# ska-telescope/ska-sdp-distributed-fourier-transform

Measured on AMD Instinct MI355X. Metric: facet_to_subgrid_contributions_per_s, higher is better.
Workload: dtype complex64 (f32 arithmetic)

## Files before the change

include/swiftly_hip.h:

```cpp
#ifndef SWIFTLY_HIP_H
#define SWIFTLY_HIP_H

#include <stddef.h>
#include <stdint.h>

#ifdef __cplusplus
extern "C" {
#endif

typedef struct swiftly_hip swiftly_hip_t;

enum { SWIFTLY_C64 = 0, SWIFTLY_C128 = 1 };
enum {
    SWIFTLY_OK = 0,
    SWIFTLY_ERR_PARAM = 1,
    SWIFTLY_ERR_UNSUPPORTED = 2,
    SWIFTLY_ERR_HIP = 3
};

const char* swiftly_hip_last_error(void);
int swiftly_hip_version(void);
int swiftly_hip_device_count(void);
const char* swiftly_hip_build_id(void);

int swiftly_hip_create(swiftly_hip_t** out, int64_t N, int64_t yN_size, int64_t xM_size, double W,
                       const double* pswf, int device);
void swiftly_hip_destroy(swiftly_hip_t* h);
int64_t swiftly_hip_contribution_size(const swiftly_hip_t* h);
int swiftly_hip_supports_dtype(const swiftly_hip_t* h, int dtype);
enum {
    SWIFTLY_FEATURE_FUSED_SUBGRID = 0,
    SWIFTLY_FEATURE_BAND_PIPELINE = 1,
    SWIFTLY_FEATURE_BAND_PIPELINE_EXPLICIT = 2,
    SWIFTLY_FEATURE_BACKWARD_BAND = 3,
    SWIFTLY_FEATURE_SPLIT_BAND = 4,
    SWIFTLY_FEATURE_WINDOW_ROWS = 5,
    SWIFTLY_FEATURE_BACKWARD_BAND_EXPLICIT = 6,
    SWIFTLY_FEATURE_SPLIT_PREPARE = 7
};
int swiftly_hip_supports(int feature, int dtype, int64_t N, int64_t yN_size, int64_t xM_size, int64_t n_facets);
enum {
    SWIFTLY_LIMIT_FUSED_FACETS = 0,
    SWIFTLY_LIMIT_WINDOW_ROWS_STAGE_COLUMNS = 1,
    SWIFTLY_LIMIT_WINDOW_ROWS_WINDOWS = 2
};
int64_t swiftly_hip_limit(int which);
int swiftly_hip_mixed_factor(int64_t n, int* Q, int* log2_rest);
int swiftly_hip_set_column_precision(swiftly_hip_t* h, int bits);
int swiftly_hip_get_column_precision(const swiftly_hip_t* h);
void swiftly_hip_chain_chunk_streams(int chain);


int swiftly_hip_prepare_facet(swiftly_hip_t* h, int dtype, const void* in, int64_t rows, int64_t facet_size,
                              int64_t in_row_stride, int64_t in_col_stride, void* out, int64_t out_row_stride,
                              int64_t out_col_stride, int64_t facet_off, void* stream);

int swiftly_hip_extract_from_facet(swiftly_hip_t* h, int dtype, const void* in, int64_t rows, int64_t in_row_stride,
                                   int64_t in_col_stride, void* out, int64_t out_row_stride, int64_t out_col_stride,
                                   int64_t subgrid_off, void* stream);

int swiftly_hip_add_to_subgrid(swiftly_hip_t* h, int dtype, const void* in, int64_t rows, int64_t in_row_stride,
                               int64_t in_col_stride, void* out, int64_t out_row_stride, int64_t out_col_stride,
                               int64_t facet_off, void* stream);

int swiftly_hip_add_to_subgrid_2d(swiftly_hip_t* h, int dtype, const void* in, int64_t in_row_stride,
                                  int64_t in_col_stride, void* out, int64_t out_row_stride, int64_t out_col_stride,
                                  int64_t facet_off0, int64_t facet_off1, void* stream);

int swiftly_hip_finish_subgrid(swiftly_hip_t* h, int dtype, const void* in, int64_t rows, int64_t in_row_stride,
                               int64_t in_col_stride, void* out, int64_t out_row_stride, int64_t out_col_stride,
                               int64_t subgrid_off, int64_t subgrid_size, const void* mask, void* stream);


int swiftly_hip_prepare_subgrid(swiftly_hip_t* h, int dtype, const void* in, int64_t rows, int64_t subgrid_size,
                                int64_t in_row_stride, int64_t in_col_stride, void* out, int64_t out_row_stride,
                                int64_t out_col_stride, int64_t subgrid_off, void* stream);

int swiftly_hip_prepare_subgrid_inplace(swiftly_hip_t* h, int dtype, void* data, int64_t rows, int64_t row_stride,
                                        int64_t col_stride, int64_t subgrid_off, void* stream);
int swiftly_hip_prepare_subgrid_inplace_2d(swiftly_hip_t* h, int dtype, void* data, int64_t row_stride, int64_t col_stride,
                                           int64_t subgrid_off0, int64_t subgrid_off1, void* stream);

int swiftly_hip_extract_from_subgrid(swiftly_hip_t* h, int dtype, const void* in, int64_t rows, int64_t in_row_stride,
                                     int64_t in_col_stride, void* out, int64_t out_row_stride,
                                     int64_t out_col_stride, int64_t facet_off, void* stream);

int swiftly_hip_add_to_facet(swiftly_hip_t* h, int dtype, const void* in, int64_t rows, int64_t in_row_stride,
                             int64_t in_col_stride, void* out, int64_t out_row_stride, int64_t out_col_stride,
                             int64_t subgrid_off, void* stream);

int swiftly_hip_finish_facet(swiftly_hip_t* h, int dtype, const void* in, int64_t rows, int64_t in_row_stride,
                             int64_t in_col_stride, void* out, int64_t out_row_stride, int64_t out_col_stride,
                             int64_t facet_off, int64_t facet_size, const void* mask, void* stream);



int swiftly_hip_extract_column(swiftly_hip_t* h, int dtype, const void* in, int64_t facet_size,
                               int64_t in_row_stride, int64_t in_col_stride, void* out, int64_t out_row_stride,
                               int64_t out_col_stride, int64_t subgrid_off0, int64_t facet_off1, void* stream);

int swiftly_hip_prepare_facet_rows(swiftly_hip_t* h, int dtype, const void* in, int64_t rows, int64_t facet_size,
                                   int64_t in_row_stride, int64_t in_col_stride, void* out, int64_t out_row_stride,
                                   int64_t out_col_stride, int64_t facet_off, const int32_t* rowmap,
                                   int fold_other_axis_window, void* stream);
int swiftly_hip_extract_column_rows(swiftly_hip_t* h, int dtype, const void* in, int64_t facet_size,
                                    int64_t in_row_stride, int64_t in_col_stride, void* out, int64_t out_row_stride,
                                    int64_t out_col_stride, int64_t subgrid_off0, int64_t facet_off1,
                                    const int32_t* rowmap, int prewindowed, void* stream);

int swiftly_hip_extract_from_facet_batch(swiftly_hip_t* h, int dtype, const void* in, int64_t rows,
                                         int64_t in_row_stride, int64_t in_col_stride, void* out,
                                         int64_t out_row_stride, int64_t out_col_stride, int64_t subgrid_off,
                                         int64_t nbatch, int64_t in_batch_stride, int64_t out_batch_stride,
                                         const int64_t* subgrid_offs, void* stream);
int swiftly_hip_add_to_subgrid_batch(swiftly_hip_t* h, int dtype, const void* in, int64_t rows,
                                     int64_t in_row_stride, int64_t in_col_stride, void* out, int64_t out_row_stride,
                                     int64_t out_col_stride, int64_t facet_off, int64_t nbatch,
                                     int64_t in_batch_stride, int64_t out_batch_stride, const int64_t* facet_offs,
                                     void* stream);
int swiftly_hip_finish_subgrid_batch(swiftly_hip_t* h, int dtype, const void* in, int64_t rows,
                                     int64_t in_row_stride, int64_t in_col_stride, void* out, int64_t out_row_stride,
                                     int64_t out_col_stride, int64_t subgrid_off, int64_t subgrid_size,
                                     const void* mask, int64_t nbatch, int64_t in_batch_stride,
                                     int64_t out_batch_stride, const int64_t* subgrid_offs,
                                     int64_t mask_batch_stride, void* stream);
int swiftly_hip_prepare_subgrid_batch(swiftly_hip_t* h, int dtype, const void* in, int64_t rows,
                                      int64_t subgrid_size, int64_t in_row_stride, int64_t in_col_stride, void* out,
                                      int64_t out_row_stride, int64_t out_col_stride, int64_t subgrid_off,
                                      int64_t nbatch, int64_t in_batch_stride, int64_t out_batch_stride,
                                      const int64_t* subgrid_offs, void* stream);
int swiftly_hip_extract_from_subgrid_batch(swiftly_hip_t* h, int dtype, const void* in, int64_t rows,
                                           int64_t in_row_stride, int64_t in_col_stride, void* out,
                                           int64_t out_row_stride, int64_t out_col_stride, int64_t facet_off,
                                           int64_t nbatch, int64_t in_batch_stride, int64_t out_batch_stride,
                                           const int64_t* facet_offs, void* stream);
int swiftly_hip_add_to_facet_batch(swiftly_hip_t* h, int dtype, const void* in, int64_t rows, int64_t in_row_stride,
                                   int64_t in_col_stride, void* out, int64_t out_row_stride, int64_t out_col_stride,
                                   int64_t subgrid_off, int64_t nbatch, int64_t in_batch_stride,
                                   int64_t out_batch_stride, const int64_t* subgrid_offs, void* stream);
int swiftly_hip_finish_facet_batch(swiftly_hip_t* h, int dtype, const void* in, int64_t rows, int64_t in_row_stride,
                                   int64_t in_col_stride, void* out, int64_t out_row_stride, int64_t out_col_stride,
                                   int64_t facet_off, int64_t facet_size, const void* mask, int64_t nbatch,
                                   int64_t in_batch_stride, int64_t out_batch_stride, const int64_t* facet_offs,
                                   int64_t mask_batch_stride, void* stream);

int swiftly_hip_sum_finish_rows(swiftly_hip_t* h, int dtype, const void* in, int64_t ngroups, int64_t in_group_stride,
                                int64_t in_batch_stride, int64_t in_row_stride, const int64_t* group_facet_offs,
                                void* out, int64_t out_batch_stride, int64_t out_row_stride,
                                const int64_t* subgrid_offs, int64_t subgrid_size, const void* mask,
                                int64_t mask_batch_stride, int64_t nbatch, void* stream);

int swiftly_hip_add_to_subgrid_from_columns(swiftly_hip_t* h, int dtype, const void* in, int64_t in_row_stride,
                                            int64_t in_facet_stride, int64_t nfacets, void* out,
                                            int64_t out_col_stride, int64_t out_batch_stride, int64_t facet_off0,
                                            int64_t nsub, const int64_t* subgrid_off1s, void* stream);


int64_t swiftly_hip_band_columns(int64_t band_len);
int64_t swiftly_hip_band_columns_for(const swiftly_hip_t* h, int64_t band_len);

int swiftly_hip_prepare_facet_band(swiftly_hip_t* h, int dtype, const void* in, int64_t rows, int64_t facet_size,
                                   int64_t in_row_stride, void* out, int64_t out_row_stride, int64_t facet_off,
                                   int64_t band_start, int64_t band_len, int fold_other_axis_window, void* stream);
int swiftly_hip_prepare_facet_band_rows(swiftly_hip_t* h, int dtype, const void* in, int64_t rows, int64_t facet_size,
                                        int64_t in_row_stride, void* out, int64_t out_row_stride, int64_t facet_off,
                                        int64_t band_start, int64_t band_len, int64_t other_axis_size,
                                        int64_t other_axis_row0, void* stream);

int swiftly_hip_prepare_facet_columns(swiftly_hip_t* h, int dtype, const void* in, int64_t rows, int64_t in_row_stride,
                                      int64_t in_facet_stride, int64_t nfacets, const int64_t* facet_off0s,
                                      int64_t band_start, int64_t band_len, int64_t subgrid_off1, void* out,
                                      int64_t out_row_stride, int64_t out_facet_stride, const int32_t* out_rowmap,
                                      void* stream);

int swiftly_hip_prepare_facet_columns_waves(swiftly_hip_t* h, int dtype, const void* in, int64_t rows,
                                            int64_t in_row_stride, int64_t in_facet_stride, int64_t nfacets,
                                            const int64_t* facet_off0s, int64_t band_start, int64_t band_len,
                                            int64_t nwaves, const int64_t* wave_off1s, void* out, int64_t out_row_stride,
                                            int64_t out_facet_stride, int64_t out_wave_stride, const int32_t* rowmaps,
                                            int64_t rowmap_stride, void* workspace, int64_t workspace_bytes,
                                            void* stream);

int swiftly_hip_prepare_facet_columns_range(swiftly_hip_t* h, int dtype, const void* in, int64_t rows, int64_t in_row_stride,
                                            int64_t in_facet_stride, int64_t nfacets, const int64_t* facet_off0s,
                                            int64_t band_start, int64_t band_len, int64_t subgrid_off1, int64_t col_first,
                                            int64_t ncols, void* out, int64_t out_row_stride, int64_t out_facet_stride,
                                            const int32_t* out_rowmap, void* workspace, int64_t workspace_bytes,
                                            void* stream);

int swiftly_hip_transform_contributions(swiftly_hip_t* h, int dtype, const void* in, int layout, int64_t in_row_stride,
                                        int64_t in_facet_stride, int64_t in_sub_stride, const int32_t* in_rowmap,
                                        int64_t band_start, int64_t band_len, int64_t nfacets,
                                        const int64_t* facet_off0s, int64_t nsub, const int64_t* subgrid_offs,
                                        void* out, int64_t out_facet_stride, int64_t out_sub_stride, void* stream);

int swiftly_hip_transform_contributions_pieces(swiftly_hip_t* h, int dtype, int64_t npieces, const void* const* q,
                                               const int64_t* q_facet_strides, const int32_t* const* rowmaps,
                                               const int64_t* n_rows, const int64_t* first, const int64_t* count,
                                               int64_t nfacets, const int64_t* facet_off0s, int64_t nsub,
                                               const int64_t* sub_off0s, void* g_out, int64_t g_facet_stride,
                                               int64_t g_sub_stride, const int64_t* g_offsets,
                                               const int64_t* g_facet_strides, void* stream);
int swiftly_hip_k3_one_launch(int on);

int swiftly_hip_sum_finish_facets(swiftly_hip_t* h, int dtype, const void* in, int64_t nfacets, int64_t in_facet_stride,
                                  int64_t in_sub_stride, int64_t in_row_stride, const int64_t* facet_off0s,
                                  const int64_t* facet_off1s, void* out, int64_t out_sub_stride, int64_t out_row_stride,
                                  const int64_t* subgrid_off1s, int64_t subgrid_size, const void* mask,
                                  int64_t mask_batch_stride, int64_t nsub, void* stream);

int swiftly_hip_wave_facet_side(swiftly_hip_t* h, int dtype, const void* bands, int64_t rows, int64_t band_row_stride,
                                int64_t band_facet_stride, int64_t nfacets, const int64_t* facet_off0s,
                                int64_t band_start, int64_t band_len, int64_t wave_off1, const int32_t* rowmap,
                                int64_t n_rows, void* q_work, int64_t q_facet_stride, int compute_q, int64_t nsub,
                                const int64_t* sub_off0s, void* g_out, int64_t g_facet_stride, int64_t g_sub_stride,
                                const int64_t* g_offsets, const int64_t* g_facet_strides, void* scratch,
                                int64_t scratch_bytes, void* stream);
int swiftly_hip_wave_subgrid_side(swiftly_hip_t* h, int dtype, const void* g, int64_t nfacets, int64_t g_facet_stride,
                                  int64_t g_sub_stride, const int64_t* facet_off0s, const int64_t* facet_off1s,
                                  int64_t nsub, const int64_t* sub_off0s, const int64_t* sub_off1s, int64_t subgrid_size,
                                  const void* mask0, int64_t mask0_bs, const void* mask1, int64_t mask1_bs,
                                  void* tmp_work, void* out, void* scratch, int64_t scratch_bytes, void* stream);

int swiftly_hip_finish_axis1_rows(swiftly_hip_t* h, int dtype, const void* bands, int64_t rows, int64_t band_row_stride,
                                  int64_t band_facet_stride, int64_t nfacets, const int64_t* facet_off1s,
                                  int64_t band_start, int64_t band_len, int64_t wave_off1, void* out,
                                  int64_t out_row_stride, int64_t out_facet_stride, void* stream);
int swiftly_hip_wave_subgrid_side_placed(swiftly_hip_t* h, int dtype, const void* g, int64_t nfacets, int64_t g_facet_stride,
                                         int64_t g_sub_stride, const int64_t* facet_off0s, const int64_t* facet_off1s,
                                         int64_t nsub, const int64_t* sub_off0s, const int64_t* sub_off1s,
                                         int64_t subgrid_size, const void* mask0, int64_t mask0_bs, const void* mask1,
                                         int64_t mask1_bs, void* tmp_work, void* out, void* scratch, int64_t scratch_bytes,
                                         void* stream);

int swiftly_hip_prepare_facet_window_rows(swiftly_hip_t* h, int dtype, const void* in, int64_t rows, int64_t facet_size,
                                          int64_t in_row_stride, void* out, int64_t out_row_stride, int64_t facet_off,
                                          int64_t band_start, int64_t band_len, int64_t other_axis_size,
                                          int64_t other_axis_row0, const int32_t* window_starts, int64_t nwindows,
                                          int64_t out_window_stride, void* stream);
int swiftly_hip_split_prepare_facets(swiftly_hip_t* h, int dtype, const void* in, int64_t in_sub_stride,
                                     int64_t in_row_stride, int64_t subgrid_size, int64_t nsub,
                                     const int64_t* subgrid_off1s, int64_t nfacets, const int64_t* facet_off0s,
                                     const int64_t* facet_off1s, void* out, int64_t out_facet_stride,
                                     int64_t out_sub_stride, void* stream);

int swiftly_hip_wave_split_subgrids(swiftly_hip_t* h, int dtype, const void* subgrids, int64_t subgrid_size, int64_t nsub,
                                    const int64_t* subgrid_off0s, const int64_t* subgrid_off1s, int64_t nfacets,
                                    const int64_t* facet_off0s, const int64_t* facet_off1s, void* work,
                                    int64_t work_elems, void* out, int64_t out_facet_stride, int64_t out_sub_stride,
                                    void* stream);

int swiftly_hip_accumulate_facet_columns(swiftly_hip_t* h, int dtype, const void* parts, int64_t part_row_stride,
                                         int64_t nchunks, const int64_t* chunk_offsets,
                                         const int64_t* chunk_facet_strides, const int32_t* row_sources,
                                         int64_t nfacets, const int64_t* facet_off0s, int64_t facet_size,
                                         const void* masks, int64_t subgrid_off1, void* bands, int64_t band_row_stride,
                                         int64_t band_facet_stride, int64_t band_start, int64_t band_len,
                                         unsigned char* touched, void* workspace, int64_t workspace_bytes,
                                         void* stream);
int swiftly_hip_band_zero_untouched(swiftly_hip_t* h, int dtype, void* bands, int64_t rows, int64_t band_row_stride,
                                    int64_t band_len, const unsigned char* touched, void* stream);
int swiftly_hip_finish_facet_band(swiftly_hip_t* h, int dtype, const void* in, int64_t rows, int64_t in_row_stride,
                                  int64_t band_start, int64_t band_len, void* out, int64_t out_row_stride,
                                  int64_t facet_off, int64_t facet_size, const void* mask, void* stream);

int swiftly_hip_subgrids_from_sources(int dtype, const void* sources, int64_t n_sources, int64_t image_size,
                                      int64_t size, const int64_t* off0s, const int64_t* off1s, int64_t n_subgrids,
                                      const double* mask0s, const double* mask1s, void* out, int64_t out_sub_stride,
                                      int64_t out_row_stride, void* stream);
int swiftly_hip_check_subgrids_from_sources(int dtype, const void* sources, int64_t n_sources, int64_t image_size,
                                            int64_t size, const int64_t* off0s, const int64_t* off1s,
                                            int64_t n_subgrids, const double* mask0s, const double* mask1s,
                                            const void* approx, int64_t approx_sub_stride, int64_t approx_row_stride,
                                            double* result, void* stream);
int swiftly_hip_facet_from_sources(int dtype, const void* sources, int64_t n_sources, int64_t image_size, int64_t size,
                                   int64_t off0, int64_t off1, const double* mask0, const double* mask1, void* out,
                                   int64_t out_row_stride, void* stream);
int swiftly_hip_check_facet_from_sources(int dtype, const void* sources, int64_t n_sources, int64_t image_size,
                                         int64_t size, int64_t off0, int64_t off1, const double* mask0,
                                         const double* mask1, const void* approx, int64_t approx_row_stride,
                                         const int32_t* row_start, const int32_t* row_sources, double* result,
                                         void* stream);

int swiftly_hip_malloc(void** ptr, size_t bytes);
int swiftly_hip_free(void* ptr);
int swiftly_hip_memset_async(void* ptr, int value, size_t bytes, void* stream);
int swiftly_hip_memcpy_h2d(void* dst, const void* src, size_t bytes, void* stream);
int swiftly_hip_memcpy_d2h(void* dst, const void* src, size_t bytes, void* stream);
int swiftly_hip_stream_synchronize(void* stream);

int swiftly_hip_stream_create_cu_mask(void** stream, const uint32_t* cu_mask, int nwords);
int swiftly_hip_stream_destroy(void* stream);
int swiftly_hip_cu_census(int32_t* out, int nblocks, void* stream);

int swiftly_hip_kernel_table(int64_t* count, int64_t* max_lds_bytes);

#ifdef __cplusplus
}
#endif
#endif
```

ska-sdp-distributed-fourier-transform_amd/csrc/col_pass.hip:

```cpp
#include <cstdlib>

#include "swiftly_colpass.h"
#include "swiftly_launch.h"

namespace swf {

using CGeo512Half = CGeo<9, 5, true, 32>;
static int col512_tile32() {
    static const int v = getenv("SWIFTLY_COL512_TILE32") ? atoi(getenv("SWIFTLY_COL512_TILE32")) : 1;
    return v;
}

bool col_pass_pieces_supported(int logn, const ColPassArgs& a) {
    if (a.c128 || a.gs || a.in_bdiv <= 0 || a.in_bs) return false;
    if (a.f64) return logn == 9 && a.twd;
    return logn == 7 || logn == 8 || (logn == 9 && a.tile32 && col512_tile32());
}
template <class G, typename RC>
static int launch_pieces(const ColPassArgs& a, const ColPassSrc2& s2, const ColZ& cz, int outer, int nbatch, hipStream_t s,
                         const cx<RC>* tw, const cx<RC>* tw_full) {
    dim3 grid((unsigned)((a.ncols + G::COLS - 1) / G::COLS), (unsigned)outer, (unsigned)nbatch);
    return launch_lds<col_pass2_kernel<G, RC>, G::LDS_BYTES>(grid, dim3(G::NT), s, a, s2, a.in, a.out, a.ld_win, a.ld_win2,
                                                             a.st_win, a.st_win2, a.st_rowmap, tw, tw_full, cz);
}
template <int LOGN>
static int launch_mode_pieces(const ColPassArgs& a, const ColPassSrc2& s2, const ColZ& cz, int outer, int nbatch,
                              hipStream_t s) {
    if (!col_pass_pieces_supported(LOGN, a)) return (int)hipErrorInvalidConfiguration;
    if constexpr (LOGN == 9) {
        if (a.f64) return launch_pieces<typename CGeoFor<9, double>::type, double>(a, s2, cz, outer, nbatch, s, a.twd, a.twd_full);
        return launch_pieces<CGeo512Half, float>(a, s2, cz, outer, nbatch, s, a.tw, a.tw_full);
    }
    if constexpr (LOGN == 7 || LOGN == 8)
        return launch_pieces<typename CGeoFor<LOGN>::type, float>(a, s2, cz, outer, nbatch, s, a.tw, a.tw_full);
    return (int)hipErrorInvalidConfiguration;
}

template <int LOGN, int MODE>
static int launch_mode(const ColPassArgs& a, const ColZ& cz, int outer, int nbatch, hipStream_t s) {
    using G = typename CGeoFor<LOGN>::type;
    if constexpr (LOGN == 9 && MODE == 2) {
        if (a.tile32 && !a.gs && col512_tile32()) {
            using GH = CGeo512Half;
            dim3 hgrid((unsigned)((a.ncols + GH::COLS - 1) / GH::COLS), (unsigned)outer, (unsigned)nbatch);
            return launch_lds<col_pass_kernel<GH, 2, true>, GH::LDS_BYTES>(hgrid, dim3(GH::NT), s, a, a.in, a.out, a.ld_win,
                                                                           a.ld_win2, a.st_win, a.st_win2, a.st_rowmap, a.tw,
                                                                           a.tw_full, cz);
        }
    }
    dim3 grid((unsigned)((a.ncols + G::COLS - 1) / G::COLS), (unsigned)outer, (unsigned)nbatch);
    if constexpr (MODE == 1 || G::HALF) {
        if (a.gs) return (int)hipErrorInvalidConfiguration;
    }
    if constexpr (MODE != 1 && !G::HALF) {
        if (a.gs) {
            return launch_lds<col_pass_kernel<G, MODE, true, true>, G::LDS_BYTES>(grid, dim3(G::NT), s, a, a.in, a.out, a.ld_win,
                                                                                  a.ld_win2, a.st_win, a.st_win2, a.st_rowmap,
                                                                                  a.tw, a.tw_full, cz);
        }
    }
    if (MODE == 2 || a.scratch_nt)
        return launch_lds<col_pass_kernel<G, MODE, true>, G::LDS_BYTES>(grid, dim3(G::NT), s, a, a.in, a.out, a.ld_win, a.ld_win2,
                                                                        a.st_win, a.st_win2, a.st_rowmap, a.tw, a.tw_full, cz);
    return launch_lds<col_pass_kernel<G, (MODE == 2 ? 0 : MODE), false>, G::LDS_BYTES>(
        grid, dim3(G::NT), s, a, a.in, a.out, a.ld_win, a.ld_win2, a.st_win, a.st_win2, a.st_rowmap, a.tw, a.tw_full, cz);
}
constexpr int kColF64MinLog = 5;
template <int LOGN, int MODE>
static int launch_mode_f64(const ColPassArgs& a, const ColZ& cz, int outer, int nbatch, hipStream_t s) {
    if constexpr (LOGN < kColF64MinLog || LOGN > kColPassMaxLogF64) {
        return (int)hipErrorInvalidConfiguration;
    } else {
        using G = typename CGeoFor<LOGN, double>::type;
        if (!a.twd || (MODE == 0 && !a.twd_full)) return (int)hipErrorInvalidValue;
        if (a.gs) {
            using GG = typename CGeoFor<LOGN, double>::type_gs;
            if constexpr (MODE != 1 && !GG::HALF) {
                dim3 ggrid((unsigned)((a.ncols + GG::COLS - 1) / GG::COLS), (unsigned)outer, (unsigned)nbatch);
                return launch_lds<col_pass_kernel<GG, MODE, true, true, double>, GG::LDS_BYTES>(
                    ggrid, dim3(GG::NT), s, a, a.in, a.out, a.ld_win, a.ld_win2, a.st_win, a.st_win2, a.st_rowmap, a.twd,
                    a.twd_full, cz);
            } else {
                return (int)hipErrorInvalidConfiguration;
            }
        }
        dim3 grid((unsigned)((a.ncols + G::COLS - 1) / G::COLS), (unsigned)outer, (unsigned)nbatch);
        if (MODE == 2 || a.scratch_nt)
            return launch_lds<col_pass_kernel<G, MODE, true, false, double>, G::LDS_BYTES>(
                grid, dim3(G::NT), s, a, a.in, a.out, a.ld_win, a.ld_win2, a.st_win, a.st_win2, a.st_rowmap, a.twd, a.twd_full, cz);
        return launch_lds<col_pass_kernel<G, (MODE == 2 ? 0 : MODE), false, false, double>, G::LDS_BYTES>(
            grid, dim3(G::NT), s, a, a.in, a.out, a.ld_win, a.ld_win2, a.st_win, a.st_win2, a.st_rowmap, a.twd, a.twd_full, cz);
    }
}

template <int LOGN>
struct CGeoC128 : CGeoFor<LOGN, double>::type {};
template <>
struct CGeoC128<8> : CGeo<8, 4, true, 32, 8> {
    static constexpr int MINW = 2;
};
template <int LOGN, int MODE>
constexpr bool kColC128HasGs = (MODE == 0 && LOGN >= 5 && LOGN <= 7) || (MODE == 2 && LOGN >= 6 && LOGN <= kColPassMaxLogF64);
template <int LOGN, int MODE>
static int launch_mode_c128(const ColPassArgs& a, const ColZ& cz, int outer, int nbatch, hipStream_t s) {
    if constexpr (LOGN < kColF64MinLog || LOGN > kColPassMaxLogF64) {
        return (int)hipErrorInvalidConfiguration;
    } else {
        using G = CGeoC128<LOGN>;
        if (!a.twd || (MODE == 0 && !a.twd_full)) return (int)hipErrorInvalidValue;
        const cx<double>* in = reinterpret_cast<const cx<double>*>(a.in);
        cx<double>* out = reinterpret_cast<cx<double>*>(a.out);
        dim3 grid((unsigned)((a.ncols + G::COLS - 1) / G::COLS), (unsigned)outer, (unsigned)nbatch);
        if (a.gs) {
            if constexpr (kColC128HasGs<LOGN, MODE>) {
                return launch_lds<col_pass_kernel<G, MODE, true, true, double, double>, G::LDS_BYTES>(
                    grid, dim3(G::NT), s, a, in, out, a.ld_win, a.ld_win2, a.st_win, a.st_win2, a.st_rowmap, a.twd, a.twd_full, cz);
            } else {
                return (int)hipErrorInvalidConfiguration;
            }
        }
        if (MODE == 2 || a.scratch_nt)
            return launch_lds<col_pass_kernel<G, MODE, true, false, double, double>, G::LDS_BYTES>(
                grid, dim3(G::NT), s, a, in, out, a.ld_win, a.ld_win2, a.st_win, a.st_win2, a.st_rowmap, a.twd, a.twd_full, cz);
        return launch_lds<col_pass_kernel<G, (MODE == 2 ? 0 : MODE), false, false, double, double>, G::LDS_BYTES>(
            grid, dim3(G::NT), s, a, in, out, a.ld_win, a.ld_win2, a.st_win, a.st_win2, a.st_rowmap, a.twd, a.twd_full, cz);
    }
}

template <int LOGN>
static int launch_one(int mode, const ColPassArgs& a, const ColZ& cz, int outer, int nbatch, hipStream_t s,
                      const ColPassSrc2* src2) {
    if (src2) return mode == 2 ? launch_mode_pieces<LOGN>(a, *src2, cz, outer, nbatch, s) : (int)hipErrorInvalidConfiguration;
    if (a.c128) {
        if (mode == 0) return launch_mode_c128<LOGN, 0>(a, cz, outer, nbatch, s);
        if (mode == 1) return launch_mode_c128<LOGN, 1>(a, cz, outer, nbatch, s);
        return launch_mode_c128<LOGN, 2>(a, cz, outer, nbatch, s);
    }
    if (a.f64) {
        if (mode == 0) return launch_mode_f64<LOGN, 0>(a, cz, outer, nbatch, s);
        if (mode == 1) return launch_mode_f64<LOGN, 1>(a, cz, outer, nbatch, s);
        return launch_mode_f64<LOGN, 2>(a, cz, outer, nbatch, s);
    }
    if (mode == 0) return launch_mode<LOGN, 0>(a, cz, outer, nbatch, s);
    if (mode == 1) return launch_mode<LOGN, 1>(a, cz, outer, nbatch, s);
    return launch_mode<LOGN, 2>(a, cz, outer, nbatch, s);
}

template <int LO, int HI>
struct CDispatch {
    static int launch(int logn, int mode, const ColPassArgs& a, const ColZ& cz, int outer, int nbatch, hipStream_t s,
                      const ColPassSrc2* src2) {
        if (logn == LO) return launch_one<LO>(mode, a, cz, outer, nbatch, s, src2);
        if constexpr (LO < HI) return CDispatch<LO + 1, HI>::launch(logn, mode, a, cz, outer, nbatch, s, src2);
        return -1;
    }
};

int launch_col_pass(int logn, int mode, const ColPassArgs& a, const ColZ& cz, int outer, int nbatch, hipStream_t s,
                    const ColPassSrc2* src2) {
    return CDispatch<kColPassMinLog, kColPassMaxLog>::launch(logn, mode, a, cz, outer, nbatch, s, src2);
}
bool col_pass_f64_supported(int logn) { return logn >= kColF64MinLog && logn <= kColPassMaxLogF64; }

}
```

ska-sdp-distributed-fourier-transform_amd/csrc/sum_finish.hip:

```cpp
#include "swiftly_launch.h"
#include "swiftly_sumfinish.h"

namespace swf {

template <int LOGM, int LOGX>
static int launch_one(const SumFinishArgs& a, int nbatch, hipStream_t s) {
    using S = SFGeo<LOGM, LOGX>;
    dim3 grid((unsigned)((a.nrows + S::RB - 1) / S::RB), (unsigned)nbatch);
    return launch_lds<sum_finish_rows_kernel<LOGM, LOGX>, S::LDS_BYTES>(grid, dim3(S::NT), s, a);
}

template <int LOGM, int LOGX, typename R = float>
static int launch_one_f(const SumFinishFacetArgs& a, int nbatch, hipStream_t s) {
    using S = SFGeo<LOGM, LOGX, R>;
    dim3 grid((unsigned)((a.nrows + S::RB - 1) / S::RB), (unsigned)nbatch);
    constexpr size_t lds = sum_finish_facets_kernel_lds<LOGM, LOGX, R>();
    return launch_lds<sum_finish_facets_kernel<LOGM, LOGX, R>, lds>(grid, dim3(S::NT), s, a);
}
template <int LOGM, int LOGX, typename R>
constexpr size_t split_prepare_lds() {
    if constexpr (std::is_same_v<R, float>) return sum_finish_facets_lds<LOGM, LOGX>();
    else return SFGeo<LOGM, LOGX, R>::LDS_BYTES;
}
template <int LOGM, int LOGX, typename R = float>
static int launch_one_s(const SplitFacetArgs& a, int nbatch, hipStream_t s) {
    using S = SFGeo<LOGM, LOGX, R>;
    dim3 grid((unsigned)((a.nrows + S::RB - 1) / S::RB), (unsigned)nbatch);
    constexpr size_t lds = split_prepare_lds<LOGM, LOGX, R>();
    return launch_lds<split_prepare_facets_kernel<LOGM, LOGX, R>, lds>(grid, dim3(S::NT), s, a);
}

template <int LOGM>
static int launch_axis1(const Axis1RowsArgs& a, int nfacets, hipStream_t s) {
    using GM = typename Axis1Geo<LOGM>::GM;
    dim3 grid((unsigned)((a.nrows + GM::RB - 1) / GM::RB), (unsigned)nfacets);
    return launch_lds<axis1_rows_kernel<LOGM>, Axis1Geo<LOGM>::LDS_BYTES>(grid, dim3(kAxis1Threads), s, a);
}
int launch_axis1_rows(int logm, const Axis1RowsArgs& a, int nfacets, hipStream_t s) {
    switch (logm) {
        case 7: return launch_axis1<7>(a, nfacets, s);
        case 8: return launch_axis1<8>(a, nfacets, s);
        case 9: return launch_axis1<9>(a, nfacets, s);
        case 10: return launch_axis1<10>(a, nfacets, s);
        default: return -1;
    }
}


int launch_sum_finish_rows(int logm, int logx, const SumFinishArgs& a, int nbatch, hipStream_t s) {
#define SF_CASE(M, XX) \
    if (logm == M && logx == XX) return launch_one<M, XX>(a, nbatch, s);
    SF_PAIRS(SF_CASE)
#undef SF_CASE
    return -1;
}
int launch_sum_finish_facets(int logm, int logx, const SumFinishFacetArgs& a, int nbatch, hipStream_t s) {
#define SF_CASE_F(M, XX) \
    if (logm == M && logx == XX) return launch_one_f<M, XX>(a, nbatch, s);
    SF_PAIRS(SF_CASE_F)
#undef SF_CASE_F
    return -1;
}
int launch_sum_finish_facets_c128(int logm, int logx, const SumFinishFacetArgs& a, int nbatch, hipStream_t s) {
#define SF_CASE_D(M, XX) \
    if (logm == M && logx == XX) return launch_one_f<M, XX, double>(a, nbatch, s);
    SF_PAIRS_C128(SF_CASE_D)
#undef SF_CASE_D
    return -1;
}
int launch_split_prepare_facets(int logm, int logx, const SplitFacetArgs& a, int nbatch, hipStream_t s) {
#define SF_CASE_S(M, XX) \
    if (logm == M && logx == XX) return launch_one_s<M, XX>(a, nbatch, s);
    SF_PAIRS(SF_CASE_S)
#undef SF_CASE_S
    return -1;
}
int launch_split_prepare_facets_c128(int logm, int logx, const SplitFacetArgs& a, int nbatch, hipStream_t s) {
#define SF_CASE_SD(M, XX) \
    if (logm == M && logx == XX) return launch_one_s<M, XX, double>(a, nbatch, s);
    SPLIT_PAIRS_C128(SF_CASE_SD)
#undef SF_CASE_SD
    return -1;
}

}
```

ska-sdp-distributed-fourier-transform_amd/csrc/swiftly_abi_pipeline.hip:

```cpp
#include "swiftly_abi_internal.h"

__global__ void mark_columns_kernel(unsigned char* __restrict__ touched, int m, int rot, int base, int yN, int band_start,
                                    int band_len) {
    const int col = blockIdx.x * blockDim.x + threadIdx.x;
    if (col >= m) return;
    int scol = base + ((col + rot) & (m - 1));
    if (scol >= yN) scol -= yN;
    int d = scol - band_start;
    if (d < 0) d += yN;
    if (d < band_len) touched[d] = 1;
}
template <typename R>
__global__ void zero_untouched_kernel(cx<R>* __restrict__ band, const unsigned char* __restrict__ touched, long long rows,
                                      long long pitch, int band_len) {
    const int d = blockIdx.x * blockDim.x + threadIdx.x;
    if (d >= band_len || touched[d]) return;
    for (long long r = blockIdx.y; r < rows; r += gridDim.y) band[r * pitch + d] = cx<R>{(R)0, (R)0};
}


extern "C" {

int swiftly_hip_sum_finish_rows(swiftly_hip_t* h, int dtype, const void* in, int64_t ngroups, int64_t in_group_stride,
                                int64_t in_batch_stride, int64_t in_row_stride, const int64_t* group_facet_offs,
// ... 298 lines not shown
static int transform_contributions_impl(swiftly_hip_t* h, int dtype, const void* in, int layout, int64_t in_row_stride,
                                        int64_t in_facet_stride, int64_t in_sub_stride, const int32_t* in_rowmap,
                                        int64_t band_start, int64_t band_len, int64_t nfacets,
                                        const int64_t* facet_off0s, int64_t nsub, const int64_t* subgrid_offs,
                                        void* out, int64_t out_facet_stride, int64_t out_sub_stride,
                                        const int64_t* out_offs, const int64_t* out_fstrides, void* stream,
                                        int64_t col_first = 0, int64_t ncols = -1, const SecondSource* in_b = nullptr) {
    if (!h || !in || !out || !facet_off0s) return fail(SWIFTLY_ERR_PARAM, "null argument");
    if (ncols < 0) ncols = h->m;
    if (col_first < 0 || ncols <= 0 || col_first + ncols > h->m || ((col_first || ncols != h->m) && layout != 1))
        return fail(SWIFTLY_ERR_PARAM, "transform_contributions: bad column range [%lld, +%lld)", (long long)col_first, (long long)ncols);
    if (in_b && (layout != 1 || col_first || ncols != h->m || !in_b->in || in_b->split <= 0 || in_b->split >= h->m || in_b->split % 16))
        return fail(SWIFTLY_ERR_PARAM, "transform_contributions: bad second source (split %lld)", (long long)(in_b ? in_b->split : 0));
    const bool c128 = dtype == SWIFTLY_C128;
    CHECK_DTYPE();
    if (layout < 0 || layout > 2) return fail(SWIFTLY_ERR_PARAM, "bad layout %d", layout);
    if (c128 && (layout == 0 || !band_pipeline_c128_supported(h)))
        return fail(SWIFTLY_ERR_UNSUPPORTED, "transform_contributions: complex128 takes layouts 1 and 2 and m = 32 .. 512 with a "
                    "complex128 sum_finish_facets instance, got layout %d, m %lld, xM %lld", layout, (long long)h->m,
                    (long long)h->xM);
    if (layout != 2 && !subgrid_offs) return fail(SWIFTLY_ERR_PARAM, "null argument");
    const int m = (int)h->m, yN = (int)h->yN;
    if (h->log_m < kColPassMinLog || h->log_m > kColPassMaxLog || (layout == 0 && h->log_yN < 0))
        return fail(SWIFTLY_ERR_UNSUPPORTED, "transform_contributions: contribution size %d not supported", m);
    if (nfacets <= 0 || nsub <= 0) return 0;
    CHECK_OFFSETS_32(offsets_fit_32(yN, in_row_stride, yN));
    ColPassArgs c = col_pass_args(whole(m), whole(m));
    c.ncols = (int)ncols;
    c.full_logn = h->log_m;
    c.in_pitch = (unsigned)in_row_stride;
    c.out_pitch = (unsigned)m;
    c.st_win = c128 ? (const float*)h->fn_d : h->fn_f;
    c.scale = 1.f;
    c.tw = twiddles<float>(h, h->log_m);
    if (!c.tw) return fail(SWIFTLY_ERR_HIP, "internal: missing twiddle table");
    if (layout == 0) {
        c.cg_mod = m; c.cg_full = yN;
        c.cg_band_start = (int)band_start; c.cg_band_len = (int)band_len; c.cg_band_half = band_half_of(h, band_len);
    } else if (layout == 1) {
        c.ld_mod = yN;
        c.ld_rowmap = in_rowmap;
        c.tile32 = 1;
    }
    for (int64_t f0 = 0; f0 < nfacets; f0 += kColZF) {
        const int nf = (int)std::min<int64_t>(kColZF, nfacets - f0);
        for (int64_t b0 = 0; b0 < nsub; b0 += kColZB) {
            const int nb = (int)std::min<int64_t>(kColZB, nsub - b0);
            ColZ cz = plain_colz();
            cz.nb = nb;
            cz.flags = kZStoreAF;
            for (int f = 0; f < nf; f++) cz.f_sta[f] = contribution_in_padded_subgrid(*h, facet_off0s[f0 + f]).a;
            for (int b = 0; b < nb && layout != 2; b++) {
                const Window w = window_of(*h, subgrid_offs[b0 + b]);
                if (layout == 0) {
                    cz.b_rot[b] = w.rot;
                    cz.b_base[b] = w.base;
                } else {
                    cz.b_lda[b] = w.rot;
                    cz.b_ldc[b] = w.base;
                }
            }
            if (layout == 0) cz.flags |= kZColGather;
            if (layout == 1) cz.flags |= kZLoadB;
            c.in = cx_at(in, f0 * in_facet_stride + (layout == 2 ? b0 * in_sub_stride : 0) + col_first, c128);
            c.in_bdiv = nb; c.in_bs_hi = in_facet_stride; c.in_bs = layout == 2 ? in_sub_stride : 0;
            c.out = cx_at(out, f0 * out_facet_stride + b0 * out_sub_stride + col_first, c128);
            c.out_bdiv = nb; c.out_bs_hi = out_facet_stride; c.out_bs = out_sub_stride;
            if (out_offs) {
                cz.flags |= kZOutB;
                c.out = cx_at(out, col_first, c128);
                for (int b = 0; b < nb; b++) {
                    cz.b_out_fs[b] = out_fstrides[b0 + b];
                    cz.b_out_off[b] = out_offs[b0 + b] + f0 * out_fstrides[b0 + b];
                }
            }
            if (int rc = set_col_precision(h, c, h->log_m, c128)) return rc;
            ColPassSrc2 src2 = {};
            if (in_b) {
                if (!col_pass_pieces_supported(h->log_m, c))
                    return fail(SWIFTLY_ERR_UNSUPPORTED, "transform_contributions: no two-source instance for m = %d", m);
                src2.in = cx_at(in_b->in, f0 * in_b->facet_stride, c128);
                src2.in_bs_hi = in_b->facet_stride;
                src2.ld_rowmap = in_b->rowmap;
                src2.split = (int)in_b->split;
            }
            if (int rc = launch_col_checked(h->log_m, 2, c, cz, 1, nf * nb, (hipStream_t)stream, in_b ? &src2 : nullptr)) return rc;
        }
    }
    return 0;
}

static std::atomic<int> g_k3_one_launch{getenv("SWIFTLY_K3_ONE_LAUNCH") ? atoi(getenv("SWIFTLY_K3_ONE_LAUNCH")) != 0 : 1};

extern "C" {
int swiftly_hip_k3_one_launch(int on) {
    return on < 0 ? g_k3_one_launch.load() : g_k3_one_launch.exchange(on ? 1 : 0);
}

int swiftly_hip_transform_contributions(swiftly_hip_t* h, int dtype, const void* in, int layout, int64_t in_row_stride,
                                        int64_t in_facet_stride, int64_t in_sub_stride, const int32_t* in_rowmap,
                                        int64_t band_start, int64_t band_len, int64_t nfacets,
                                        const int64_t* facet_off0s, int64_t nsub, const int64_t* subgrid_offs,
                                        void* out, int64_t out_facet_stride, int64_t out_sub_stride, void* stream) {
    if (!h) return fail(SWIFTLY_ERR_PARAM, "null argument");
    DeviceGuard device_guard_(h->device);
    return transform_contributions_impl(h, dtype, in, layout, in_row_stride, in_facet_stride, in_sub_stride, in_rowmap,
                                        band_start, band_len, nfacets, facet_off0s, nsub, subgrid_offs, out,
                                        out_facet_stride, out_sub_stride, nullptr, nullptr, stream);
}

int swiftly_hip_transform_contributions_pieces(swiftly_hip_t* h, int dtype, int64_t npieces, const void* const* q,
                                               const int64_t* q_facet_strides, const int32_t* const* rowmaps,
                                               const int64_t* n_rows, const int64_t* first, const int64_t* count,
                                               int64_t nfacets, const int64_t* facet_off0s, int64_t nsub,
                                               const int64_t* sub_off0s, void* g_out, int64_t g_facet_stride,
                                               int64_t g_sub_stride, const int64_t* g_offsets,
                                               const int64_t* g_facet_strides, void* stream) {
    if (!h || !q || !q_facet_strides || !rowmaps || !n_rows || !first || !count || !g_out || !facet_off0s || !sub_off0s)
        return fail(SWIFTLY_ERR_PARAM, "null argument");
    if (npieces < 0 || npieces > 2) return fail(SWIFTLY_ERR_PARAM, "transform_contributions_pieces: 0..2 pieces, got %lld", (long long)npieces);
    if (!g_offsets != !g_facet_strides) return fail(SWIFTLY_ERR_PARAM, "g_offsets and g_facet_strides go together");
    DeviceGuard device_guard_(h->device);
    const int64_t m = h->m;
    int64_t covered = 0;
    for (int64_t i = 0; i < npieces; i++) {
        if (count[i] < 0 || first[i] < 0 || first[i] + count[i] > m || first[i] % 16 || count[i] % 16)
            return fail(SWIFTLY_ERR_PARAM, "transform_contributions_pieces: piece %lld = [%lld, +%lld) must be multiples of 16 "
                        "inside [0, %lld)", (long long)i, (long long)first[i], (long long)count[i], (long long)m);
        if (count[i] && (!q[i] || n_rows[i] <= 0 || n_rows[i] > h->yN || q_facet_strides[i] < n_rows[i] * m))
            return fail(SWIFTLY_ERR_PARAM, "bad row count %lld / facet stride %lld", (long long)n_rows[i], (long long)q_facet_strides[i]);
        covered += count[i];
    }
    if (npieces == 2 && count[0] && count[1] && first[0] < first[1] + count[1] && first[1] < first[0] + count[0])
        return fail(SWIFTLY_ERR_PARAM, "transform_contributions_pieces: the pieces overlap");
    if (covered != m) return fail(SWIFTLY_ERR_PARAM, "transform_contributions_pieces: the pieces hold %lld of %lld positions", (long long)covered, (long long)m);
    if (npieces == 2 && count[0] && count[1] && g_k3_one_launch.load()) {
        const int b = first[0] == 0 ? 0 : 1, a = 1 - b;
        const SecondSource second = {q[b], q_facet_strides[b], rowmaps[b], count[b]};
        const int rc = transform_contributions_impl(h, dtype, q[a], 1, m, q_facet_strides[a], 0, rowmaps[a], 0, 0, nfacets,
                                                    facet_off0s, nsub, sub_off0s, g_out, g_facet_stride, g_sub_stride,
                                                    g_offsets, g_facet_strides, stream, 0, -1, &second);
        if (rc != SWIFTLY_ERR_UNSUPPORTED) return rc;
    }
    for (int64_t i = 0; i < npieces; i++) {
        if (!count[i]) continue;
        if (int rc = transform_contributions_impl(h, dtype, q[i], 1, m, q_facet_strides[i], 0, rowmaps[i], 0, 0, nfacets,
                                                  facet_off0s, nsub, sub_off0s, g_out, g_facet_stride, g_sub_stride, g_offsets,
                                                  g_facet_strides, stream, first[i], count[i]))
            return rc;
    }
    return 0;
}

static int sum_finish_facets_impl(swiftly_hip_t* h, int dtype, const void* in, int64_t nfacets, int64_t in_facet_stride,
                                  int64_t in_sub_stride, int64_t in_row_stride, const int64_t* facet_off0s,
                                  const int64_t* facet_off1s, void* out, int64_t out_sub_stride, int64_t out_row_stride,
                                  const int64_t* subgrid_off1s, int64_t subgrid_size, const void* mask,
                                  int64_t mask_batch_stride, int64_t nsub, int placed, void* stream) {
    if (!h || !in || !out || !facet_off0s || !facet_off1s || !subgrid_off1s) return fail(SWIFTLY_ERR_PARAM, "null argument");
    DeviceGuard device_guard_(h->device);
    CHECK_SUBGRID_SIZE();
    const bool c128 = dtype == SWIFTLY_C128;
    CHECK_DTYPE();
    if (nfacets <= 0 || nfacets > kSumFinishMaxFacets)
        return fail(SWIFTLY_ERR_UNSUPPORTED, "sum_finish_facets: 1..%d facets supported", kSumFinishMaxFacets);
    if (c128 && (placed || !sum_finish_c128_supported(h->log_m, h->log_xM)))
        return fail(SWIFTLY_ERR_UNSUPPORTED, "sum_finish_facets: complex128 %s", placed ? "has no placed mode (axis-1-first pipeline)"
                    : ("instances exist for (m, xM) = " + sum_finish_c128_sizes()).c_str());
    if (!sum_finish_supported(h->log_m, h->log_xM))
        return fail(SWIFTLY_ERR_UNSUPPORTED, "sum_finish_facets: (m, xM) = (%lld, %lld) not instantiated", (long long)h->m,
                    (long long)h->xM);
    if (nsub <= 0) return 0;
    const int xM = (int)h->xM, xA = (int)subgrid_size;
    SumFinishFacetArgs a;
    std::memset(&a, 0, sizeof a);
    a.in_fs = in_facet_stride; a.in_bs = in_sub_stride; a.in_rs = in_row_stride;
    a.out_bs = out_sub_stride; a.out_rs = out_row_stride;
    a.nrows = xM;
    a.nfacets = (int)nfacets;
    a.xA = xA;
    fill_facet_groups(a, h, nfacets, facet_off0s, facet_off1s);
    fill_group_rounds(a, h);
    a.placed = placed ? 1 : 0;
    if (placed && h->log_xM > kPlacedMaxLogXM)
        return fail(SWIFTLY_ERR_UNSUPPORTED, "axis-1-first pipeline: rows of %lld points run the wave-parallel sum_finish form, "
                    "which has no placed mode", (long long)h->xM);
    a.mask_bs = mask ? mask_batch_stride : 0;
    if (int rc = fill_sum_finish_tables(h, c128, &a.fn, &a.tw_m, &a.tw_x, &a.twc_m, &a.twc_x)) return rc;
    for (int64_t b0 = 0; b0 < nsub; b0 += kSumFinishMaxBatch) {
        const int nb = (int)std::min<int64_t>(kSumFinishMaxBatch, nsub - b0);
        a.in = cx_at(in, b0 * in_sub_stride, c128);
        a.out = cx_at(out, b0 * out_sub_stride, c128);
        a.mask = mask ? (const float*)((const char*)mask + b0 * mask_batch_stride * (c128 ? 8 : 4)) : nullptr;
        for (int b = 0; b < nb; b++) a.st_a[b] = subgrid_in_padded_subgrid(*h, xA, subgrid_off1s[b0 + b]).a;
        int e = c128 ? launch_sum_finish_facets_c128(h->log_m, h->log_xM, a, nb, (hipStream_t)stream)
                     : launch_sum_finish_facets(h->log_m, h->log_xM, a, nb, (hipStream_t)stream);
        if (int rc = launch_status(e)) return rc;
    }
    return 0;
}

int swiftly_hip_sum_finish_facets(swiftly_hip_t* h, int dtype, const void* in, int64_t nfacets, int64_t in_facet_stride,
                                  int64_t in_sub_stride, int64_t in_row_stride, const int64_t* facet_off0s,
                                  const int64_t* facet_off1s, void* out, int64_t out_sub_stride, int64_t out_row_stride,
                                  const int64_t* subgrid_off1s, int64_t subgrid_size, const void* mask,
                                  int64_t mask_batch_stride, int64_t nsub, void* stream) {
    return sum_finish_facets_impl(h, dtype, in, nfacets, in_facet_stride, in_sub_stride, in_row_stride, facet_off0s, facet_off1s,
                                  out, out_sub_stride, out_row_stride, subgrid_off1s, subgrid_size, mask, mask_batch_stride, nsub,
                                  0, stream);
}

int swiftly_hip_finish_axis1_rows(swiftly_hip_t* h, int dtype, const void* bands, int64_t rows, int64_t band_row_stride,
                                  int64_t band_facet_stride, int64_t nfacets, const int64_t* facet_off1s,
                                  int64_t band_start, int64_t band_len, int64_t wave_off1, void* out,
                                  int64_t out_row_stride, int64_t out_facet_stride, void* stream) {
    if (!h || !bands || !out || !facet_off1s) return fail(SWIFTLY_ERR_PARAM, "null argument");
    DeviceGuard device_guard_(h->device);
    if (dtype != SWIFTLY_C64) return fail(SWIFTLY_ERR_UNSUPPORTED, "finish_axis1_rows: complex64 only");
    if (!band_is_split(h) || h->log_m < 7 || h->log_m > 10)
        return fail(SWIFTLY_ERR_UNSUPPORTED, "finish_axis1_rows: needs the parity-split band layout (yN_size 16384 .. 65536) and "
                    "m = 128 .. 1024");
    if (nfacets <= 0 || nfacets > kSumFinishMaxFacets)
        return fail(SWIFTLY_ERR_UNSUPPORTED, "finish_axis1_rows: 1..%d facets supported", kSumFinishMaxFacets);
    const int yN = (int)h->yN, m = (int)h->m;
    CHECK_BAND();
    if (rows <= 0) return 0;
    Axis1RowsArgs a;
    std::memset(&a, 0, sizeof a);
    a.in = (const cx<float>*)bands; a.out = (cx<float>*)out;
    a.in_fs = band_facet_stride; a.in_rs = band_row_stride; a.out_fs = out_facet_stride; a.out_rs = out_row_stride;
    a.nrows = (int)rows; a.yN = yN;
    a.band_start = (int)band_start; a.band_len = (int)band_len; a.band_half = (int)band_half_columns(band_len);
    const Window w = window_of(*h, wave_off1);
    a.c0 = w.base;
    a.s = pmod(w.s, m);
    if (window_in_band(*h, w, 0, m, band_start, band_len) >= 0)
        return fail(SWIFTLY_ERR_PARAM, "finish_axis1_rows: the window of off1 = %lld is not inside the band", (long long)wave_off1);
    for (int64_t f = 0; f < nfacets; f++) a.sp[f] = pmod(facet_shift(*h, facet_off1s[f]), m);
    if (int rc = fill_sum_finish_tables(h, false, &a.fn, &a.tw_m, nullptr, &a.twc_m, nullptr)) return rc;
    return launch_status(launch_axis1_rows(h->log_m, a, (int)nfacets, (hipStream_t)stream), nullptr, "no instance");
}

int swiftly_hip_split_prepare_facets(swiftly_hip_t* h, int dtype, const void* in, int64_t in_sub_stride,
                                     int64_t in_row_stride, int64_t subgrid_size, int64_t nsub,
                                     const int64_t* subgrid_off1s, int64_t nfacets, const int64_t* facet_off0s,
                                     const int64_t* facet_off1s, void* out, int64_t out_facet_stride,
                                     int64_t out_sub_stride, void* stream) {
    if (!h || !in || !out || !facet_off0s || !facet_off1s || !subgrid_off1s) return fail(SWIFTLY_ERR_PARAM, "null argument");
    DeviceGuard device_guard_(h->device);
    CHECK_SUBGRID_SIZE();
    const bool c128 = dtype == SWIFTLY_C128;
    CHECK_DTYPE();
    if (nfacets <= 0) return fail(SWIFTLY_ERR_UNSUPPORTED, "split_prepare_facets: 1..%d facets supported", kSumFinishMaxFacets);
    if (const std::string why = why_not_split_prepare(*h, dtype, nfacets); !why.empty())
        return fail(SWIFTLY_ERR_UNSUPPORTED, "split_prepare_facets: %s", why.c_str());
    if (nsub <= 0) return 0;
    const int xM = (int)h->xM, xA = (int)subgrid_size, m = (int)h->m;
    SplitFacetArgs a;
    std::memset(&a, 0, sizeof a);
    a.in_bs = in_sub_stride; a.in_rs = in_row_stride;
    a.out_fs = out_facet_stride; a.out_bs = out_sub_stride; a.out_rs = m;
    a.nrows = xM;
    a.nfacets = (int)nfacets;
    a.xA = xA;
    fill_facet_groups(a, h, nfacets, facet_off0s, facet_off1s);
    if (int rc = fill_sum_finish_tables(h, c128, &a.fn, &a.tw_m, &a.tw_x, c128 ? nullptr : &a.twc_m, c128 ? nullptr : &a.twc_x))
        return rc;
    for (int64_t b0 = 0; b0 < nsub; b0 += kSumFinishMaxBatch) {
        const int nb = (int)std::min<int64_t>(kSumFinishMaxBatch, nsub - b0);
        a.in = cx_at(in, b0 * in_sub_stride, c128);
        a.out = cx_at(out, b0 * out_sub_stride, c128);
        for (int b = 0; b < nb; b++) a.ld_a[b] = subgrid_in_padded_subgrid(*h, xA, subgrid_off1s[b0 + b]).a;
        int e = c128 ? launch_split_prepare_facets_c128(h->log_m, h->log_xM, a, nb, (hipStream_t)stream)
                     : launch_split_prepare_facets(h->log_m, h->log_xM, a, nb, (hipStream_t)stream);
        if (int rc = launch_status(e, nullptr, "no instance")) return rc;
    }
    ColPassArgs c = col_pass_args(whole(m), whole(m));
    c.ncols = m;
    c.full_logn = h->log_m;
    c.in_pitch = c.out_pitch = (unsigned)m;
    c.ld_win = c128 ? (const float*)h->fn_d : h->fn_f;
    c.conj_ld = c.conj_st = 1;
    c.scale = 1.f / (float)m;
    c.tw = twiddles<float>(h, h->log_m);
    for (int64_t f0 = 0; f0 < nfacets; f0 += kColZF) {
        const int nf = (int)std::min<int64_t>(kColZF, nfacets - f0);
        for (int64_t b0 = 0; b0 < nsub; b0 += kColZB) {
            const int nb = (int)std::min<int64_t>(kColZB, nsub - b0);
            ColZ cz = plain_colz();
            cz.nb = nb;
            cz.flags = kZLoadAF;
            for (int f = 0; f < nf; f++) cz.f_lda[f] = contribution_in_padded_subgrid(*h, facet_off0s[f0 + f]).a;
            c.in = cx_at((const void*)out, f0 * out_facet_stride + b0 * out_sub_stride, c128);
            c.in_bdiv = nb; c.in_bs_hi = out_facet_stride; c.in_bs = out_sub_stride;
            c.out = cx_at(out, f0 * out_facet_stride + b0 * out_sub_stride, c128);
            c.out_bdiv = nb; c.out_bs_hi = out_facet_stride; c.out_bs = out_sub_stride;
            if (int rc = set_col_precision(h, c, h->log_m, c128)) return rc;
            if (int rc = launch_col_checked(h->log_m, 2, c, cz, 1, nf * nb, (hipStream_t)stream)) return rc;
        }
    }
    return 0;
}

int swiftly_hip_wave_split_subgrids(swiftly_hip_t* h, int dtype, const void* subgrids, int64_t subgrid_size, int64_t nsub,
                                    const int64_t* subgrid_off0s, const int64_t* subgrid_off1s, int64_t nfacets,
                                    const int64_t* facet_off0s, const int64_t* facet_off1s, void* work,
                                    int64_t work_elems, void* out, int64_t out_facet_stride, int64_t out_sub_stride,
                                    void* stream) {
    if (!h || !subgrids || !work || !out || !subgrid_off0s || !subgrid_off1s) return fail(SWIFTLY_ERR_PARAM, "null argument");
    DeviceGuard device_guard_(h->device);
    CHECK_SUBGRID_SIZE();
    const bool c128 = dtype == SWIFTLY_C128;
    CHECK_DTYPE();
    if (const std::string why = why_not_split_prepare(*h, dtype, nfacets); !why.empty())
        return fail(SWIFTLY_ERR_UNSUPPORTED, "wave_split_subgrids: %s", why.c_str());
    if (nsub <= 0 || nfacets <= 0) return 0;
    const int xM = (int)h->xM, xA = (int)subgrid_size;
    const int64_t half = nsub * (int64_t)xM * xA;
    if (work_elems < 2 * half) return fail(SWIFTLY_ERR_PARAM, "work holds %lld elements, %lld needed", (long long)work_elems, (long long)(2 * half));
    void* tmp = work;
    const size_t esz = c128 ? sizeof(cx<double>) : sizeof(cx<float>);
    ColPassArgs c = col_pass_args(whole(xA), whole(xM));
    c.c128 = c128 ? 1 : 0;
    c.ncols = xA;
    c.full_logn = h->log_xM;
    c.in_pitch = c.out_pitch = (unsigned)xA;
    c.scale = 1.f;
    for (int64_t b0 = 0; b0 < nsub; b0 += kColZB) {
        const int nb = (int)std::min<int64_t>(kColZB, nsub - b0);
        ColZ cz = plain_colz();
        cz.nb = nb;
        cz.flags = kZLoadB;
        for (int b = 0; b < nb; b++) {
            cz.b_lda[b] = subgrid_in_padded_subgrid(*h, xA, subgrid_off0s[b0 + b]).a;
            cz.b_ldc[b] = 0;
        }
        c.in = cx_at(subgrids, b0 * (int64_t)xA * xA, c128);
        c.in_bs = (long long)xA * xA;
        c.out = cx_at(tmp, b0 * (int64_t)xM * xA, c128);
        c.out_bs = (long long)xM * xA;
        const int rc = col_transform(h, h->log_xM, c, cz, xA, nb, (hipStream_t)stream, cx_at(tmp, half, c128), (size_t)half * esz);
        if (rc == -1) return fail(SWIFTLY_ERR_UNSUPPORTED, "wave_split_subgrids: padded subgrid size %d not supported", xM);
        if (rc) return rc;
    }
    return swiftly_hip_split_prepare_facets(h, dtype, tmp, (int64_t)xM * xA, xA, subgrid_size, nsub, subgrid_off1s, nfacets,
                                            facet_off0s, facet_off1s, out, out_facet_stride, out_sub_stride, stream);
}


int swiftly_hip_wave_facet_side(swiftly_hip_t* h, int dtype, const void* bands, int64_t rows, int64_t band_row_stride,
                                int64_t band_facet_stride, int64_t nfacets, const int64_t* facet_off0s,
                                int64_t band_start, int64_t band_len, int64_t wave_off1, const int32_t* rowmap,
                                int64_t n_rows, void* q_work, int64_t q_facet_stride, int compute_q, int64_t nsub,
                                const int64_t* sub_off0s, void* g_out,
                                int64_t g_facet_stride, int64_t g_sub_stride, const int64_t* g_offsets,
                                const int64_t* g_facet_strides, void* scratch, int64_t scratch_bytes, void* stream) {
    if (!h || (!bands && compute_q) || !q_work || !g_out || !facet_off0s || !sub_off0s) return fail(SWIFTLY_ERR_PARAM, "null argument");
    if (nfacets <= 0 || nsub <= 0) return 0;
    const int64_t m = h->m;
    if (n_rows <= 0 || n_rows > h->yN || q_facet_stride < n_rows * m)
        return fail(SWIFTLY_ERR_PARAM, "bad row count %lld / facet stride %lld", (long long)n_rows, (long long)q_facet_stride);
    DeviceGuard device_guard_(h->device);
    if (compute_q) {
        int rc = prepare_facet_columns_impl(h, dtype, bands, rows, band_row_stride, band_facet_stride, nfacets, facet_off0s,
                                            band_start, band_len, 1, &wave_off1, q_work, m, q_facet_stride, 0, rowmap, 0,
                                            stream, scratch, scratch ? (size_t)scratch_bytes : 0);
        if (rc) return rc;
    }
    return transform_contributions_impl(h, dtype, q_work, 1, m, q_facet_stride, 0, rowmap, 0, 0, nfacets, facet_off0s, nsub,
                                        sub_off0s, g_out, g_facet_stride, g_sub_stride, g_offsets, g_facet_strides, stream);
}

static int wave_subgrid_side_impl(swiftly_hip_t* h, int dtype, const void* g, int64_t nfacets, int64_t g_facet_stride,
                                  int64_t g_sub_stride, const int64_t* facet_off0s, const int64_t* facet_off1s,
                                  int64_t nsub, const int64_t* sub_off0s, const int64_t* sub_off1s, int64_t subgrid_size,
                                  const void* mask0, int64_t mask0_bs, const void* mask1, int64_t mask1_bs,
                                  void* tmp_work, void* out, void* scratch, int64_t scratch_bytes, int placed, void* stream) {
    if (!h || !g || !tmp_work || !out || !sub_off0s || !sub_off1s) return fail(SWIFTLY_ERR_PARAM, "null argument");
    if (nsub <= 0) return 0;
    const int64_t m = h->m, xM = h->xM, xA = subgrid_size;
    int rc = sum_finish_facets_impl(h, dtype, g, nfacets, g_facet_stride, g_sub_stride, m, facet_off0s, facet_off1s,
                                    tmp_work, xM * xA, xA, sub_off1s, subgrid_size, mask1, mask1_bs, nsub, placed, stream);
    if (rc) return rc;
    CallWorkspace call_ws(scratch, scratch ? (size_t)scratch_bytes : 0);
    return swiftly_hip_finish_subgrid_batch(h, dtype, tmp_work, xA, 1, xA, out, 1, xA, 0, subgrid_size, mask0, nsub,
                                            xM * xA, xA * xA, sub_off0s, mask0 ? mask0_bs : 0, stream);
}

int swiftly_hip_wave_subgrid_side(swiftly_hip_t* h, int dtype, const void* g, int64_t nfacets, int64_t g_facet_stride,
                                  int64_t g_sub_stride, const int64_t* facet_off0s, const int64_t* facet_off1s,
                                  int64_t nsub, const int64_t* sub_off0s, const int64_t* sub_off1s, int64_t subgrid_size,
                                  const void* mask0, int64_t mask0_bs, const void* mask1, int64_t mask1_bs,
                                  void* tmp_work, void* out, void* scratch, int64_t scratch_bytes, void* stream) {
    return wave_subgrid_side_impl(h, dtype, g, nfacets, g_facet_stride, g_sub_stride, facet_off0s, facet_off1s, nsub, sub_off0s,
                                  sub_off1s, subgrid_size, mask0, mask0_bs, mask1, mask1_bs, tmp_work, out, scratch, scratch_bytes,
                                  0, stream);
}

int swiftly_hip_wave_subgrid_side_placed(swiftly_hip_t* h, int dtype, const void* g, int64_t nfacets, int64_t g_facet_stride,
                                         int64_t g_sub_stride, const int64_t* facet_off0s, const int64_t* facet_off1s,
                                         int64_t nsub, const int64_t* sub_off0s, const int64_t* sub_off1s,
                                         int64_t subgrid_size, const void* mask0, int64_t mask0_bs, const void* mask1,
                                         int64_t mask1_bs, void* tmp_work, void* out, void* scratch, int64_t scratch_bytes,
                                         void* stream) {
    return wave_subgrid_side_impl(h, dtype, g, nfacets, g_facet_stride, g_sub_stride, facet_off0s, facet_off1s, nsub, sub_off0s,
                                  sub_off1s, subgrid_size, mask0, mask0_bs, mask1, mask1_bs, tmp_work, out, scratch, scratch_bytes,
                                  1, stream);
}


int swiftly_hip_accumulate_facet_columns(swiftly_hip_t* h, int dtype, const void* parts, int64_t part_row_stride,
                                         int64_t nchunks, const int64_t* chunk_offsets,
                                         const int64_t* chunk_facet_strides, const int32_t* row_sources,
                                         int64_t nfacets, const int64_t* facet_off0s, int64_t facet_size,
                                         const void* masks, int64_t subgrid_off1, void* bands, int64_t band_row_stride,
                                         int64_t band_facet_stride, int64_t band_start, int64_t band_len,
                                         unsigned char* touched, void* workspace, int64_t workspace_bytes,
                                         void* stream) {
    if (!h || !parts || !bands || !chunk_offsets || !chunk_facet_strides || !row_sources || !facet_off0s)
        return fail(SWIFTLY_ERR_PARAM, "null argument");
    DeviceGuard device_guard_(h->device);
    const bool c128 = dtype == SWIFTLY_C128;
    CHECK_DTYPE();
    CHECK_FACET_SIZE();
    const int yN = (int)h->yN, m = (int)h->m;
    const swiftly_hip::Mixed* mx = nullptr;
    if (h->log_yN < 0) {
        auto it = h->mixed.find(h->yN);
        if (it != h->mixed.end() && it->second.tw_f && !band_is_split(h)) mx = &it->second;
    }
    if (const std::string why = why_not_backward_band(*h, dtype, true); !why.empty())
        return fail(SWIFTLY_ERR_UNSUPPORTED, "accumulate_facet_columns: %s", why.c_str());
    if (h->log_yN < 0 && !mx)
        return fail(SWIFTLY_ERR_UNSUPPORTED, "accumulate_facet_columns: yN %lld = Q * 2^k has no complex64 radix-Q table "
                    "(2^k above %d), or would need the split band layout", (long long)h->yN, 1 << kBandMixedMaxLog);
    if (nchunks <= 0 || nchunks > kColZC) return fail(SWIFTLY_ERR_PARAM, "1..%d source chunks", kColZC);
    CHECK_BAND();
    if (nfacets <= 0) return 0;
    CHECK_OFFSETS_32(offsets_fit_32(facet_size, band_row_stride) && offsets_fit_32(uint64_t(1) << kGsRowBits, part_row_stride));
    const int lo = facet_lo(*h, facet_size);
    ColPassArgs c = col_pass_args(whole(yN), whole(facet_size));
    c.ncols = m;
    c.full_logn = h->log_yN;
    c.in = (const cx<float>*)parts;
    c.in_pitch = (unsigned)part_row_stride;
    c.out_pitch = (unsigned)band_row_stride;
    c.ld_rowmap = row_sources; c.gs = 1;
    c.f64 = h->col_f64;
    c.c128 = c128 ? 1 : 0;
    const size_t rsz = c128 ? sizeof(double) : sizeof(float);
    c.st_win = (const float*)masks; c.st_win_bs = masks ? facet_size : 0;
    c.st_win2 = c128 ? (const float*)(h->invp_d + lo) : h->invp_f + lo;
    c.scale = 1.f;
    c.accumulate = 1;
    c.touched = touched;
    c.cg_mod = m; c.cg_full = yN;
    c.cg_band_start = (int)band_start; c.cg_band_len = (int)band_len; c.cg_band_half = 0;
    const int64_t cap = workspace ? workspace_bytes : (int64_t(4) << 30);
    const int64_t per_item = mx ? (int64_t)MixedWorkspace(1, yN, 1ll << mx->logM, m).bytes() : (int64_t)yN * m * (c128 ? 16 : 8);
    const int per_f = (int)std::max<int64_t>(1, std::min<int64_t>(kColZF, cap / per_item));
    const Window win = window_of(*h, subgrid_off1);
    for (int64_t f0 = 0; f0 < nfacets; f0 += per_f) {
        const int nf = (int)std::min<int64_t>(per_f, nfacets - f0);
        ColZ cz = plain_colz();
        cz.flags = kZColScatter | kZStoreAF;
        cz.nb = 1;
        cz.b_rot[0] = win.rot;
        cz.b_base[0] = win.base;
        for (int f = 0; f < nf; f++) cz.f_sta[f] = facet_in_padded_facet(*h, facet_size, facet_off0s[f0 + f]).a;
        for (int k = 0; k < nchunks; k++) {
            cz.c_base[k] = chunk_offsets[k] + f0 * chunk_facet_strides[k];
            cz.c_fs[k] = chunk_facet_strides[k];
        }
        c.out = cx_at(bands, f0 * band_facet_stride, c128);
        c.out_bs = band_facet_stride;
        if (masks) c.st_win = (const float*)((const char*)masks + (size_t)(f0 * facet_size) * rsz);
        int rc = 0;
        if (!mx) {
            rc = col_transform(h, h->log_yN, c, cz, m, nf, (hipStream_t)stream, workspace,
                               workspace ? (size_t)workspace_bytes : 0);
        } else {
            const int Q = mx->Q, logM = mx->logM;
            const long long M = 1ll << logM;
            const MixedWorkspace part(nf, yN, M, m);
            hipStream_t st = (hipStream_t)stream;
            ScratchLease lease;
            if ((rc = lease.acquire(workspace, (size_t)workspace_bytes, part.bytes(), st, "hipMallocAsync(&own, radix_bytes + sub_bytes, st)")))
                return rc;
            MixedGsArgs g;
            std::memset(&g, 0, sizeof g);
            g.in = (const cx<float>*)parts;
            g.in_pitch = (unsigned)part_row_stride;
            g.rowmap = row_sources;
            g.ncols = m;
            for (int k = 0; k < nchunks; k++) {
                g.c_base[k] = cz.c_base[k];
                g.c_fs[k] = cz.c_fs[k];
            }
            MixedArgs<float> X = mixed_args<float>(*mx, yN);
            X.scratch = (cx<float>*)lease.p;
            X.s_row = 1; X.s_y = m; X.s_j = M * m; X.s_b = (long long)yN * m;
            rc = radix_launch_status(launch_mixed_gs_pass(Q, g, X, nf, st), Q, "gather-sum pass");
            for (int j = 0; j < Q && !rc; j++) {
                ColPassArgs cs = c;
                cs.in = X.scratch + (long long)j * X.s_j;
                cs.in_pitch = (unsigned)m;
                cs.in_bs = X.s_b; cs.in_bdiv = 0; cs.in_bs_hi = 0;
                cs.ld_rowmap = nullptr; cs.gs = 0;
                rc = col_transform(h, logM, cs, cz, m, nf, st, part.sub(lease.p), part.sub_bytes, Q, j, yN);
            }
            rc = lease.release(rc);
        }
        if (rc == -1) return fail(SWIFTLY_ERR_UNSUPPORTED, "accumulate_facet_columns: padded facet size %d not supported", yN);
        if (rc) return rc;
    }
    if (touched) {
        hipLaunchKernelGGL(mark_columns_kernel, dim3((unsigned)((m + 255) / 256)), dim3(256), 0, (hipStream_t)stream, touched,
                           m, win.rot, win.base, yN, (int)band_start, (int)band_len);
        HIP_TRY(hipGetLastError());
    }
    return 0;
}

int swiftly_hip_band_zero_untouched(swiftly_hip_t* h, int dtype, void* bands, int64_t rows, int64_t band_row_stride,
                                    int64_t band_len, const unsigned char* touched, void* stream) {
    if (!h || !bands || !touched) return fail(SWIFTLY_ERR_PARAM, "null argument");
    DeviceGuard device_guard_(h->device);
    CHECK_DTYPE();
    if (rows <= 0 || band_len <= 0) return 0;
    dim3 grid((unsigned)((band_len + 63) / 64), (unsigned)std::min<int64_t>(rows, 1024));
    if (dtype == SWIFTLY_C128)
        hipLaunchKernelGGL(zero_untouched_kernel<double>, grid, dim3(64), 0, (hipStream_t)stream, (cx<double>*)bands, touched,
                           (long long)rows, (long long)band_row_stride, (int)band_len);
    else
        hipLaunchKernelGGL(zero_untouched_kernel<float>, grid, dim3(64), 0, (hipStream_t)stream, (cx<float>*)bands, touched,
                           (long long)rows, (long long)band_row_stride, (int)band_len);
    HIP_TRY(hipGetLastError());
    return 0;
}


}
```

ska-sdp-distributed-fourier-transform_amd/csrc/swiftly_abi_util.hip:

```cpp
#include "swiftly_abi_internal.h"
#include "build/build_id.h"

__global__ void cu_census_kernel(int* __restrict__ out) {
    unsigned xcc, hw;
    asm volatile("s_getreg_b32 %0, hwreg(HW_REG_XCC_ID)" : "=s"(xcc));
    asm volatile("s_getreg_b32 %0, hwreg(HW_REG_HW_ID)" : "=s"(hw));
    const long long t0 = __builtin_readcyclecounter();
    while (__builtin_readcyclecounter() - t0 < 20000) {
    }
    if (threadIdx.x == 0) out[blockIdx.x] = (int)(((xcc & 0xf) << 16) | (((hw >> 13) & 0x7) << 8) | ((hw >> 8) & 0xf));
}


thread_local int g_chain_chunk_streams = 0;

namespace swf {
struct KernelLdsEntry {
    const void* host_fn;
    int lds_bytes;
};
static std::vector<KernelLdsEntry>& kernel_lds_table() {
    static std::vector<KernelLdsEntry> table;
    return table;
}
bool register_kernel_lds(const void* host_fn, int lds_bytes) {
    kernel_lds_table().push_back({host_fn, lds_bytes});
    return true;
}
int set_registered_kernel_attributes(int* failed_lds_bytes) {
    for (const KernelLdsEntry& e : kernel_lds_table())
        if (const hipError_t rc = hipFuncSetAttribute(e.host_fn, hipFuncAttributeMaxDynamicSharedMemorySize, e.lds_bytes)) {
            *failed_lds_bytes = e.lds_bytes;
            return (int)rc;
        }
    return 0;
}
}

extern "C" {

const char* swiftly_hip_build_id(void) { return SWF_SRC_HASH; }

void swiftly_hip_chain_chunk_streams(int chain) { g_chain_chunk_streams = chain ? 1 : 0; }

int swiftly_hip_set_column_precision(swiftly_hip_t* h, int bits) {
    if (!h) return fail(SWIFTLY_ERR_PARAM, "null argument");
    if (bits != 32 && bits != 64) return fail(SWIFTLY_ERR_PARAM, "column precision must be 32 or 64");
    h->col_f64 = bits == 64;
    return 0;
}
int swiftly_hip_get_column_precision(const swiftly_hip_t* h) { return h ? (h->col_f64 ? 64 : 32) : -1; }

int swiftly_hip_supports(int feature, int dtype, int64_t N, int64_t yN_size, int64_t xM_size, int64_t n_facets) {
    std::string why = check_sizes(N, yN_size, xM_size);
    if (why.empty()) {
        const Sizes s = make_sizes(N, yN_size, xM_size);
        switch (feature) {
            case SWIFTLY_FEATURE_FUSED_SUBGRID: why = why_not_fused_subgrid(s, dtype, n_facets); break;
            case SWIFTLY_FEATURE_BAND_PIPELINE: why = why_not_band_pipeline(s, dtype, n_facets, false); break;
            case SWIFTLY_FEATURE_BAND_PIPELINE_EXPLICIT: why = why_not_band_pipeline(s, dtype, n_facets, true); break;
            case SWIFTLY_FEATURE_BACKWARD_BAND: why = why_not_backward_band(s, dtype); break;
            case SWIFTLY_FEATURE_SPLIT_BAND: why = why_not_split_band(s); break;
            case SWIFTLY_FEATURE_WINDOW_ROWS: why = why_not_window_rows(s); break;
            case SWIFTLY_FEATURE_BACKWARD_BAND_EXPLICIT: why = why_not_backward_band(s, dtype, true); break;
            case SWIFTLY_FEATURE_SPLIT_PREPARE: why = why_not_split_prepare(s, dtype, n_facets); break;
            default: why = reason("unknown feature %d", feature);
        }
    }
    if (why.empty()) return 1;
    fail(SWIFTLY_ERR_UNSUPPORTED, "%s", why.c_str());
    return 0;
}
int64_t swiftly_hip_limit(int which) {
    switch (which) {
        case SWIFTLY_LIMIT_FUSED_FACETS: return kSumFinishMaxFacets;
        case SWIFTLY_LIMIT_WINDOW_ROWS_STAGE_COLUMNS: return row_pass_whole_stage_columns();
        case SWIFTLY_LIMIT_WINDOW_ROWS_WINDOWS: return kWholeMaxWindows;
        default: return -1;
    }
}
int swiftly_hip_mixed_factor(int64_t n, int* Q, int* log2_rest) {
    int q = 0, l = 0;
    if (!mixed_factor(n, &q, &l)) return 0;
    if (Q) *Q = q;
    if (log2_rest) *log2_rest = l;
    return 1;
}

int swiftly_hip_debug_row_band_occupancy(void) { return swf::row_pass_band_occupancy(); }

int swiftly_hip_debug_occupancy(int lds_bytes) { return swf::row_pass_half_occupancy(lds_bytes); }

int swiftly_hip_malloc(void** ptr, size_t bytes) {
    if (!ptr) return fail(SWIFTLY_ERR_PARAM, "null argument");
    HIP_TRY(hipMalloc(ptr, bytes));
    return 0;
}
int swiftly_hip_free(void* ptr) {
    HIP_TRY(hipFree(ptr));
    return 0;
}
int swiftly_hip_memset_async(void* ptr, int value, size_t bytes, void* stream) {
    HIP_TRY(hipMemsetAsync(ptr, value, bytes, (hipStream_t)stream));
    return 0;
}
int swiftly_hip_memcpy_h2d(void* dst, const void* src, size_t bytes, void* stream) {
    HIP_TRY(hipMemcpyAsync(dst, src, bytes, hipMemcpyHostToDevice, (hipStream_t)stream));
    return 0;
}
int swiftly_hip_memcpy_d2h(void* dst, const void* src, size_t bytes, void* stream) {
    HIP_TRY(hipMemcpyAsync(dst, src, bytes, hipMemcpyDeviceToHost, (hipStream_t)stream));
    return 0;
}
int swiftly_hip_stream_synchronize(void* stream) {
    HIP_TRY(hipStreamSynchronize((hipStream_t)stream));
    return 0;
}

int swiftly_hip_stream_create_cu_mask(void** stream, const uint32_t* cu_mask, int nwords) {
    if (!stream || !cu_mask || nwords <= 0) return fail(SWIFTLY_ERR_PARAM, "null argument");
    hipStream_t st = nullptr;
    HIP_TRY(hipExtStreamCreateWithCUMask(&st, (uint32_t)nwords, cu_mask));
    *stream = (void*)st;
    return 0;
}
int swiftly_hip_stream_destroy(void* stream) {
    HIP_TRY(hipStreamDestroy((hipStream_t)stream));
    return 0;
}
int swiftly_hip_cu_census(int32_t* out, int nblocks, void* stream) {
    if (!out || nblocks <= 0) return fail(SWIFTLY_ERR_PARAM, "null argument");
    hipLaunchKernelGGL(cu_census_kernel, dim3((unsigned)nblocks), dim3(64), 0, (hipStream_t)stream, out);
    HIP_TRY(hipGetLastError());
    return 0;
}
int swiftly_hip_kernel_table(int64_t* count, int64_t* max_lds_bytes) {
    if (!count || !max_lds_bytes) return fail(SWIFTLY_ERR_PARAM, "null argument");
    *count = 0;
    *max_lds_bytes = 0;
    for (const KernelLdsEntry& e : kernel_lds_table()) {
        ++*count;
        *max_lds_bytes = std::max<int64_t>(*max_lds_bytes, e.lds_bytes);
    }
    return 0;
}

}
```

ska-sdp-distributed-fourier-transform_amd/csrc/swiftly_caps.h:

```cpp
#pragma once

#include <cstdarg>
#include <cstdint>
#include <cstdio>
#include <string>

#include "../../include/swiftly_hip.h"

namespace swf {

static inline int ilog2_exact(int64_t n) {
    if (n <= 0 || (n & (n - 1))) return -1;
    int l = 0;
    while ((int64_t(1) << l) < n) l++;
    return l;
}

constexpr int kMinLogN = 3;
constexpr int kMaxLogNFloat = 15;

constexpr int kSumFinishMaxFacets = 64;
constexpr int kWholeMaxWindows = 256;

bool col_pass_f64_supported(int logn);
int row_pass_whole_stage_columns();

#define SF_PAIRS(X) X(7, 8) X(7, 10) X(8, 9) X(8, 10) X(9, 10) X(9, 11) X(10, 11) X(10, 12)
#define SF_PAIRS_C128(X) X(7, 8) X(7, 10) X(8, 9) X(8, 10) X(9, 10)
#define SPLIT_PAIRS_C128(X) X(7, 8) X(7, 10) X(8, 9) X(8, 10) X(9, 10)

#define SF_HAS(M, XX) \
    if (logm == M && logx == XX) return true;
inline bool sum_finish_supported(int logm, int logx) {
    SF_PAIRS(SF_HAS)
    return false;
}
inline bool sum_finish_c128_supported(int logm, int logx) {
    SF_PAIRS_C128(SF_HAS)
    return false;
}
inline bool split_prepare_c128_supported(int logm, int logx) {
    SPLIT_PAIRS_C128(SF_HAS)
    return false;
}
#undef SF_HAS
#define SF_NAME(M, XX) s += (s.empty() ? "(" : ", (") + std::to_string(1 << M) + ", " + std::to_string(1 << XX) + ")";
inline std::string sum_finish_c128_sizes() {
    std::string s;
    SF_PAIRS_C128(SF_NAME)
    return s;
}
inline std::string split_prepare_c128_sizes() {
    std::string s;
    SPLIT_PAIRS_C128(SF_NAME)
    return s;
}
#undef SF_NAME

inline bool mixed_factor(int64_t n, int* Q, int* logM) {
    if (n <= 0) return false;
    for (int q : {3, 5, 7, 9}) {
        if (n % q) continue;
        const int l = ilog2_exact(n / q);
        if (l >= kMinLogN) {
            *Q = q;
            *logM = l;
            return true;
        }
    }
    return false;
}

struct Sizes {
    int64_t N = 0, yN = 0, xM = 0, m = 0;
    int log_yN = -1, log_xM = -1, log_m = -1;
};

inline std::string reason(const char* fmt, ...) {
    char buf[512];
    va_list ap;
    va_start(ap, fmt);
    vsnprintf(buf, sizeof buf, fmt, ap);
    va_end(ap);
    return buf;
}
inline std::string check_sizes(int64_t N, int64_t yN, int64_t xM) {
    if (N <= 0 || yN <= 0 || xM <= 0) return "sizes must be positive";
    if (N % yN != 0) return reason("Image size %lld not divisible by facet size %lld!", (long long)N, (long long)yN);
    if (N % xM != 0) return reason("Image size %lld not divisible by subgrid size %lld!", (long long)N, (long long)xM);
    if ((xM * yN) % N != 0)
        return reason("Contribution size not integer with image size %lld, subgrid size %lld and facet size %lld!", (long long)N,
                      (long long)xM, (long long)yN);
    return {};
}
inline Sizes make_sizes(int64_t N, int64_t yN, int64_t xM) {
    Sizes s;
    s.N = N; s.yN = yN; s.xM = xM; s.m = xM * yN / N;
    s.log_yN = ilog2_exact(yN); s.log_xM = ilog2_exact(xM); s.log_m = ilog2_exact(s.m);
    return s;
}

constexpr int kBandMinLog = 6;
constexpr int kBandMaxLogYN = kMaxLogNFloat + 1;
constexpr int kBandMaxLogYNC128 = 15;
constexpr int kBandMixedMaxLog = kMaxLogNFloat;
constexpr int kFusedMaxLogM = 10;
constexpr int kBackwardBandMinLogYN = kBandMinLog;
constexpr int kBackwardBandMaxLogYN = kMaxLogNFloat + 1;
constexpr int kSplitBandMinLogYN = 14;
constexpr int kSplitBandMaxLogYN = 16;
constexpr int kPlacedMaxLogXM = 11;
constexpr int kWindowRowsLogYN = 15, kWindowRowsLogM = 9;

inline bool band_is_split(const Sizes* s) { return s->log_yN >= kSplitBandMinLogYN && s->log_yN <= kSplitBandMaxLogYN; }
inline bool band_pipeline_c128_supported(const Sizes* s) {
    return s->log_yN >= kBandMinLog && s->log_yN <= kBandMaxLogYNC128 && col_pass_f64_supported(s->log_m) &&
           sum_finish_c128_supported(s->log_m, s->log_xM);
}

inline bool band_yN_supported(const Sizes& s, int lo, int hi) {
    int Q = 0, k = 0;
    if (s.log_yN >= 0) return s.log_yN >= lo && s.log_yN <= hi;
    return mixed_factor(s.yN, &Q, &k) && k >= kBandMinLog && k <= kBandMixedMaxLog;
}

inline std::string too_many_facets(int64_t n_facets) {
    if (n_facets <= kSumFinishMaxFacets) return {};
    return reason("the fused subgrid side sums at most %d facets in one kernel, got %lld", kSumFinishMaxFacets, (long long)n_facets);
}
inline std::string why_not_fused_subgrid(const Sizes& s, int dtype, int64_t n_facets) {
    if (s.log_m < 0 || s.log_xM < 0)
        return reason("fused subgrid side: m %lld and xM %lld must be powers of two", (long long)s.m, (long long)s.xM);
    if (dtype != SWIFTLY_C64) return "fused subgrid side: complex64 only (complex128: the band pipeline, when asked for explicitly)";
    if (std::string why = too_many_facets(n_facets); !why.empty()) return why;
    if (s.log_m > kFusedMaxLogM || !sum_finish_supported(s.log_m, s.log_xM))
        return reason("fused subgrid side: no sum_finish instance for m %lld, xM %lld", (long long)s.m, (long long)s.xM);
    return {};
}
inline std::string why_not_split_prepare(const Sizes& s, int dtype, int64_t n_facets) {
    if (dtype != SWIFTLY_C128) return why_not_fused_subgrid(s, dtype, n_facets);
    if (s.log_m < 0 || s.log_xM < 0)
        return reason("split_prepare_facets: m %lld and xM %lld must be powers of two", (long long)s.m, (long long)s.xM);
    if (std::string why = too_many_facets(n_facets); !why.empty()) return why;
    if (!split_prepare_c128_supported(s.log_m, s.log_xM) || !col_pass_f64_supported(s.log_m))
        return reason("split_prepare_facets: complex128 instances exist for (m, xM) = %s; got (%lld, %lld)",
                      split_prepare_c128_sizes().c_str(), (long long)s.m, (long long)s.xM);
    return {};
}
inline std::string why_not_band_pipeline(const Sizes& s, int dtype, int64_t n_facets, bool explicit_) {
    if (dtype == SWIFTLY_C128) {
        if (!explicit_) return "complex128 band pipeline: runs only when asked for explicitly";
        if (s.log_yN < 0 || s.log_xM < 0 || s.log_m < 0)
            return reason("complex128 band pipeline: yN %lld, xM %lld and m %lld must be powers of two", (long long)s.yN,
                          (long long)s.xM, (long long)s.m);
        if (std::string why = too_many_facets(n_facets); !why.empty()) return why;
        if (!band_pipeline_c128_supported(&s) || s.log_m < kBandMinLog)
            return reason("complex128 band pipeline: needs yN %d .. %d and an instance for (m, xM) = %s; got yN %lld, m %lld, xM %lld",
                          1 << kBandMinLog, 1 << kBandMaxLogYNC128, sum_finish_c128_sizes().c_str(), (long long)s.yN,
                          (long long)s.m, (long long)s.xM);
        return {};
    }
    if (std::string why = why_not_fused_subgrid(s, dtype, n_facets); !why.empty()) return why;
    if (s.log_m < kBandMinLog || !band_yN_supported(s, kBandMinLog, kBandMaxLogYN))
        return reason("band pipeline: needs m >= %d and yN a power of two %d .. %d or Q * 2^k (Q = 3, 5, 7, 9; 2^k %d .. %d); "
                      "got m %lld, yN %lld", 1 << kBandMinLog, 1 << kBandMinLog, 1 << kBandMaxLogYN, 1 << kBandMinLog,
                      1 << kBandMixedMaxLog, (long long)s.m, (long long)s.yN);
    return {};
}
inline std::string why_not_backward_band(const Sizes& s, int dtype, bool explicit_ = false) {
    if (dtype == SWIFTLY_C128 && explicit_) {
        if (s.log_xM < 0 || s.log_m < 0 || s.log_yN < kBackwardBandMinLogYN || s.log_yN > kBandMaxLogYNC128)
            return reason("complex128 backward band: needs xM and m powers of two and yN a power of two %d .. %d (no Q * 2^k: "
                          "there is no float64 radix-Q gather-sum pass); got xM %lld, m %lld, yN %lld",
                          1 << kBackwardBandMinLogYN, 1 << kBandMaxLogYNC128, (long long)s.xM, (long long)s.m, (long long)s.yN);
        return {};
    }
    if (dtype != SWIFTLY_C64) return "backward band: complex64 only (complex128: when asked for explicitly)";
    if (s.log_xM < 0 || s.log_m < 0 || !band_yN_supported(s, kBackwardBandMinLogYN, kBackwardBandMaxLogYN))
        return reason("backward band: needs xM and m powers of two and yN a power of two %d .. %d or Q * 2^k (Q = 3, 5, 7, 9; "
                      "2^k %d .. %d); got xM %lld, m %lld, yN %lld", 1 << kBackwardBandMinLogYN, 1 << kBackwardBandMaxLogYN,
                      1 << kBandMinLog, 1 << kBandMixedMaxLog, (long long)s.xM, (long long)s.m, (long long)s.yN);
    return {};
}
inline std::string why_not_split_band(const Sizes& s) {
    if (band_is_split(&s)) return {};
    return reason("yN %lld keeps the whole padded axis in the plain band layout (split: %d .. %d)", (long long)s.yN,
                  1 << kSplitBandMinLogYN, 1 << kSplitBandMaxLogYN);
}
inline std::string why_not_window_rows(const Sizes& s) {
    if (s.log_yN == kWindowRowsLogYN && s.log_m == kWindowRowsLogM && s.xM <= (int64_t(1) << kPlacedMaxLogXM)) return {};
    return reason("window rows: needs yN %d, m %d and xM <= %d; got yN %lld, m %lld, xM %lld", 1 << kWindowRowsLogYN,
                  1 << kWindowRowsLogM, 1 << kPlacedMaxLogXM, (long long)s.yN, (long long)s.m, (long long)s.xM);
}

}
```

ska-sdp-distributed-fourier-transform_amd/csrc/swiftly_colpass.h:

```cpp
#pragma once
#include "swiftly_caps.h"
#include "swiftly_fft.h"

namespace swf {

template <bool NT>
__device__ __forceinline__ cx<float> cp_load(const cx<float>* p) {
    if constexpr (NT) {
        const f32x2 v = __builtin_nontemporal_load(reinterpret_cast<const f32x2*>(p));
        return {v.x, v.y};
    } else {
        return *p;
    }
}
template <bool NT>
__device__ __forceinline__ void cp_store(cx<float>* p, cx<float> v) {
    if constexpr (NT) {
        const f32x2 w = {v.x, v.y};
        __builtin_nontemporal_store(w, reinterpret_cast<f32x2*>(p));
    } else {
        *p = v;
    }
}

// ... 261 lines not shown
                    if (A.ld_rowmap) idx = A.ld_rowmap[ok ? idx : 0];
                }
                in_row = ok ? idx : -1;
            }
            const int qs = ok ? q : 0;
            if (ld_win) in_w *= win_at(ld_win, qs);
            if (ld_win2) in_w *= win_at(ld_win2, qs);
        }
    }
    int out_row;
    RC out_w = (RC)A.scale;
    cx<RC> out_tw = {(RC)1, (RC)0};
    {
        const int u = slot >> LR, r = slot & ((1 << LR) - 1);
        const int j = t + u * T;
        const int k = j & ((1 << LNS) - 1);
        const int e = ((j - k) << LR) + k + (r << LNS);
        if constexpr (RAW_ST) {
            out_row = o * A.out_o_rows + e * A.out_i_rows;
            out_tw = tw_full[((unsigned)e * (unsigned)o) & (unsigned)(FS - 1)];
        } else {
            int pk = e * A.st_mul + o;
            if (A.st_qmul > 0) pk = pk * A.st_qmul + A.st_qadd;
            const int ck = wrapn(pk + (FN >> 1));
            const int d = wrapn(ck + st_a);
            int idx = d + A.st_c;
            if (idx >= A.st_mod) idx -= A.st_mod;
            const bool ok = d < A.st_len;
            const int ds = ok ? d : 0;
            if (st_win) out_w *= win_at(st_win, (long long)z * A.st_win_bs + ds);
            if (st_win2) out_w *= win_at(st_win2, ds);
            int row = idx;
            if (st_rowmap) row = st_rowmap[(long long)zb * A.st_rowmap_bs + (ok ? idx : 0)];
            out_row = ok ? row : -1;
        }
    }

    cx<RC> x[P];
    if constexpr (PW) {
        if (straddle) {
            static_for<0, P>([&](auto vI) {
                constexpr int v = decltype(vI)::value;
                const int row_a = slot_bcast<HALF>(in_row, v, hw), row_b = slot_bcast<HALF>(in_row_b, v, hw);
                const int row = from_b ? row_b : row_a;
                cx<ST> val = {(ST)0, (ST)0};
                if (row >= 0 && live) val = cp_load<NT_LD>(in + (unsigned)row * A.in_pitch);
                x[v] = cx<RC>{(RC)val.x, (RC)val.y};
            });
        }
    }
    if (!straddle) static_for<0, P>([&](auto vI) {
        constexpr int v = decltype(vI)::value;
        const int row = slot_bcast<HALF>(in_row, v, hw);
        cx<ST> val = {(ST)0, (ST)0};
        if constexpr (GS) {
            const int lo1 = slot_bcast<HALF>((int)gs_off1, v, hw), hi1 = slot_bcast<HALF>((int)(gs_off1 >> 32), v, hw);
            if (hi1 >= 0) {
                const long long o1 = ((long long)hi1 << 32) | (unsigned)lo1;
                if (live) val = cp_load<NT_LD>(in + o1);
            }
            const int lo2 = slot_bcast<HALF>((int)gs_off2, v, hw), hi2 = slot_bcast<HALF>((int)(gs_off2 >> 32), v, hw);
            if (hi2 >= 0) {
                const long long o2 = ((long long)hi2 << 32) | (unsigned)lo2;
                if (live) {
                    const cx<ST> w2 = cp_load<NT_LD>(in + o2);
                    if constexpr (sizeof(RC) == 8) {
                        x[v] = cx<RC>{(RC)val.x + (RC)w2.x, (RC)val.y + (RC)w2.y};
                        return;
                    }
                    val.x += w2.x;
                    val.y += w2.y;
                }
            }
        } else {
            if (row >= 0) {
                if (live) val = cp_load<NT_LD>(in + (unsigned)row * A.in_pitch);
            }
        }
        x[v] = cx<RC>{(RC)val.x, (RC)val.y};
    });
    static_for<0, P>([&](auto vI) {
        constexpr int v = decltype(vI)::value;
        if constexpr (!RAW_LD) {
            const RC w = slot_bcast_f<HALF>(in_w, v, hw);
            x[v].x *= w;
            x[v].y *= w * sg_ld;
        } else {
            x[v].y *= sg_ld;
        }
    });

    fft_phases<G, RC, 0>(x, t, clane, true, smem, tw, [&](int, cx<RC> v, auto sI) {
        constexpr int s = decltype(sI)::value;
        const int row = slot_bcast<HALF>(out_row, s, hw);
        if (row < 0) return;
        if constexpr (RAW_ST) {
            cx<RC> w;
            w.x = slot_bcast_f<HALF>(out_tw.x, s, hw);
            w.y = slot_bcast_f<HALF>(out_tw.y, s, hw);
            v = cmul(v, w);
            v.y *= sg_st;
            if (live) cp_store<NT_ST>(out + (unsigned)row * A.out_pitch, cx<ST>{(ST)v.x, (ST)v.y});
        } else {
            const RC w = slot_bcast_f<HALF>(out_w, s, hw) * col_w;
            v.x *= w;
            v.y *= w * sg_st;
            cx<ST>* p = out + (unsigned)row * A.out_pitch;
            if (A.accumulate) {
                if (live && rmw) {
                    const cx<ST> old = *p;
                    v.x += (RC)old.x;
                    v.y += (RC)old.y;
                }
            }
            if (live) cp_store<NT_ST>(p, cx<ST>{(ST)v.x, (ST)v.y});
        }
    });
}

template <class G, int MODE, bool SNT, bool GS = false, typename RC = float, typename ST = float>
__global__ __launch_bounds__(G::NT, G::MINW) void col_pass_kernel(const ColPassArgs A, const cx<ST>* __restrict__ gin,
                                                         cx<ST>* __restrict__ gout,
                                                         const float* __restrict__ ld_win,
                                                         const float* __restrict__ ld_win2,
                                                         const float* __restrict__ st_win,
                                                         const float* __restrict__ st_win2,
                                                         const int* __restrict__ st_rowmap,
                                                         const cx<RC>* __restrict__ tw,
                                                         const cx<RC>* __restrict__ tw_full, const ColZ cz) {
    extern __shared__ __attribute__((aligned(16))) unsigned char smem[];
    col_pass_body<G, MODE, SNT, GS, ColZ, RC, ST>(A, gin, gout, ld_win, ld_win2, st_win, st_win2, st_rowmap, tw, tw_full, cz,
                                    __builtin_amdgcn_readfirstlane(threadIdx.x >> 6), threadIdx.x & 63, blockIdx.x,
                                    blockIdx.y, blockIdx.z + A.z0, smem);
}

template <class G, typename RC = float>
__global__ __launch_bounds__(G::NT, G::MINW) void col_pass2_kernel(const ColPassArgs A, const ColPassSrc2 S2,
                                                          const cx<float>* __restrict__ gin,
                                                          cx<float>* __restrict__ gout,
                                                          const float* __restrict__ ld_win,
                                                          const float* __restrict__ ld_win2,
                                                          const float* __restrict__ st_win,
                                                          const float* __restrict__ st_win2,
                                                          const int* __restrict__ st_rowmap,
                                                          const cx<RC>* __restrict__ tw,
                                                          const cx<RC>* __restrict__ tw_full, const ColZ cz) {
    extern __shared__ __attribute__((aligned(16))) unsigned char smem[];
    col_pass_body<G, 2, true, false, ColZ, RC, float, true>(A, gin, gout, ld_win, ld_win2, st_win, st_win2, st_rowmap, tw,
                                                            tw_full, cz, __builtin_amdgcn_readfirstlane(threadIdx.x >> 6),
                                                            threadIdx.x & 63, blockIdx.x, blockIdx.y, blockIdx.z + A.z0, smem,
                                                            &S2);
}

constexpr int kColPassMinLog = 2;
constexpr int kColPassMaxLog = 10;

int launch_col_pass(int logn, int mode, const ColPassArgs& a, const ColZ& cz, int outer, int nbatch, hipStream_t s,
                    const ColPassSrc2* src2 = nullptr);
bool col_pass_pieces_supported(int logn, const ColPassArgs& a);

}
```

ska-sdp-distributed-fourier-transform_amd/csrc/swiftly_geometry.h:

```cpp
#pragma once

#include <cstdint>

#include "swiftly_caps.h"

namespace swf {

static inline int64_t floordiv(int64_t a, int64_t b) {
    int64_t q = a / b;
    if ((a % b != 0) && ((a < 0) != (b < 0))) q--;
    return q;
}
static inline int pmod(int64_t a, int64_t n) {
    int64_t r = a % n;
    if (r < 0) r += n;
    return (int)r;
}

struct Map {
    int a, len, c, mod;
};
inline Map whole(int64_t n) { return Map{0, (int)n, 0, (int)n}; }

inline int facet_lo(const Sizes& z, int64_t yB) { return (int)z.yN / 2 - (int)(yB / 2); }
inline Map facet_in_padded_facet(const Sizes& z, int64_t yB, int64_t facet_off) {
    return Map{pmod(-(facet_off + facet_lo(z, yB)), z.yN), (int)yB, 0, (int)yB};
}

inline int64_t facet_shift(const Sizes& z, int64_t facet_off) { return floordiv(facet_off * z.xM, z.N); }
inline int placement_start(const Sizes& z, int64_t sp) { return pmod((int)z.xM / 2 - (int)z.m / 2 + sp, z.xM); }
inline Map contribution_in_padded_subgrid(const Sizes& z, int64_t facet_off) {
    const int64_t sp = facet_shift(z, facet_off);
    return Map{pmod(-sp, z.m), (int)z.m, placement_start(z, sp), (int)z.xM};
}

inline Map subgrid_in_padded_subgrid(const Sizes& z, int64_t xA, int64_t subgrid_off) {
    return Map{pmod(-((int)z.xM / 2 - (int)xA / 2 + subgrid_off), z.xM), (int)xA, 0, (int)xA};
}

inline bool band_valid(int64_t yN, int64_t band_start, int64_t band_len) {
    return band_len > 0 && band_len <= yN && band_start >= 0 && band_start < yN;
}
inline Map band_as_load_map(const Sizes& z, int64_t band_start, int64_t band_len) {
    return Map{pmod(-band_start, z.yN), (int)band_len, 0, (int)band_len};
}

struct Window {
    int64_t s;
    int rot, base;
};
inline Window window_of(const Sizes& z, int64_t subgrid_off) {
    const int64_t s = floordiv(subgrid_off * z.yN, z.N);
    return Window{s, pmod(-s, z.m), pmod((int)z.yN / 2 - (int)z.m / 2 + s, z.yN)};
}
inline int window_column(const Sizes& z, const Window& w, int64_t q) {
    const int col = w.base + (int)((q + w.rot) % z.m);
    return col >= z.yN ? col - (int)z.yN : col;
}
inline int64_t window_in_band(const Sizes& z, const Window& w, int64_t first, int64_t count, int64_t band_start,
                              int64_t band_len) {
    for (int64_t q = first; q < first + count; q++) {
        int d = window_column(z, w, q) - (int)band_start;
        if (d < 0) d += (int)z.yN;
        if (d >= band_len) return q;
    }
    return -1;
}

inline bool offsets_fit_32(uint64_t count, uint64_t stride, uint64_t extra = 0) {
    return count * stride + extra < (uint64_t(1) << 32);
}

}
```

ska-sdp-distributed-fourier-transform_amd/csrc/swiftly_sumfinish.h:

```cpp
#pragma once
#include "swiftly_caps.h"
#include "swiftly_fft.h"

namespace swf {

constexpr int kSumFinishThreads = 256;
constexpr int kSumFinishInFlight = 3;
constexpr int kSumFinishMaxGroups = 8;
constexpr int kSumFinishMaxBatch = 64;
#ifndef SWF_SUMFINISH_COMPACT
#define SWF_SUMFINISH_COMPACT 1
#endif
template <class G>
using SFCompact = std::conditional_t<SWF_SUMFINISH_COMPACT != 0, CompactTw<G>, G>;

struct SumFinishArgs {
    const cx<float>* in;
    cx<float>* out;
    long long in_gs, in_bs, in_rs;
    long long out_bs, out_rs;
    int nrows;
    int ngroups, xA;
    int sp[kSumFinishMaxGroups];
    int st_a[kSumFinishMaxBatch];
    const float* fn;
    const float* mask;
    long long mask_bs;
    const cx<float>* tw_m;
    const cx<float>* tw_x;
};

template <int LOGM, int LOGX, typename R = float>
struct SFGeo {
    static constexpr int LOGTR = LOGX >= 12 ? 8 : 6;
    static constexpr int TR = 1 << LOGTR;
    static constexpr int NT = LOGX >= 12 ? 256 : (LOGX == 11 ? 64 : kSumFinishThreads);
    using GM = Geo<R, LOGM, LOGM - LOGTR, NT, false>;
    using GX = Geo<R, LOGX, LOGX - LOGTR, NT, false>;
    static_assert(LOGM - LOGTR >= 1, "at least two points per lane");
    static_assert(GM::T == TR && GX::T == TR, "TR threads per row");
    static constexpr int RB = NT / TR;
    static constexpr size_t LDS_M = (size_t)RB * GM::PITCH * 2 * sizeof(R);
    static constexpr size_t LDS_X = (size_t)RB * GX::PITCH * 2 * sizeof(R);
    static constexpr size_t LDS_BYTES = LDS_M + LDS_X;
};

template <int LOGM, int LOGX>
struct SFWide {
    using S = SFGeo<LOGM, LOGX>;
    static constexpr bool ON = LOGX >= 12 && LOGM >= 7;
    using GM = Geo<float, LOGM, (LOGM >= 7 ? LOGM - 6 : 1), S::NT, false>;
    static constexpr size_t LDS_M = GM::LDS_BYTES;
    static constexpr size_t LDS_BYTES = LDS_M + S::LDS_X;
};
template <int LOGM, int LOGX>
constexpr size_t sum_finish_facets_lds() {
    return SFWide<LOGM, LOGX>::ON ? SFWide<LOGM, LOGX>::LDS_BYTES : SFGeo<LOGM, LOGX>::LDS_BYTES;
}
template <int LOGM, int LOGX, typename R = float>
constexpr size_t sum_finish_facets_reg_lds() {
    using S = SFGeo<LOGM, LOGX, R>;
    return (S::LDS_X > S::LDS_M ? S::LDS_X : S::LDS_M) + (sizeof(R) << LOGM);
}
template <int LOGM, int LOGX, typename R = float>
constexpr size_t sum_finish_facets_kernel_lds() {
    return SFWide<LOGM, LOGX>::ON ? SFWide<LOGM, LOGX>::LDS_BYTES : sum_finish_facets_reg_lds<LOGM, LOGX, R>();
}

template <int LOGM, int LOGX>
__global__ __launch_bounds__((SFGeo<LOGM, LOGX>::NT)) void sum_finish_rows_kernel(const SumFinishArgs A) {
    using S = SFGeo<LOGM, LOGX>;
    using GM = typename S::GM;
    using GX = typename S::GX;
    extern __shared__ __attribute__((aligned(16))) unsigned char smem[];
    cx<float>* ex_m = reinterpret_cast<cx<float>*>(smem);
    cx<float>* acc = reinterpret_cast<cx<float>*>(smem + S::LDS_M);
    constexpr int M = GM::N, X = GX::N, PM = GM::P, PX = GX::P, TR = S::TR;
    const int t = threadIdx.x % TR, rb = threadIdx.x / TR;
    const int b = blockIdx.y;
    const int row = blockIdx.x * S::RB + rb;
    const bool live = row < A.nrows;
    const int rrow = live ? row : 0;

    static_for<0, PX>([&](auto vI) {
        constexpr int v = decltype(vI)::value;
        acc[lds_pos<GX>(rb, t + v * TR, false)] = cx<float>{0.f, 0.f};
    });
    row_sync<GX>(false);

    for (int g = 0; g < A.ngroups; g++) {
        const cx<float>* __restrict__ in = A.in + (long long)g * A.in_gs + (long long)b * A.in_bs + (long long)rrow * A.in_rs;
        cx<float> x[PM];
        static_for<0, PM>([&](auto vI) {
            constexpr int v = decltype(vI)::value;
            x[v] = in[(t + v * TR) ^ (M >> 1)];
        });
        const int sp = A.sp[g];
        fft_phases<GM, float, 0>(x, t, rb, false, ex_m, A.tw_m, [&](int e, cx<float> v) {
            const int ck = e ^ (M >> 1);
            const int k = (ck - sp) & (M - 1);
            const int dest = (k + (X >> 1) - (M >> 1) + sp) & (X - 1);
            const float w = A.fn[k];
            cx<float>* p = acc + lds_pos<GX>(rb, dest ^ (X >> 1), false);
            cx<float> o = *p;
            o.x += v.x * w;
            o.y += v.y * w;
            *p = o;
        });
        row_sync<GX>(false);
    }

    cx<float> y[PX];
    static_for<0, PX>([&](auto vI) {
        constexpr int v = decltype(vI)::value;
        cx<float> val = acc[lds_pos<GX>(rb, t + v * TR, false)];
        val.y = -val.y;
        y[v] = val;
    });
    row_sync<GX>(false);
    cx<float>* __restrict__ out = A.out + (long long)b * A.out_bs + (long long)rrow * A.out_rs;
    const float* __restrict__ mask = A.mask ? A.mask + (long long)b * A.mask_bs : nullptr;
    const int st_a = A.st_a[b];
    const float scale = 1.f / (float)X;
    fft_phases<GX, float, 0>(y, t, rb, false, acc, A.tw_x, [&](int e, cx<float> v) {
        const int ck = e ^ (X >> 1);
        const int d = (ck + st_a) & (X - 1);
        if (d < A.xA && live) {
            float w = scale;
            if (mask) w *= mask[d];
            out[d] = cx<float>{v.x * w, -v.y * w};
        }
    });
}

struct SumFinishFacetArgs {
    const cx<float>* in;
    cx<float>* out;
    long long in_fs, in_bs, in_rs;
    long long out_bs, out_rs;
    int nrows;
    int nfacets, xA;
    int ngroups;
    int gstart[kSumFinishMaxFacets + 1];
    int fidx[kSumFinishMaxFacets];
    int base0[kSumFinishMaxFacets];
    int gsp1[kSumFinishMaxFacets];
    int st_a[kSumFinishMaxBatch];
    const float* fn;
    const float* mask;
    long long mask_bs;
    const cx<float>* tw_m;
    const cx<float>* tw_x;
    const cx<float>* twc_m;
    const cx<float>* twc_x;
    int nrounds;
    int rstart[kSumFinishMaxFacets + 1];
    int rgroup[kSumFinishMaxFacets];
    int placed;
};

template <int LOGM, int LOGX, typename R = float>
__global__ __launch_bounds__((SFGeo<LOGM, LOGX, R>::NT), (!std::is_same_v<R, float> ? 2 : LOGX <= 10 ? 4 : 1)) void sum_finish_facets_kernel(const SumFinishFacetArgs A) {
    using S = SFGeo<LOGM, LOGX, R>;
    using GX = typename S::GX;
    using W = SFWide<LOGM, LOGX>;
    using GM = std::conditional_t<W::ON, typename W::GM, typename S::GM>;
    static_assert(std::is_same_v<R, float> || !W::ON, "complex128: register form only");
    constexpr bool F32 = std::is_same_v<R, float>;
    using GMC = std::conditional_t<F32, SFCompact<GM>, GM>;
    using GXC = std::conditional_t<F32, SFCompact<GX>, GX>;
    const cx<R>* g_in = reinterpret_cast<const cx<R>*>(A.in);
    cx<R>* g_out = reinterpret_cast<cx<R>*>(A.out);
    const R* g_fn = reinterpret_cast<const R*>(A.fn);
    const R* g_mask = reinterpret_cast<const R*>(A.mask);
    const cx<R>* tw_m = reinterpret_cast<const cx<R>*>(A.tw_m);
    const cx<R>* tw_x = reinterpret_cast<const cx<R>*>(A.tw_x);
    const cx<R>* twc_m = F32 ? reinterpret_cast<const cx<R>*>(A.twc_m) : nullptr;
    const cx<R>* twc_x = F32 ? reinterpret_cast<const cx<R>*>(A.twc_x) : nullptr;
    extern __shared__ __attribute__((aligned(16))) unsigned char smem[];
    cx<R>* ex_m = reinterpret_cast<cx<R>*>(smem);
    cx<R>* acc = reinterpret_cast<cx<R>*>(smem + (W::ON ? W::LDS_M : 0));
    constexpr int M = GM::N, X = GX::N, PM = GM::P, PX = GX::P, TR = S::TR;
    const int t = threadIdx.x % TR, rb = threadIdx.x / TR;
    const int b = blockIdx.y;
    const int row0 = blockIdx.x * S::RB;
    const int row = row0 + rb;
    const bool live = row < A.nrows;
    cx<R> y[PX];

    if constexpr (W::ON) {
        static_for<0, PX>([&](auto vI) {
            constexpr int v = decltype(vI)::value;
            acc[lds_pos<GX>(rb, t + v * TR, false)] = cx<R>{(R)0, (R)0};
        });
        row_sync<GX>(false);
    }

    if constexpr (W::ON) {
        static_assert(S::RB == 1, "one row per workgroup");
        constexpr int NBW = 2;
        const int lane = threadIdx.x & 63;
        const int wv = __builtin_amdgcn_readfirstlane(threadIdx.x >> 6);
        constexpr int NW = S::NT / 64;
        for (int r = 0; r < A.nrounds; r++) {
            for (int i0 = A.rstart[r]; i0 < A.rstart[r + 1]; i0 += NW) {
                const int i = i0 + wv;
                if (i < A.rstart[r + 1]) {
                    const int g = A.rgroup[i];
                    cx<R> xs[PM];
                    static_for<0, PM>([&](auto vI) { xs[decltype(vI)::value] = cx<R>{(R)0, (R)0}; });
                    bool anyg = false;
                    int n = A.gstart[g];
                    const int ne = A.gstart[g + 1];
                    while (n < ne) {
                        int fs[NBW];
                        int cnt = 0;
                        for (; n < ne && cnt < NBW; n++) {
                            const bool any = live && ((row - A.base0[n]) & (X - 1)) < M;
                            if (any) fs[cnt++] = n;
                        }
                        if (cnt == 0) break;
                        anyg = true;
                        cx<R> x[NBW][PM];
                        static_for<0, NBW>([&](auto sI) {
                            constexpr int sl = decltype(sI)::value;
                            if (sl < cnt) {
                                const int nn = fs[sl];
                                const int k = (row - A.base0[nn]) & (X - 1);
                                const cx<R>* __restrict__ in = g_in + (long long)A.fidx[nn] * A.in_fs +
                                                                   (long long)b * A.in_bs + (long long)(live ? k : 0) * A.in_rs;
                                static_for<0, PM>([&](auto vI) {
                                    constexpr int v = decltype(vI)::value;
                                    x[sl][v] = in[(lane + v * 64) ^ (M >> 1)];
                                });
                            }
                        });
                        const R lw = live ? (R)1 : (R)0;
                        static_for<0, NBW>([&](auto sI) {
                            constexpr int sl = decltype(sI)::value;
                            if (sl < cnt) {
                                static_for<0, PM>([&](auto vI) {
                                    constexpr int v = decltype(vI)::value;
                                    xs[v].x += x[sl][v].x * lw;
                                    xs[v].y += x[sl][v].y * lw;
                                });
                            }
                        });
                    }
                    if (anyg) {
                        const int sp = A.gsp1[g];
                        fft_phases<GMC, R, 0>(xs, lane, wv, false, ex_m, tw_m, [&](int e, cx<R> v) {
                            const int ck = e ^ (M >> 1);
                            const int kk = (ck - sp) & (M - 1);
                            const int dest = (kk + (X >> 1) - (M >> 1) + sp) & (X - 1);
                            const R w = g_fn[kk];
                            cx<R>* p = acc + lds_pos<GX>(0, dest ^ (X >> 1), false);
                            cx<R> o = *p;
                            o.x += v.x * w;
                            o.y += v.y * w;
                            *p = o;
                        }, nullptr, twc_m);
                    }
                }
            }
            __syncthreads();
        }
    } else {

    static_assert(S::LDS_X >= S::LDS_M, "one exchange buffer per row, sized by the longer transform");
    constexpr int RATIO = X / M;
    static_assert(PX == PM * RATIO, "accumulator slots");
    cx<R>* ex_row = reinterpret_cast<cx<R>*>(smem) + (size_t)rb * GX::PITCH;
    R* fn_l = reinterpret_cast<R*>(smem + (S::LDS_X > S::LDS_M ? S::LDS_X : S::LDS_M));
    for (int i = threadIdx.x; i < M; i += S::NT) fn_l[i] = g_fn[i];
    static_for<0, PX>([&](auto vI) { y[decltype(vI)::value] = cx<R>{(R)0, (R)0}; });
    __syncthreads();
    constexpr int NB = (PM >= 8 && LOGX <= 10 && kSumFinishInFlight > 2) ? 2 : kSumFinishInFlight;
    for (int g = 0; g < A.ngroups; g++) {
        cx<R> xs[PM];
        static_for<0, PM>([&](auto vI) { xs[decltype(vI)::value] = cx<R>{(R)0, (R)0}; });
        bool anyg = false;
        int n = A.gstart[g];
        const int ne = A.gstart[g + 1];
        while (n < ne) {
            int fs[NB];
            int cnt = 0;
            for (; n < ne && cnt < NB; n++) {
                const int base = A.base0[n];
                bool any = false;
                for (int q = 0; q < S::RB; q++) any = any || (((row0 + q - base) & (X - 1)) < M && row0 + q < A.nrows);
                if (any) fs[cnt++] = n;
            }
            if (cnt == 0) break;
            anyg = true;
            cx<R> x[NB][PM];
            R wgt[NB];
            static_for<0, NB>([&](auto sI) {
                constexpr int sl = decltype(sI)::value;
                if (sl < cnt) {
                    const int nn = fs[sl];
                    const int k = (row - A.base0[nn]) & (X - 1);
                    const bool on = live && k < M;
                    const cx<R>* __restrict__ in =
                        g_in + (long long)A.fidx[nn] * A.in_fs + (long long)b * A.in_bs + (long long)(on ? k : 0) * A.in_rs;
                    wgt[sl] = on ? (R)1 : (R)0;
                    const int rot = A.placed ? A.gsp1[g] : 0;
                    static_for<0, PM>([&](auto vI) {
                        constexpr int v = decltype(vI)::value;
                        x[sl][v] = in[(((t + v * TR) ^ (M >> 1)) - rot) & (M - 1)];
                    });
                }
            });
            static_for<0, NB>([&](auto sI) {
                constexpr int sl = decltype(sI)::value;
                if (sl < cnt) {
                    static_for<0, PM>([&](auto vI) {
                        constexpr int v = decltype(vI)::value;
                        xs[v].x += x[sl][v].x * wgt[sl];
                        xs[v].y += x[sl][v].y * wgt[sl];
                    });
                }
            });
        }
        if (!anyg) continue;
        const int sp = A.gsp1[g];
        if (A.placed) {
            static_for<0, PM>([&](auto vI) {
                constexpr int v = decltype(vI)::value;
                const int ck = (t + v * TR) ^ (M >> 1);
                const int kk = (ck - sp) & (M - 1);
                const int p = (kk - (M >> 1) + sp) & (X - 1);
                const int c = p >> LOGM;
                static_for<0, RATIO>([&](auto cI) {
                    constexpr int cc = decltype(cI)::value;
                    const R wc = c == cc ? (R)1 : (R)0;
                    y[v + PM * cc].x += xs[v].x * wc;
                    y[v + PM * cc].y += xs[v].y * wc;
                });
            });
            continue;
        }
        fft_phases<GMC, R, 0>(xs, t, 0, false, ex_row, tw_m, [&](int e, cx<R> v, auto sI) {
            constexpr int LR = GM::LOGN % GM::LOGP == 0 ? GM::LOGP : GM::LOGN % GM::LOGP, RAD = 1 << LR, NBL = PM / RAD;
            constexpr int slot = (decltype(sI)::value / RAD) + NBL * (decltype(sI)::value % RAD);
            const int ck = e ^ (M >> 1);
            const int kk = (ck - sp) & (M - 1);
            const int p = (kk - (M >> 1) + sp) & (X - 1);
            const int c = p >> LOGM;
            const R w = fn_l[kk];
            static_for<0, RATIO>([&](auto cI) {
                constexpr int cc = decltype(cI)::value;
                const R wc = c == cc ? w : (R)0;
                y[slot + PM * cc].x += v.x * wc;
                y[slot + PM * cc].y += v.y * wc;
            });
        }, nullptr, twc_m);
        row_sync<GX>(false);
    }
    static_for<0, PX>([&](auto vI) { y[decltype(vI)::value].y = -y[decltype(vI)::value].y; });
    acc = ex_row - (size_t)rb * GX::PITCH;

    }

    if constexpr (W::ON) {
        static_for<0, PX>([&](auto vI) {
            constexpr int v = decltype(vI)::value;
            cx<R> val = acc[lds_pos<GX>(rb, t + v * TR, false)];
            val.y = -val.y;
            y[v] = val;
        });
        row_sync<GX>(false);
    }
    cx<R>* __restrict__ out = g_out + (long long)b * A.out_bs + (long long)(live ? row : 0) * A.out_rs;
    const R* __restrict__ mask = A.mask ? g_mask + (long long)b * A.mask_bs : nullptr;
    const int st_a = A.st_a[b];
    const R scale = (R)1 / (R)X;
    if constexpr (!W::ON) {
        constexpr int LRX = GX::LOGN % GX::LOGP == 0 ? GX::LOGP : GX::LOGN % GX::LOGP, RADX = 1 << LRX, NBX = PX / RADX;
        R mw[PX];
        static_for<0, PX>([&](auto sI) {
            constexpr int sl = decltype(sI)::value;
            constexpr int vi = (sl / RADX) + NBX * (sl % RADX);
            const int d = (((t + TR * vi) ^ (X >> 1)) + st_a) & (X - 1);
            const bool ok = d < A.xA && live;
            mw[sl] = mask ? mask[ok ? d : 0] : (R)1;
        });
        fft_phases<GXC, R, 0>(y, t, rb, false, acc, tw_x, [&](int e, cx<R> v, auto sI) {
            constexpr int sl = decltype(sI)::value;
            const int ck = e ^ (X >> 1);
            const int d = (ck + st_a) & (X - 1);
            const R w = scale * mw[sl];
            if (d < A.xA && live) out[d] = cx<R>{v.x * w, -v.y * w};
        }, nullptr, twc_x);
        return;
    }
    fft_phases<GXC, R, 0>(y, t, rb, false, acc, tw_x, [&](int e, cx<R> v) {
        const int ck = e ^ (X >> 1);
        const int d = (ck + st_a) & (X - 1);
        if (d < A.xA && live) {
            R w = scale;
            if (mask) w *= mask[d];
            out[d] = cx<R>{v.x * w, -v.y * w};
        }
    }, nullptr, twc_x);
}

struct Axis1RowsArgs {
    const cx<float>* in;
    cx<float>* out;
    long long in_fs, in_rs, out_fs, out_rs;
    int nrows, yN;
    int band_start, band_len, band_half;
    int c0;
    int s;
    int sp[kSumFinishMaxFacets];
    const float* fn;
    const cx<float>* tw_m;
    const cx<float>* twc_m;
};
constexpr int kAxis1Threads = 256;
template <int LOGM>
struct Axis1Geo {
    using GM = Geo<float, LOGM, LOGM - 6, kAxis1Threads, false>;
    static constexpr size_t LDS_BYTES = GM::LDS_BYTES;
};
template <int LOGM>
__global__ __launch_bounds__(kAxis1Threads) void axis1_rows_kernel(const Axis1RowsArgs A) {
    using GM = typename Axis1Geo<LOGM>::GM;
    extern __shared__ __attribute__((aligned(16))) unsigned char smem[];
    cx<float>* ex = reinterpret_cast<cx<float>*>(smem);
    constexpr int M = GM::N, PM = GM::P, TR = 64;
    const int t = threadIdx.x & 63, rb = threadIdx.x >> 6;
    const int f = blockIdx.y;
    const int row = blockIdx.x * GM::RB + rb;
    const bool live = row < A.nrows;
    const cx<float>* __restrict__ in = A.in + (long long)f * A.in_fs + (long long)(live ? row : 0) * A.in_rs;
// ... 31 lines not shown
    int ngroups;
    int gstart[kSumFinishMaxFacets + 1];
    int fidx[kSumFinishMaxFacets];
    int base0[kSumFinishMaxFacets];
    int gsp1[kSumFinishMaxFacets];
    int ld_a[kSumFinishMaxBatch];
    const float* fn;
    const cx<float>* tw_m;
    const cx<float>* tw_x;
    const cx<float>* twc_m;
    const cx<float>* twc_x;
};

template <int LOGM, int LOGX, typename R = float>
__global__ __launch_bounds__((SFGeo<LOGM, LOGX, R>::NT)) void split_prepare_facets_kernel(const SplitFacetArgs A) {
    using S = SFGeo<LOGM, LOGX, R>;
    using GX = typename S::GX;
    using W = SFWide<LOGM, LOGX>;
    using GM = std::conditional_t<W::ON, typename W::GM, typename S::GM>;
    constexpr bool F32 = std::is_same_v<R, float>;
    static_assert(F32 || !W::ON, "complex128: one transform per row group only");
    using GMC = std::conditional_t<F32, SFCompact<GM>, GM>;
    using GXC = std::conditional_t<F32, SFCompact<GX>, GX>;
    const cx<R>* g_in = reinterpret_cast<const cx<R>*>(A.in);
    cx<R>* g_out = reinterpret_cast<cx<R>*>(A.out);
    const R* g_fn = reinterpret_cast<const R*>(A.fn);
    const cx<R>* tw_m = reinterpret_cast<const cx<R>*>(A.tw_m);
    const cx<R>* tw_x = reinterpret_cast<const cx<R>*>(A.tw_x);
    const cx<R>* twc_m = F32 ? reinterpret_cast<const cx<R>*>(A.twc_m) : nullptr;
    const cx<R>* twc_x = F32 ? reinterpret_cast<const cx<R>*>(A.twc_x) : nullptr;
    extern __shared__ __attribute__((aligned(16))) unsigned char smem[];
    cx<R>* ex_m = reinterpret_cast<cx<R>*>(smem);
    cx<R>* acc = reinterpret_cast<cx<R>*>(smem + (W::ON ? W::LDS_M : S::LDS_M));
    constexpr int M = GM::N, X = GX::N, PM = GM::P, PX = GX::P, TR = S::TR;
    const int t = threadIdx.x % TR, rb = threadIdx.x / TR;
    const int b = blockIdx.y;
    const int row0 = blockIdx.x * S::RB;
    const int row = row0 + rb;
    const bool live = row < A.nrows;

    {
        const cx<R>* __restrict__ in = g_in + (long long)b * A.in_bs + (long long)(live ? row : 0) * A.in_rs;
        const int lda = A.ld_a[b];
        cx<R> y[PX];
        static_for<0, PX>([&](auto vI) {
            constexpr int v = decltype(vI)::value;
            const int q = (((t + v * TR) ^ (X >> 1)) + lda) & (X - 1);
            const bool ok = live && q < A.xA;
            const cx<R> val = in[ok ? q : 0];
            y[v] = ok ? val : cx<R>{(R)0, (R)0};
        });
        fft_phases<GXC, R, 0>(y, t, rb, false, acc, tw_x, [&](int e, cx<R> v) {
            acc[lds_pos<GX>(rb, e ^ (X >> 1), false)] = v;
        }, nullptr, twc_x);
        row_sync<GX>(false);
    }
    const R scale = (R)1 / (R)M;
    constexpr int NS = 4;
    if constexpr (W::ON) {
        static_assert(S::RB == 1, "one row per workgroup");
        const int lane = threadIdx.x & 63;
        const int wv = __builtin_amdgcn_readfirstlane(threadIdx.x >> 6);
        constexpr int NW = S::NT / 64;
        for (int g = wv; g < A.ngroups; g += NW) {
            int n = A.gstart[g];
            const int ne = A.gstart[g + 1];
            const int sp = A.gsp1[g];
            const int c1 = ((X >> 1) - (M >> 1) + sp) & (X - 1);
            while (n < ne) {
                cx<R>* outp[NS];
                int cnt = 0;
                static_for<0, NS>([&](auto sI) {
                    constexpr int sl = decltype(sI)::value;
                    outp[sl] = nullptr;
                    for (; n < ne && cnt == sl; n++) {
                        const int k = (row - A.base0[n]) & (X - 1);
                        if (live && k < M) {
                            outp[sl] = g_out + (long long)A.fidx[n] * A.out_fs + (long long)b * A.out_bs + (long long)k * A.out_rs;
                            cnt++;
                        }
                    }
                });
                if (cnt == 0) break;
                cx<R> x[PM];
                static_for<0, PM>([&](auto vI) {
                    constexpr int v = decltype(vI)::value;
                    const int q = (((lane + v * 64) ^ (M >> 1)) - sp) & (M - 1);
                    const cx<R> val = acc[lds_pos<GX>(0, (q + c1) & (X - 1), false)];
                    const R w = g_fn[q];
                    x[v] = cx<R>{val.x * w, -val.y * w};
                });
                fft_phases<GMC, R, 0>(x, lane, wv, false, ex_m, tw_m, [&](int e, cx<R> v) {
                    const cx<R> o = cx<R>{v.x * scale, -v.y * scale};
                    static_for<0, NS>([&](auto sI) {
                        constexpr int sl = decltype(sI)::value;
                        if (outp[sl]) outp[sl][e ^ (M >> 1)] = o;
                    });
                }, nullptr, twc_m);
                __builtin_amdgcn_wave_barrier();
            }
        }
        return;
    }
    for (int g = 0; g < A.ngroups; g++) {
        int n = A.gstart[g];
        const int ne = A.gstart[g + 1];
        const int sp = A.gsp1[g];
        const int c1 = ((X >> 1) - (M >> 1) + sp) & (X - 1);
        while (n < ne) {
            int fs[NS];
            int cnt = 0;
            for (; n < ne && cnt < NS; n++) {
                const int base = A.base0[n];
                bool any = false;
                for (int q = 0; q < S::RB; q++) any = any || (((row0 + q - base) & (X - 1)) < M && row0 + q < A.nrows);
                if (any) fs[cnt++] = n;
            }
            if (cnt == 0) break;
            cx<R>* outp[NS];
            static_for<0, NS>([&](auto sI) {
                constexpr int sl = decltype(sI)::value;
                outp[sl] = nullptr;
                if (sl < cnt) {
                    const int nn = fs[sl];
                    const int k = (row - A.base0[nn]) & (X - 1);
                    if (live && k < M)
                        outp[sl] = g_out + (long long)A.fidx[nn] * A.out_fs + (long long)b * A.out_bs + (long long)k * A.out_rs;
                }
            });
            cx<R> x[PM];
            static_for<0, PM>([&](auto vI) {
                constexpr int v = decltype(vI)::value;
                const int q = (((t + v * TR) ^ (M >> 1)) - sp) & (M - 1);
                const cx<R> val = acc[lds_pos<GX>(rb, (q + c1) & (X - 1), false)];
                const R w = g_fn[q];
                x[v] = cx<R>{val.x * w, -val.y * w};
            });
            fft_phases<GMC, R, 0>(x, t, rb, false, ex_m, tw_m, [&](int e, cx<R> v) {
                const cx<R> o = cx<R>{v.x * scale, -v.y * scale};
                static_for<0, NS>([&](auto sI) {
                    constexpr int sl = decltype(sI)::value;
                    if (outp[sl]) outp[sl][e ^ (M >> 1)] = o;
                });
            }, nullptr, twc_m);
            row_sync<GX>(false);
        }
    }
}

int launch_split_prepare_facets(int logm, int logx, const SplitFacetArgs& a, int nbatch, hipStream_t s);
int launch_split_prepare_facets_c128(int logm, int logx, const SplitFacetArgs& a, int nbatch, hipStream_t s);
int launch_sum_finish_facets(int logm, int logx, const SumFinishFacetArgs& a, int nbatch, hipStream_t s);
int launch_sum_finish_facets_c128(int logm, int logx, const SumFinishFacetArgs& a, int nbatch, hipStream_t s);
int launch_sum_finish_rows(int logm, int logx, const SumFinishArgs& a, int nbatch, hipStream_t s);
int launch_axis1_rows(int logm, const Axis1RowsArgs& a, int nfacets, hipStream_t s);

}
```

ska-sdp-distributed-fourier-transform_amd/ska_sdp_exec_swiftly_amd/_lib.py:

```python
import ctypes
import os
from ctypes import POINTER, c_char_p, c_double, c_int, c_int64, c_size_t, c_void_p

_HERE = os.path.dirname(os.path.abspath(__file__))
LIB_PATH = os.path.join(_HERE, os.environ.get("SWIFTLY_HIP_LIB", "libswiftly_hip.so"))

C64, C128 = 0, 1
ERR_PARAM, ERR_UNSUPPORTED, ERR_HIP = 1, 2, 3
(FEATURE_FUSED_SUBGRID, FEATURE_BAND_PIPELINE, FEATURE_BAND_PIPELINE_EXPLICIT, FEATURE_BACKWARD_BAND, FEATURE_SPLIT_BAND,
 FEATURE_WINDOW_ROWS, FEATURE_BACKWARD_BAND_EXPLICIT, FEATURE_SPLIT_PREPARE) = range(8)
LIMIT_FUSED_FACETS, LIMIT_WINDOW_ROWS_STAGE_COLUMNS, LIMIT_WINDOW_ROWS_WINDOWS = range(3)

_lib = None


class SwiftlyHipError(RuntimeError):
    """HIP runtime / launch failure reported by libswiftly_hip.so"""


def _declare(lib):
    i64, vp = c_int64, c_void_p
    lib.swiftly_hip_last_error.restype = c_char_p
    lib.swiftly_hip_last_error.argtypes = []
    lib.swiftly_hip_version.restype = c_int
    lib.swiftly_hip_device_count.restype = c_int
    lib.swiftly_hip_create.restype = c_int
    lib.swiftly_hip_create.argtypes = [POINTER(vp), i64, i64, i64, c_double, POINTER(c_double), c_int]
    lib.swiftly_hip_destroy.restype = None
    lib.swiftly_hip_destroy.argtypes = [vp]
    lib.swiftly_hip_contribution_size.restype = i64
    lib.swiftly_hip_contribution_size.argtypes = [vp]
    lib.swiftly_hip_supports_dtype.restype = c_int
    lib.swiftly_hip_supports_dtype.argtypes = [vp, c_int]
    lib.swiftly_hip_supports.restype = c_int
    lib.swiftly_hip_supports.argtypes = [c_int, c_int, i64, i64, i64, i64]
    lib.swiftly_hip_limit.restype = i64
    lib.swiftly_hip_limit.argtypes = [c_int]
    lib.swiftly_hip_mixed_factor.restype = c_int
    lib.swiftly_hip_mixed_factor.argtypes = [i64, POINTER(c_int), POINTER(c_int)]
    lib.swiftly_hip_build_id.restype = ctypes.c_char_p
    lib.swiftly_hip_build_id.argtypes = []
    lib.swiftly_hip_k3_one_launch.restype = c_int
    lib.swiftly_hip_k3_one_launch.argtypes = [c_int]
    lib.swiftly_hip_chain_chunk_streams.restype = None
    lib.swiftly_hip_chain_chunk_streams.argtypes = [ctypes.c_int]
    lib.swiftly_hip_set_column_precision.restype = ctypes.c_int
    lib.swiftly_hip_set_column_precision.argtypes = [vp, ctypes.c_int]
    lib.swiftly_hip_get_column_precision.restype = ctypes.c_int
    lib.swiftly_hip_get_column_precision.argtypes = [vp]
    sized_in = [vp, c_int, vp, i64, i64, i64, i64, vp, i64, i64, i64, vp]
    plain = [vp, c_int, vp, i64, i64, i64, vp, i64, i64, i64, vp]
    finish = [vp, c_int, vp, i64, i64, i64, vp, i64, i64, i64, i64, vp, vp]
    for name, args in [
        ("prepare_facet", sized_in),
        ("extract_from_facet", plain),
        ("add_to_subgrid", plain),
        ("finish_subgrid", finish),
        ("prepare_subgrid", sized_in),
        ("extract_from_subgrid", plain),
        ("add_to_facet", plain),
        ("finish_facet", finish),
    ]:
        fn = getattr(lib, "swiftly_hip_" + name)
        fn.restype = c_int
        fn.argtypes = args
    lib.swiftly_hip_add_to_subgrid_2d.restype = c_int
    lib.swiftly_hip_add_to_subgrid_2d.argtypes = [vp, c_int, vp, i64, i64, vp, i64, i64, i64, i64, vp]
    lib.swiftly_hip_prepare_subgrid_inplace.restype = c_int
    lib.swiftly_hip_prepare_subgrid_inplace.argtypes = [vp, c_int, vp, i64, i64, i64, i64, vp]
    lib.swiftly_hip_prepare_subgrid_inplace_2d.restype = c_int
    lib.swiftly_hip_prepare_subgrid_inplace_2d.argtypes = [vp, c_int, vp, i64, i64, i64, i64, vp]
    pi64 = POINTER(i64)
    batch = [i64, i64, i64, pi64]
    for name, args in [
        ("extract_column", [vp, c_int, vp, i64, i64, i64, vp, i64, i64, i64, i64, vp]),
        ("extract_column_rows", [vp, c_int, vp, i64, i64, i64, vp, i64, i64, i64, i64, vp, c_int, vp]),
        ("prepare_facet_rows", sized_in[:-1] + [vp, c_int, vp]),
        ("extract_from_facet_batch", plain[:-1] + batch + [vp]),
        ("add_to_subgrid_batch", plain[:-1] + batch + [vp]),
        ("finish_subgrid_batch", finish[:-1] + batch + [i64, vp]),
        ("prepare_subgrid_batch", sized_in[:-1] + batch + [vp]),
        ("extract_from_subgrid_batch", plain[:-1] + batch + [vp]),
        ("add_to_facet_batch", plain[:-1] + batch + [vp]),
        ("finish_facet_batch", finish[:-1] + batch + [i64, vp]),
    ]:
        fn = getattr(lib, "swiftly_hip_" + name)
        fn.restype = c_int
        fn.argtypes = args
    lib.swiftly_hip_sum_finish_rows.restype = c_int
    lib.swiftly_hip_sum_finish_rows.argtypes = [vp, c_int, vp, i64, i64, i64, i64, pi64, vp, i64, i64, pi64, i64, vp, i64, i64, vp]
    lib.swiftly_hip_add_to_subgrid_from_columns.restype = c_int
    lib.swiftly_hip_add_to_subgrid_from_columns.argtypes = [vp, c_int, vp, i64, i64, i64, vp, i64, i64, i64, i64, pi64, vp]
    lib.swiftly_hip_band_columns.restype = i64
    lib.swiftly_hip_band_columns.argtypes = [i64]
    lib.swiftly_hip_band_columns_for.restype = i64
    lib.swiftly_hip_band_columns_for.argtypes = [vp, i64]
    lib.swiftly_hip_prepare_facet_band.restype = c_int
    lib.swiftly_hip_prepare_facet_band.argtypes = [vp, c_int, vp, i64, i64, i64, vp, i64, i64, i64, i64, c_int, vp]
    lib.swiftly_hip_prepare_facet_band_rows.restype = c_int
    lib.swiftly_hip_prepare_facet_band_rows.argtypes = [vp, c_int, vp, i64, i64, i64, vp, i64, i64, i64, i64, i64, i64, vp]
    lib.swiftly_hip_prepare_facet_columns.restype = c_int
    lib.swiftly_hip_prepare_facet_columns.argtypes = [vp, c_int, vp, i64, i64, i64, i64, pi64, i64, i64, i64, vp, i64, i64, vp, vp]
    lib.swiftly_hip_transform_contributions.restype = c_int
    lib.swiftly_hip_transform_contributions.argtypes = [
        vp, c_int, vp, c_int, i64, i64, i64, vp, i64, i64, i64, pi64, i64, pi64, vp, i64, i64, vp,
    ]
    lib.swiftly_hip_sum_finish_facets.restype = c_int
    lib.swiftly_hip_sum_finish_facets.argtypes = [
        vp, c_int, vp, i64, i64, i64, i64, pi64, pi64, vp, i64, i64, pi64, i64, vp, i64, i64, vp,
    ]
    lib.swiftly_hip_wave_facet_side.restype = c_int
    lib.swiftly_hip_wave_facet_side.argtypes = [
        vp, c_int, vp, i64, i64, i64, i64, pi64, i64, i64, i64, vp, i64, vp, i64, c_int, i64, pi64, vp, i64, i64, pi64, pi64,
        vp, i64, vp,
    ]
    lib.swiftly_hip_prepare_facet_columns_waves.restype = c_int
    lib.swiftly_hip_prepare_facet_columns_waves.argtypes = [
        vp, c_int, vp, i64, i64, i64, i64, pi64, i64, i64, i64, pi64, vp, i64, i64, i64, vp, i64, vp, i64, vp,
    ]
    lib.swiftly_hip_prepare_facet_columns_range.restype = c_int
    lib.swiftly_hip_prepare_facet_columns_range.argtypes = [
        vp, c_int, vp, i64, i64, i64, i64, pi64, i64, i64, i64, i64, i64, vp, i64, i64, vp, vp, i64, vp,
    ]
    lib.swiftly_hip_transform_contributions_pieces.restype = c_int
    lib.swiftly_hip_transform_contributions_pieces.argtypes = [
        vp, c_int, i64, POINTER(vp), pi64, POINTER(vp), pi64, pi64, pi64, i64, pi64, i64, pi64, vp, i64, i64, pi64, pi64, vp,
    ]
    lib.swiftly_hip_wave_subgrid_side.restype = c_int
    lib.swiftly_hip_wave_subgrid_side.argtypes = [
        vp, c_int, vp, i64, i64, i64, pi64, pi64, i64, pi64, pi64, i64, vp, i64, vp, i64, vp, vp, vp, i64, vp,
    ]
    lib.swiftly_hip_wave_subgrid_side_placed.restype = c_int
    lib.swiftly_hip_wave_subgrid_side_placed.argtypes = list(lib.swiftly_hip_wave_subgrid_side.argtypes)
    lib.swiftly_hip_prepare_facet_window_rows.restype = c_int
    lib.swiftly_hip_prepare_facet_window_rows.argtypes = [
        vp, c_int, vp, i64, i64, i64, vp, i64, i64, i64, i64, i64, i64, vp, i64, i64, vp,
    ]
    lib.swiftly_hip_finish_axis1_rows.restype = c_int
    lib.swiftly_hip_finish_axis1_rows.argtypes = [vp, c_int, vp, i64, i64, i64, i64, pi64, i64, i64, i64, vp, i64, i64, vp]
    lib.swiftly_hip_accumulate_facet_columns.restype = c_int
    lib.swiftly_hip_accumulate_facet_columns.argtypes = [
        vp, c_int, vp, i64, i64, pi64, pi64, vp, i64, pi64, i64, vp, i64, vp, i64, i64, i64, i64, vp, vp, i64, vp,
    ]
    lib.swiftly_hip_split_prepare_facets.restype = c_int
    lib.swiftly_hip_split_prepare_facets.argtypes = [vp, c_int, vp, i64, i64, i64, i64, pi64, i64, pi64, pi64, vp, i64, i64, vp]
    lib.swiftly_hip_wave_split_subgrids.restype = c_int
    lib.swiftly_hip_wave_split_subgrids.argtypes = [vp, c_int, vp, i64, i64, pi64, pi64, i64, pi64, pi64, vp, i64, vp, i64, i64, vp]
    lib.swiftly_hip_band_zero_untouched.restype = c_int
    lib.swiftly_hip_band_zero_untouched.argtypes = [vp, c_int, vp, i64, i64, i64, vp, vp]
    lib.swiftly_hip_finish_facet_band.restype = c_int
    lib.swiftly_hip_finish_facet_band.argtypes = [vp, c_int, vp, i64, i64, i64, i64, vp, i64, i64, i64, vp, vp]
    src = [c_int, vp, i64, i64, i64]
    for name, args in [
        ("subgrids_from_sources", src + [pi64, pi64, i64, vp, vp, vp, i64, i64, vp]),
        ("check_subgrids_from_sources", src + [pi64, pi64, i64, vp, vp, vp, i64, i64, vp, vp]),
        ("facet_from_sources", src + [i64, i64, vp, vp, vp, i64, vp]),
        ("check_facet_from_sources", src + [i64, i64, vp, vp, vp, i64, vp, vp, vp, vp]),
    ]:
        fn = getattr(lib, "swiftly_hip_" + name)
        fn.restype = c_int
        fn.argtypes = args
    lib.swiftly_hip_malloc.restype = c_int
    lib.swiftly_hip_malloc.argtypes = [POINTER(vp), c_size_t]
    lib.swiftly_hip_free.restype = c_int
    lib.swiftly_hip_free.argtypes = [vp]
    lib.swiftly_hip_memset_async.restype = c_int
    lib.swiftly_hip_memset_async.argtypes = [vp, c_int, c_size_t, vp]
    for name in ("swiftly_hip_memcpy_h2d", "swiftly_hip_memcpy_d2h"):
        fn = getattr(lib, name)
        fn.restype = c_int
        fn.argtypes = [vp, vp, c_size_t, vp]
    lib.swiftly_hip_stream_synchronize.restype = c_int
    lib.swiftly_hip_stream_synchronize.argtypes = [vp]
    lib.swiftly_hip_stream_create_cu_mask.restype = c_int
    lib.swiftly_hip_stream_create_cu_mask.argtypes = [POINTER(vp), POINTER(ctypes.c_uint32), c_int]
    lib.swiftly_hip_stream_destroy.restype = c_int
    lib.swiftly_hip_stream_destroy.argtypes = [vp]
    lib.swiftly_hip_cu_census.restype = c_int
    lib.swiftly_hip_cu_census.argtypes = [vp, c_int, vp]
    lib.swiftly_hip_kernel_table.restype = c_int
    lib.swiftly_hip_kernel_table.argtypes = [POINTER(ctypes.c_int64), POINTER(ctypes.c_int64)]


def load():
    global _lib
    if _lib is not None:
        return _lib
    if not os.path.exists(LIB_PATH):
        raise ImportError(
            f"{LIB_PATH} is missing: build it with `python -c 'import __graft_entry__ as g; g.build()'` "
            "or `make -C ska-sdp-distributed-fourier-transform_amd/csrc`. "
            "The HIP backend has no CPU fallback."
        )
    import torch

    lib = ctypes.CDLL(LIB_PATH, mode=ctypes.RTLD_GLOBAL)
    _declare(lib)
    _lib = lib
    return lib


def check(rc):
    if rc == 0:
        return
    msg = last_error()
    if rc == ERR_PARAM:
        raise ValueError(msg)
    if rc == ERR_UNSUPPORTED:
        raise NotImplementedError(msg)
    raise SwiftlyHipError(msg)


def last_error():
    return load().swiftly_hip_last_error().decode("utf-8", "replace")


def build_info():
    import hashlib

    lib = load()
    with open(LIB_PATH, "rb") as fh:
        sha = hashlib.sha256(fh.read()).hexdigest()
    head = None
    try:
        with open(os.path.join(os.path.dirname(_HERE), "csrc", "build", "GIT_HEAD"), encoding="utf-8") as fh:
            head = "".join(fh.read().split())
    except OSError:
        pass
    return dict(src_hash=lib.swiftly_hip_build_id().decode(), so_sha256=sha[:16], git_head=head, library=os.path.basename(LIB_PATH))
```

ska-sdp-distributed-fourier-transform_amd/ska_sdp_exec_swiftly_amd/core_hip.py:

```python
import ctypes
import functools

import numpy
import scipy.special

from . import _lib

__all__ = ["SwiftlyCoreHip", "calculate_pswf"]


def calculate_pswf(W, yN_size):
    half = yN_size // 2
    hi = half if yN_size % 2 == 0 else half + 1
    xs = 2.0 * numpy.arange(-half, hi, dtype=float) / yN_size
    vals = numpy.empty(yN_size, dtype=float)
    for start in range(1, yN_size, 500):
        stop = start + 500
        vals[start:stop] = scipy.special.pro_ang1(0, 0, numpy.pi * W / 2, xs[start:stop])[0]
    vals[0] = 0.0
    return vals


def band_range(N, yN, m, subgrid_offs, align=32):
    return _band_range_cached(int(N), int(yN), int(m), tuple(sorted(set(int(o) for o in subgrid_offs))), int(align))
# ... 400 lines not shown
    def MAX_FUSED_FACETS(self):
        return int(_lib.load().swiftly_hip_limit(_lib.LIMIT_FUSED_FACETS))

    def supports_fused_subgrid(self, dtype=None, n_facets=None):
        return self._supports(_lib.FEATURE_FUSED_SUBGRID, dtype, n_facets)

    def supports_band_pipeline(self, dtype=None, n_facets=None, explicit=False):
        feature = _lib.FEATURE_BAND_PIPELINE_EXPLICIT if explicit else _lib.FEATURE_BAND_PIPELINE
        return self._supports(feature, dtype, n_facets)

    def supports_backward_band(self, dtype=None, explicit=False):
        feature = _lib.FEATURE_BACKWARD_BAND_EXPLICIT if explicit else _lib.FEATURE_BACKWARD_BAND
        return self._supports(feature, dtype)

    def supports_split_prepare(self, dtype=None, n_facets=None):
        return self._supports(_lib.FEATURE_SPLIT_PREPARE, dtype, n_facets)

    def band_for_offsets(self, subgrid_offs):
        if not self._supports(_lib.FEATURE_SPLIT_BAND):
            return 0, self.yN_size
        return band_range(self.N, self.yN_size, self.xM_yN_size, subgrid_offs)

    def band_columns(self, band):
        return int(self._lib.swiftly_hip_band_columns_for(self._handle, int(band[1])))

    def prepare_facet_band(self, facet, facet_off, band, out=None, fold_other_axis_window=True, rows_of=None):
        torch = _torch()
        if facet.dim() != 2 or facet.stride(1) != 1:
            raise ValueError("prepare_facet_band needs a row-major 2-D device tensor")
        ncols = self.band_columns(band)
        if out is None:
            out = torch.empty((facet.shape[0], ncols), dtype=facet.dtype, device=self._device)
        elif tuple(out.shape) != (facet.shape[0], ncols) or out.stride(1) != 1:
            raise ValueError(f"Output array has shape {tuple(out.shape)}, expected {(facet.shape[0], ncols)}!")
        if rows_of is not None:
            _lib.check(
                self._lib.swiftly_hip_prepare_facet_band_rows(
                    self._handle, self._code(facet), ctypes.c_void_p(facet.data_ptr()), int(facet.shape[0]),
                    int(facet.shape[1]), facet.stride(0), ctypes.c_void_p(out.data_ptr()), out.stride(0), int(facet_off),
                    int(band[0]), int(band[1]), int(rows_of[0]) if fold_other_axis_window else 0, int(rows_of[1]),
                    self._stream(),
                )
            )
            return out
        _lib.check(
            self._lib.swiftly_hip_prepare_facet_band(
                self._handle, self._code(facet), ctypes.c_void_p(facet.data_ptr()), int(facet.shape[0]),
                int(facet.shape[1]), facet.stride(0), ctypes.c_void_p(out.data_ptr()), out.stride(0), int(facet_off),
                int(band[0]), int(band[1]), int(bool(fold_other_axis_window)), self._stream(),
            )
        )
        return out

    @property
    def WINDOW_ROWS_STAGE_COLUMNS(self):
        return int(_lib.load().swiftly_hip_limit(_lib.LIMIT_WINDOW_ROWS_STAGE_COLUMNS))

    def window_starts(self, band, wave_off1s):
        m, yN = self.xM_yN_size, self.yN_size
        return [((yN // 2 - m // 2 + int(o) * yN // self.N) - int(band[0])) % yN for o in wave_off1s]

    def supports_window_rows(self, band, facet_size, facet_off1s, n_windows=1):
        return (
            0 < int(n_windows) <= int(_lib.load().swiftly_hip_limit(_lib.LIMIT_WINDOW_ROWS_WINDOWS)) and
            self._supports(_lib.FEATURE_WINDOW_ROWS) and
            self.band_columns(band) <= self.WINDOW_ROWS_STAGE_COLUMNS and int(band[1]) < self.yN_size and
            int(facet_size) % 2 == 0 and all(int(o) % 2 == 0 for o in facet_off1s)
        )

    def prepare_facet_window_rows(self, facet, facet_off, band, window_starts, out, fold_other_axis_window=True,
                                  rows_of=None):
        m = self.xM_yN_size
        nwin = int(window_starts.numel())
        if facet.dim() != 2 or facet.stride(1) != 1 or out.stride(-1) != 1:
            raise ValueError("prepare_facet_window_rows needs row-major device tensors")
        if out.dim() == 3 and tuple(out.shape) == (nwin, facet.shape[0], m):
            row_stride, win_stride = out.stride(1), out.stride(0)
        elif out.dim() == 2 and tuple(out.shape) == (facet.shape[0], nwin * m):
            row_stride, win_stride = out.stride(0), m
        else:
            raise ValueError(f"Output array has shape {tuple(out.shape)}, expected {(nwin, facet.shape[0], m)} or "
                             f"{(facet.shape[0], nwin * m)}!")
        size, row0 = rows_of if rows_of is not None else (facet.shape[0], 0)
        cvp = ctypes.c_void_p
        _lib.check(
            self._lib.swiftly_hip_prepare_facet_window_rows(
                self._handle, self._code(facet), cvp(facet.data_ptr()), int(facet.shape[0]), int(facet.shape[1]),
                facet.stride(0), cvp(out.data_ptr()), row_stride, int(facet_off), int(band[0]), int(band[1]),
                int(size) if fold_other_axis_window else 0, int(row0), cvp(window_starts.data_ptr()), nwin, win_stride,
                self._stream(),
            )
        )
        return out

    def prepare_facet_columns(self, bands, facet_off0s, band, subgrid_off1, rowmap=None, n_rows=None, out=None):
        torch = _torch()
        F, yB = bands.shape[0], bands.shape[1]
        m = self.xM_yN_size
        n_rows = self.yN_size if rowmap is None else int(n_rows)
        if out is None:
            out = torch.empty((F, n_rows, m), dtype=bands.dtype, device=self._device)
        scr = self.scratch("k2", self._k2_scratch_bytes(F, bands.element_size()))
        cvp = ctypes.c_void_p
        _lib.check(
            self._lib.swiftly_hip_prepare_facet_columns_waves(
                self._handle, self._code(bands), cvp(bands.data_ptr()), int(yB), bands.stride(1), bands.stride(0), F,
                self._i64(facet_off0s), int(band[0]), int(band[1]), 1, self._i64([subgrid_off1]), cvp(out.data_ptr()),
                out.stride(1), out.stride(0), 0, cvp(rowmap.data_ptr()) if rowmap is not None else None, 0,
                cvp(scr.data_ptr()), scr.numel(), self._stream(),
            )
        )
        self.k2_columns_issued += m
        return out

    k2_columns_issued = 0

    def prepare_facet_columns_range(self, bands, facet_off0s, band, subgrid_off1, col_first, ncols, out, rowmap=None):
        F, yB = bands.shape[0], bands.shape[1]
        if out.dim() != 3 or out.shape[0] != F or out.shape[2] != self.xM_yN_size or out.stride(2) != 1:
            raise ValueError(f"Output array has shape {tuple(out.shape)}, expected ({F}, rows, {self.xM_yN_size})!")
        scr = self.scratch("k2", self._k2_scratch_bytes(F, bands.element_size()))
        cvp = ctypes.c_void_p
        _lib.check(
            self._lib.swiftly_hip_prepare_facet_columns_range(
                self._handle, self._code(bands), cvp(bands.data_ptr()), int(yB), bands.stride(1), bands.stride(0), F,
                self._i64(facet_off0s), int(band[0]), int(band[1]), int(subgrid_off1), int(col_first), int(ncols),
                cvp(out.data_ptr()), out.stride(1), out.stride(0), cvp(rowmap.data_ptr()) if rowmap is not None else None,
                cvp(scr.data_ptr()), scr.numel(), self._stream(),
            )
        )
        self.k2_columns_issued += int(ncols)
        return out

    def transform_contributions_pieces(self, pieces, facet_off0s, sub_off0s, g_out, g_layout=None):
        n = len(pieces)
        F, S = pieces[0][0].shape[0], len(sub_off0s)
        cvp = ctypes.c_void_p
        qs = (cvp * n)(*[pc[0].data_ptr() for pc in pieces])
        maps = (cvp * n)(*[pc[1].data_ptr() if pc[1] is not None else None for pc in pieces])
        if g_layout is None:
            fs, ss, offs, fstr = g_out.stride(0), g_out.stride(1), None, None
        else:
            fs, ss, offs, fstr = 0, 0, self._i64(g_layout[0]), self._i64(g_layout[1])
        _lib.check(
            self._lib.swiftly_hip_transform_contributions_pieces(
                self._handle, self._code(pieces[0][0]), n, qs, self._i64([pc[0].stride(0) for pc in pieces]), maps,
                self._i64([pc[2] for pc in pieces]), self._i64([pc[3] for pc in pieces]),
                self._i64([pc[4] for pc in pieces]), F, self._i64(facet_off0s), S, self._i64(sub_off0s),
                cvp(g_out.data_ptr()), fs, ss, offs, fstr, self._stream(),
            )
        )
        return g_out

    def transform_contributions(self, src, layout, facet_off0s, subgrid_offs, out=None, rowmap=None, band=None, nsub=None):
        torch = _torch()
        F = src.shape[0]
        m = self.xM_yN_size
        S = int(nsub) if layout == 2 else len(subgrid_offs)
        if out is None:
            out = torch.empty((F, S, m, m), dtype=src.dtype, device=self._device)
        foffs = (ctypes.c_int64 * F)(*[int(o) for o in facet_off0s])
        soffs = (ctypes.c_int64 * S)(*[int(o) for o in subgrid_offs]) if layout != 2 else None
        if layout == 2:
            row_stride, facet_stride, sub_stride = src.stride(2), src.stride(0), src.stride(1)
        else:
            row_stride, facet_stride, sub_stride = src.stride(1), src.stride(0), 0
        band = band or (0, 0)
        _lib.check(
            self._lib.swiftly_hip_transform_contributions(
                self._handle, self._code(src), ctypes.c_void_p(src.data_ptr()), int(layout), row_stride, facet_stride,
                sub_stride, ctypes.c_void_p(rowmap.data_ptr()) if rowmap is not None else None, int(band[0]),
                int(band[1]), F, foffs, S, soffs, ctypes.c_void_p(out.data_ptr()), out.stride(0), out.stride(1),
                self._stream(),
            )
        )
        return out

    _I64_CACHE = {}

    @classmethod
    def _i64(cls, values):
        key = tuple(values)
        arr = cls._I64_CACHE.get(key)
        if arr is None:
            if len(cls._I64_CACHE) >= 8192:
                cls._I64_CACHE.clear()
            arr = cls._I64_CACHE[key] = (ctypes.c_int64 * len(key))(*[int(v) for v in key])
        return arr

    def _k2_scratch_bytes(self, F, element_size=8):
        n = F * self.yN_size * self.xM_yN_size * int(element_size)
        return n if mixed_factor(self.yN_size) is None else 2 * n + 4096

    SCRATCH_TAIL_BYTES = 1 << 16

    def scratch(self, name, nbytes):
        torch = _torch()
        pool = self.__dict__.setdefault("_scratch_pool", {})
        key = (name, self._raw_stream())
        nbytes = int(nbytes) + self.SCRATCH_TAIL_BYTES
        buf = pool.get(key)
        if buf is None or buf.numel() < nbytes:
            buf = pool[key] = torch.empty((nbytes,), dtype=torch.uint8, device=self._device)
        return buf

    def wave_facet_side(self, bands, facet_off0s, band, wave_off1, rowmap, n_rows, Q, compute_q, sub_off0s, g_out,
                        g_layout=None):
        F, S = Q.shape[0], len(sub_off0s)
        cvp = ctypes.c_void_p
        scr = self.scratch("k2", self._k2_scratch_bytes(F, Q.element_size())) if compute_q else None
        if g_layout is None:
            fs, ss, offs, fstr = g_out.stride(0), g_out.stride(1), None, None
        else:
            fs, ss, offs, fstr = 0, 0, self._i64(g_layout[0]), self._i64(g_layout[1])
        _lib.check(
            self._lib.swiftly_hip_wave_facet_side(
                self._handle, self._code(Q), cvp(bands.data_ptr()) if bands is not None else None,
                int(bands.shape[1]) if bands is not None else 0, bands.stride(1) if bands is not None else 0,
                bands.stride(0) if bands is not None else 0, F, self._i64(facet_off0s), int(band[0]), int(band[1]),
                int(wave_off1), cvp(rowmap.data_ptr()) if rowmap is not None else None, int(n_rows),
                cvp(Q.data_ptr()), Q.stride(0), int(bool(compute_q)), S, self._i64(sub_off0s), cvp(g_out.data_ptr()), fs,
                ss, offs, fstr, cvp(scr.data_ptr()) if scr is not None else None, scr.numel() if scr is not None else 0,
                self._stream(),
            )
        )
        if compute_q:
            self.k2_columns_issued += self.xM_yN_size

    def chain_chunk_streams(self, chain):
        self._lib.swiftly_hip_chain_chunk_streams(1 if chain else 0)

    def side_stream(self):
        st = self.__dict__.get("_side_stream")
        if st is None:
            st = self.__dict__["_side_stream"] = _torch().cuda.Stream(device=self._device)
        return st

    def stacked_rowmaps(self, key, maps):
        cache = self.__dict__.setdefault("_rowmap_stack_cache", {})
        hit = cache.get(key)
        if hit is None:
            if len(cache) >= 64:
                cache.pop(next(iter(cache)))
            hit = cache[key] = _torch().stack(list(maps)).contiguous()
        return hit

    def prepare_facet_columns_waves(self, bands, facet_off0s, band, wave_off1s, out, rowmaps=None, workspace=None):
        F, W = bands.shape[0], len(wave_off1s)
        cvp = ctypes.c_void_p
        _lib.check(
            self._lib.swiftly_hip_prepare_facet_columns_waves(
                self._handle, self._code(bands), cvp(bands.data_ptr()), int(bands.shape[1]), bands.stride(1),
                bands.stride(0), F, self._i64(facet_off0s), int(band[0]), int(band[1]), W, self._i64(wave_off1s),
                cvp(out.data_ptr()), out.stride(2), out.stride(0), out.stride(1),
                cvp(rowmaps.data_ptr()) if rowmaps is not None else None,
                rowmaps.stride(0) if rowmaps is not None else 0,
                cvp(workspace.data_ptr()) if workspace is not None else None,
                workspace.numel() * workspace.element_size() if workspace is not None else 0, self._stream(),
            )
        )
        self.k2_columns_issued += W * self.xM_yN_size
        return out

    def wave_subgrid_side(self, G, facet_off0s, facet_off1s, sub_off0s, sub_off1s, subgrid_size, mask0, mask1, tmp, out,
                          placed=False):
        F, S = G.shape[0], G.shape[1]
        cvp = ctypes.c_void_p
        scr = self.scratch("k5b", min(S, 64) * self.xM_size * int(subgrid_size) * G.element_size())
        entry = self._lib.swiftly_hip_wave_subgrid_side_placed if placed else self._lib.swiftly_hip_wave_subgrid_side
        _lib.check(
            entry(
                self._handle, self._code(G), cvp(G.data_ptr()), F, G.stride(0), G.stride(1), self._i64(facet_off0s),
                self._i64(facet_off1s), S, self._i64(sub_off0s), self._i64(sub_off1s), int(subgrid_size),
                cvp(mask0.data_ptr()) if mask0 is not None else None, mask0.stride(0) if mask0 is not None else 0,
                cvp(mask1.data_ptr()) if mask1 is not None else None, mask1.stride(0) if mask1 is not None else 0,
                cvp(tmp.data_ptr()), cvp(out.data_ptr()), cvp(scr.data_ptr()), scr.numel(), self._stream(),
            )
        )
        return out

    def finish_axis1_rows(self, bands, facet_off1s, band, wave_off1, out=None):
        torch = _torch()
        F, rows = bands.shape[0], bands.shape[1]
        m, yN = self.xM_yN_size, self.yN_size
        if out is None:
            out = torch.empty((F, rows, m), dtype=bands.dtype, device=bands.device)
        cvp = ctypes.c_void_p
        _lib.check(
            self._lib.swiftly_hip_finish_axis1_rows(
                self._handle, self._code(bands), cvp(bands.data_ptr()), rows, bands.stride(1), bands.stride(0), F,
                self._i64(facet_off1s), int(band[0]), int(band[1]), int(wave_off1), cvp(out.data_ptr()), out.stride(1),
                out.stride(0), self._stream(),
            )
        )
        s = int(wave_off1) * yN // self.N
        return out, ((yN // 2 - m // 2 + s) % yN, m)

    def sum_finish_facets(self, G, facet_off0s, facet_off1s, out, subgrid_off1s, subgrid_size, mask=None):
        F, S = G.shape[0], G.shape[1]
        f0 = (ctypes.c_int64 * F)(*[int(o) for o in facet_off0s])
        f1 = (ctypes.c_int64 * F)(*[int(o) for o in facet_off1s])
        so = (ctypes.c_int64 * S)(*[int(o) for o in subgrid_off1s])
        _lib.check(
            self._lib.swiftly_hip_sum_finish_facets(
                self._handle, self._code(G), ctypes.c_void_p(G.data_ptr()), F, G.stride(0), G.stride(1), G.stride(2),
                f0, f1, ctypes.c_void_p(out.data_ptr()), out.stride(0), out.stride(1), so, int(subgrid_size),
# ... 246 lines not shown
```

ska-sdp-distributed-fourier-transform_amd/ska_sdp_exec_swiftly_amd/forward.py:

```python
import logging
import os
from functools import cached_property

import numpy

from . import _lib, slabs
from .core_hip import band_range
from .ingest import _FacetIngest, _mask_table
from .prefetch import WavePrefetch, _knobs
from .tasks import DeviceTask, LRUCache, TaskQueue, _torch, _unwrap

log = logging.getLogger("fourier-logger")


def preferred_wave_axis(swiftly_config, dtype=None, n_facets=None):
    return 1 if swiftly_config.core.supports_band_pipeline(dtype, n_facets) else 0


K1_DESCRIPTION = {
    0: "K1 prepare_facet(axis=0) per facet = col_pass<n1=128, mapped load> + col_pass<n2=256, mapped store>",
    1: "K1 prepare_facet(axis=1) of all facet rows, band-compacted parity-split store = row_pass_band_kernel (2 workgroups per row)",
}

class SwiftlyForward(WavePrefetch):
# ... 313 lines not shown
                t0 = timer.start() if timer is not None else None
                if mode == 2:
                    core.prepare_facet_window_rows(data, cfg.off1, self._band, starts, bands[j])
                else:
                    core.prepare_facet_band(data, cfg.off1, self._band, out=bands[j])
                if timer is not None:
                    timer.stop("K1_full_facet_transform", t0)
                self._ingest.prefetch(j + 1)
            ready = None
            if self._plan is not None and _knobs()._PREFETCH and _knobs()._PREFETCH_DEPTH >= 2:
                ready = torch.cuda.Event()
                ready.record(torch.cuda.current_stream(core.device))
            self.install_bands(bands, ready)
            self._bands_own = True
        return self.BF_Fs_persist

    def set_band(self, band):
        self._band = band
        self._axis1_mode = self._choose_axis1_mode()
        self._window_of = {k: w for w, k in enumerate(sorted(self._planned_keys))} if self._axis1_mode == 2 else None
        return self._axis1_mode

    def install_bands(self, bands, ready=None):
        self.BF_Fs_persist, self._bands_ready = bands, ready
        self._k2_chain_forked = False
        self._bands_own = False

    def _wave_rows(self, off1):
        if self._plan is None:
            return None, self.core.yN_size
        key = int(off1)
        if key not in self._wave_rowmaps:
            self._wave_rowmaps[key] = self.core.subgrid_column_rows(self._plan_off0s.get(key, []))
        return self._wave_rowmaps[key]

    axis1_fused = True

    def _choose_axis1_mode(self):
        if not axis1_first_active(self.core, self.wave_axis, self.dtype):
            return 0
        if (self.core.axis1_first is True and self.axis1_fused and self._plan is not None and self._band is not None and
                self.core.supports_window_rows(self._band, self._facet_info[0][1][1], [cfg.off1 for cfg in self.facet_configs],
                                               n_windows=len(self._planned_keys))):
            return 2
        return 1

    def _axis1(self):
        mode = self._axis1_mode
        if mode is None:
            mode = self._choose_axis1_mode() if self.BF_Fs_persist is None else 0
        return mode

    def _placed(self):
        return bool(self._axis1())

    def _k2_source(self, off1):
        bands = self.BF_Fs_persist
        mode = self._axis1()
        if not mode:
            return bands, self._band
        if mode == 2:
            core = self.core
            m, w = core.xM_yN_size, self._window_of[int(off1)]
            start = (core.window_starts(self._band, [off1])[0] + self._band[0]) % core.yN_size
            return bands[:, w], (start, m)
        return self.core.finish_axis1_rows(bands, [cfg.off1 for cfg in self.facet_configs], self._band, off1)

    def _lookup_Q(self, off1):
        self._take_prefetched(off1)
        hit = self.lru.get(("b", off1))
        if hit is not None:
            return hit, hit[1], hit[0].shape[1]
        if self._plan is not None and int(off1) not in self._planned_keys:
            raise ValueError(f"subgrid wave off1={off1} was not in the subgrid_configs plan")
        self.prepare_all_facets()
        return (None, *self._wave_rows(off1))

    def _get_wave_columns(self, off1):
        hit, rowmap, n_rows = self._lookup_Q(off1)
        if hit is None:
            bands, band = self._k2_source(off1)
            Q = self.core.prepare_facet_columns(
                bands, [cfg.off0 for cfg in self.facet_configs], band, off1, rowmap, n_rows
            )
            hit = (Q, rowmap)
            self.lru.set(("b", off1), hit)
        return hit

    def _check_planned(self, sgs):
        if self._plan is not None and any((int(sg.off0), int(sg.off1)) not in self._plan_set for sg in sgs):
            raise ValueError("subgrid was not in the subgrid_configs plan")

    def _wave_b_staged(self, sgs):
        Q, rowmap = self._get_wave_columns(sgs[0].off1)
        self._check_planned(sgs)
        return _finish_from_columns(self.core, Q, 1, self.facet_configs, sgs, [sg.off0 for sg in sgs], rowmap=rowmap,
                                    placed=self._placed())

    def _wave_Q(self, off1):
        hit, rowmap, n_rows = self._lookup_Q(off1)
        if hit is not None:
            return hit[0], rowmap, n_rows, False
        core = self.core
        Q = _torch().empty((len(self.facet_configs), n_rows, core.xM_yN_size), dtype=self.dtype, device=core.device)
        self.lru.set(("b", off1), (Q, rowmap))
        return Q, rowmap, n_rows, True

    @cached_property
    def _slab_plan(self):
        core = self.core
        N, yN, m = core.N, core.yN_size, core.xM_yN_size
        if self._plan is None or yN & (yN - 1) or not slabs.supported(N, yN, m, self._planned_keys):
            return None
        return slabs.SlabPlan(N, yN, m, ((sg.off0, sg.off1) for sg in self._plan))

    def _slabs_on(self):
        return bool(
            _knobs()._K2_SLABS and self.wave_axis == 1 and self._plan is not None and self._bands_own
            and self.dtype == _torch().complex64 and self._axis1() == 0 and self._slab_plan is not None
        )

    def _slab_rows(self, j):
        if j not in self._slab_rowmaps:
            self._slab_rowmaps[j] = self.core.subgrid_column_rows(self._slab_plan.off0s[j])
        return self._slab_rowmaps[j]

    def _slab_has(self, j):
        return ("q", j) in self._slab_lru._items or j in self._slab_kept

    def _slab_cached(self, j):
        hit = self._slab_lru.get(("q", j))
        if hit is None and j in self._slab_kept:
            hit = self._slab_kept.pop(j)
            self._slab_store(j, hit, fresh=False)
        return hit

    def _slab_store(self, j, hit, fresh=True):
        if fresh:
            self._slab_served[j] = set()
        key, old = self._slab_lru.set(("q", j), hit)
        if key is not None and set(self._slab_plan.users[key[1]]) - self._slab_served.get(key[1], set()):
            kept = self._slab_kept
            kept[key[1]] = old
            while len(kept) > self._slab_lru.cache_size:
                kept.pop(next(iter(kept)))

    def _compute_slab(self, j, Q, rowmap):
        plan = self._slab_plan
        off0s = [cfg.off0 for cfg in self.facet_configs]
        for first, count in plan.ranges[j]:
            self.core.prepare_facet_columns_range(self.BF_Fs_persist, off0s, self._band, plan.off1(j), first, count, Q, rowmap)
        return len(plan.ranges[j])

    def _facet_side_slabs(self, sgs, g_out, g_layout):
        core, off1 = self.core, sgs[0].off1
        if int(off1) not in self._planned_keys:
            raise ValueError(f"subgrid wave off1={off1} was not in the subgrid_configs plan")
        torch = _torch()
        wanted = self._slab_plan.pieces(off1)
        self._check_slab_prediction([j for j, _, _ in wanted])
        nxt = self._predict_next_waves(off1, _knobs()._PREFETCH_DEPTH)
        pieces = []
        for j, first, count in wanted:
            hit = self._slab_hit(j)
            if hit is None:
                rowmap, n_rows = self._slab_rows(j)
                Q = torch.empty((len(self.facet_configs), n_rows, core.xM_yN_size), dtype=self.dtype, device=core.device)
                self._compute_slab(j, Q, rowmap)
                hit = (Q, rowmap, n_rows)
                self._slab_store(j, hit)
            self._slab_served.setdefault(j, set()).add(int(off1))
            pieces.append((*hit, first, count))
        self._prefetch_slabs_of(nxt)
        if g_out is None:
            m = core.xM_yN_size
            g_out = torch.empty((len(self.facet_configs), len(sgs), m, m), dtype=self.dtype, device=core.device)
        core.transform_contributions_pieces(pieces, [cfg.off0 for cfg in self.facet_configs], [sg.off0 for sg in sgs], g_out,
                                            g_layout=g_layout)
        return g_out

    def _facet_side(self, sgs, g_out=None, g_layout=None):
        core, off1 = self.core, sgs[0].off1
        bands = self.prepare_all_facets()
        if self._slabs_on():
            return self._facet_side_slabs(sgs, g_out, g_layout)
        Q, rowmap, n_rows, compute = self._wave_Q(off1)
        nxt = self._predict_next_waves(off1, _knobs()._PREFETCH_DEPTH)
        if not compute:
            self._prefetch_waves(nxt)
        if g_out is None:
            m = core.xM_yN_size
            g_out = _torch().empty((len(self.facet_configs), len(sgs), m, m), dtype=self.dtype, device=core.device)
        band = self._band
        if compute:
            bands, band = self._k2_source(off1)
        try:
            core.wave_facet_side(bands, [cfg.off0 for cfg in self.facet_configs], band, off1, rowmap, n_rows, Q, compute,
                                 [sg.off0 for sg in sgs], g_out, g_layout=g_layout)
        except Exception:
            if compute:
                self.lru.discard(("b", off1))
            raise
        if compute:
            self._prefetch_waves(nxt)
        return g_out

    def _wave_b(self, sgs):
        self._check_planned(sgs)
        return _finish_from_G(self.core, self._facet_side(sgs), self.facet_configs, sgs, placed=self._placed())


def axis1_first_active(core, wave_axis, dtype):
    if not (wave_axis == 1 and bool(getattr(core, "axis1_first", False))):
        return False
    return dtype == _torch().complex64


def _finish_from_columns(core, src, layout, facet_configs, sgs, window_offs, rowmap=None, band=None, placed=False):
    torch = _torch()
    xM, xA, S = core.xM_size, sgs[0].size, len(sgs)
    dt, dev = src.dtype, core.device
    if dt != torch.complex64 and not (dt == torch.complex128 and layout == 1):
        raise NotImplementedError("fused subgrid path is complex64 only")
    off0s = [cfg.off0 for cfg in facet_configs]
    off1s = [cfg.off1 for cfg in facet_configs]
    G = core.transform_contributions(src, layout, off0s, window_offs, rowmap=rowmap, band=band)
    return _finish_from_G(core, G, facet_configs, sgs, placed=placed)


def _finish_from_G(core, G, facet_configs, sgs, placed=False):
    torch = _torch()
    xM, xA, S = core.xM_size, sgs[0].size, len(sgs)
    dt, dev = G.dtype, core.device
    off0s = [cfg.off0 for cfg in facet_configs]
    off1s = [cfg.off1 for cfg in facet_configs]
    mask1 = _mask_table(core, sgs, "mask1", xA, dt)
    mask0 = _mask_table(core, sgs, "mask0", xA, dt)
    tmp = torch.empty((S, xM, xA), dtype=dt, device=dev)
    res = torch.empty((S, xA, xA), dtype=dt, device=dev)
    return core.wave_subgrid_side(G, off0s, off1s, [sg.off0 for sg in sgs], [sg.off1 for sg in sgs], xA, mask0, mask1,
                                  tmp, res, placed=placed)


def finish_from_blocks(core, blocks, facet_configs, sgs, transformed=True, placed=False):
    if transformed:
        return _finish_from_G(core, blocks, facet_configs, sgs, placed=placed)
    return sum_and_finish_wave(core, blocks, facet_configs, sgs)


def _facet_grid(facet_configs):
    off0s = sorted({cfg.off0 for cfg in facet_configs})
    off1s = sorted({cfg.off1 for cfg in facet_configs})
    if [(cfg.off0, cfg.off1) for cfg in facet_configs] == [(a, b) for a in off0s for b in off1s]:
        return off0s, off1s
    return None


def _colacc_from_columns(core, cols, facet_configs, sgs):
    torch = _torch()
    grid = _facet_grid(facet_configs)
    if grid is None:
        raise NotImplementedError("fused path needs an off0 x off1 facet grid")
    off0s, groups = grid
    m, xM, S, G = core.xM_yN_size, core.xM_size, len(sgs), len(groups)
    colacc = torch.zeros((G, S, xM, m), dtype=cols.dtype, device=core.device)
    off1s = [sg.off1 for sg in sgs]
    for i, off0_f in enumerate(off0s):
        core.add_to_subgrid_from_columns(cols[i * G : (i + 1) * G], off0_f, colacc, off1s)
    return colacc


def sum_and_finish_wave(core, contrib, facet_configs, sgs):
    torch = _torch()
    m, xM = core.xM_yN_size, core.xM_size
    S = len(sgs)
    dev, dt = core.device, contrib.dtype
    groups = sorted({cfg.off1 for cfg in facet_configs})
    colacc = torch.zeros((len(groups), S, xM, m), dtype=dt, device=dev)
    grid = _facet_grid(facet_configs)
    if grid is not None and contrib.is_contiguous():
        G = len(groups)
        for i, off0_f in enumerate(grid[0]):
            core.launch("add_to_subgrid", contrib[i * G], m, 1, m, colacc, 1, m, off0_f,
                        nbatch=G * S, in_bs=m * m, out_bs=xM * m)
    else:
        for j, cfg in enumerate(facet_configs):
            core.launch("add_to_subgrid", contrib[j], m, 1, m, colacc[groups.index(cfg.off1)], 1, m, cfg.off0,
                        nbatch=S, in_bs=m * m, out_bs=xM * m)
    return _finish_from_colacc(core, colacc, facet_configs, sgs)


def _finish_from_colacc(core, colacc, facet_configs, sgs):
    torch = _torch()
    m, xM = core.xM_yN_size, core.xM_size
    off0, xA, S = sgs[0].off0, sgs[0].size, len(sgs)
    dev, dt = core.device, colacc.dtype
    groups = sorted({cfg.off1 for cfg in facet_configs})
    off1s = [sg.off1 for sg in sgs]
    mask1 = _mask_table(core, sgs, "mask1", xA, dt)
    mask0 = _mask_table(core, sgs, "mask0", xA, dt)
    tmp = torch.empty((S, xM, xA), dtype=dt, device=dev)
    try:
        core.sum_finish_rows(colacc, groups, tmp, off1s, xA, mask=mask1)
    except NotImplementedError:
        acc = torch.zeros((S, xM, xM), dtype=dt, device=dev)
        for g, off1 in enumerate(groups):
            core.launch("add_to_subgrid", colacc[g], xM, m, 1, acc, xM, 1, off1,
                        nbatch=S, in_bs=xM * m, out_bs=xM * xM)
        core.launch("finish_subgrid", acc, xM, xM, 1, tmp, xA, 1, 0, size=xA, mask=mask1,
                    nbatch=S, in_bs=xM * xM, out_bs=xM * xA, offs=off1s, mask_bs=xA if mask1 is not None else 0)
    res = torch.empty((S, xA, xA), dtype=dt, device=dev)
    core.launch("finish_subgrid", tmp, xA, 1, xA, res, 1, xA, off0, size=xA, mask=mask0,
                nbatch=S, in_bs=xM * xA, out_bs=xA * xA, mask_bs=xA if mask0 is not None else 0)
    return res
```

Baseline: 135,700.

## Sum facet contributions per off1 group inside the K3 column kernel

Adds a group-summing K3 column kernel that accumulates the contributions of all facets sharing an off1 into one plane per group, instead of writing a separate plane per facet. A matching sum/finish kernel then reads one plane per group. This cuts the intermediate G tensor size and the memory traffic between K3 and the subgrid-side finish. It is enabled by default through an environment switch when the slab path is on and the facet geometry fits the kernel's held-row budget. The cost is extra planning logic and an LDS-heavy kernel whose occupancy may be limited.

```diff
diff --git a/include/swiftly_hip.h b/include/swiftly_hip.h
--- a/include/swiftly_hip.h
+++ b/include/swiftly_hip.h
@@ -36,7 +36,8 @@
     SWIFTLY_FEATURE_SPLIT_BAND = 4,
     SWIFTLY_FEATURE_WINDOW_ROWS = 5,
     SWIFTLY_FEATURE_BACKWARD_BAND_EXPLICIT = 6,
-    SWIFTLY_FEATURE_SPLIT_PREPARE = 7
+    SWIFTLY_FEATURE_SPLIT_PREPARE = 7,
+    SWIFTLY_FEATURE_K3_GROUP_SUM = 8
 };
 int swiftly_hip_supports(int feature, int dtype, int64_t N, int64_t yN_size, int64_t xM_size, int64_t n_facets);
 enum {
@@ -203,6 +204,16 @@
                                                const int64_t* g_facet_strides, void* stream);
 int swiftly_hip_k3_one_launch(int on);
 
+int swiftly_hip_transform_contributions_groups(swiftly_hip_t* h, int dtype, int64_t npieces, const void* const* q,
+                                               const int64_t* q_facet_strides, const int32_t* const* rowmaps,
+                                               const int64_t* n_rows, const int64_t* first, const int64_t* count,
+                                               int64_t nfacets, const int64_t* facet_off0s, const int64_t* facet_off1s,
+                                               int64_t nsub, const int64_t* sub_off0s, void* p_out, int64_t p_group_stride,
+                                               int64_t p_sub_stride, void* stream);
+int swiftly_hip_k3_group_sum_cover(const swiftly_hip_t* h, int dtype, int64_t nfacets, const int64_t* facet_off0s,
+                                   const int64_t* facet_off1s);
+int swiftly_hip_k3_group_sum(int on);
+
 int swiftly_hip_sum_finish_facets(swiftly_hip_t* h, int dtype, const void* in, int64_t nfacets, int64_t in_facet_stride,
                                   int64_t in_sub_stride, int64_t in_row_stride, const int64_t* facet_off0s,
                                   const int64_t* facet_off1s, void* out, int64_t out_sub_stride, int64_t out_row_stride,
@@ -221,6 +232,12 @@
                                   int64_t nsub, const int64_t* sub_off0s, const int64_t* sub_off1s, int64_t subgrid_size,
                                   const void* mask0, int64_t mask0_bs, const void* mask1, int64_t mask1_bs,
                                   void* tmp_work, void* out, void* scratch, int64_t scratch_bytes, void* stream);
+int swiftly_hip_wave_subgrid_side_groups(swiftly_hip_t* h, int dtype, const void* p, int64_t p_group_stride,
+                                         int64_t p_sub_stride, int64_t nfacets, const int64_t* facet_off0s,
+                                         const int64_t* facet_off1s, int64_t nsub, const int64_t* sub_off0s,
+                                         const int64_t* sub_off1s, int64_t subgrid_size, const void* mask0, int64_t mask0_bs,
+                                         const void* mask1, int64_t mask1_bs, void* tmp_work, void* out, void* scratch,
+                                         int64_t scratch_bytes, void* stream);
 
 int swiftly_hip_finish_axis1_rows(swiftly_hip_t* h, int dtype, const void* bands, int64_t rows, int64_t band_row_stride,
                                   int64_t band_facet_stride, int64_t nfacets, const int64_t* facet_off1s,
diff --git a/ska-sdp-distributed-fourier-transform_amd/csrc/col_pass.hip b/ska-sdp-distributed-fourier-transform_amd/csrc/col_pass.hip
--- a/ska-sdp-distributed-fourier-transform_amd/csrc/col_pass.hip
+++ b/ska-sdp-distributed-fourier-transform_amd/csrc/col_pass.hip
@@ -34,6 +34,28 @@
     if constexpr (LOGN == 7 || LOGN == 8)
         return launch_pieces<typename CGeoFor<LOGN>::type, float>(a, s2, cz, outer, nbatch, s, a.tw, a.tw_full);
     return (int)hipErrorInvalidConfiguration;
+}
+
+template <int LOGN>
+static int launch_group(const ColGroupArgs& a, int ngroups, int nbatch, hipStream_t s) {
+    using G = CGroupGeo<LOGN>;
+    static_assert(G::LDS_BYTES <= 80 * 1024, "two workgroups per CU next to K2");
+    dim3 grid((unsigned)((a.ncols + G::COLS - 1) / G::COLS), (unsigned)ngroups, (unsigned)nbatch);
+    return launch_lds<col_group_kernel<G>, G::LDS_BYTES>(grid, dim3(G::NT), s, a);
+}
+int launch_col_group(int logn, const ColGroupArgs& a, int ngroups, int nbatch, hipStream_t s) {
+#define CG_CASE(M, XX) \
+    if (logn == M) return launch_group<M>(a, ngroups, nbatch, s);
+    K3_GROUP_PAIRS(CG_CASE)
+#undef CG_CASE
+    return (int)hipErrorInvalidConfiguration;
+}
+int col_group_held_rows(int logn) {
+#define CG_HELD(M, XX) \
+    if (logn == M) return CGroupGeo<M>::HELD;
+    K3_GROUP_PAIRS(CG_HELD)
+#undef CG_HELD
+    return 0;
 }
 
 template <int LOGN, int MODE>
diff --git a/ska-sdp-distributed-fourier-transform_amd/csrc/sum_finish.hip b/ska-sdp-distributed-fourier-transform_amd/csrc/sum_finish.hip
--- a/ska-sdp-distributed-fourier-transform_amd/csrc/sum_finish.hip
+++ b/ska-sdp-distributed-fourier-transform_amd/csrc/sum_finish.hip
@@ -16,6 +16,13 @@
     dim3 grid((unsigned)((a.nrows + S::RB - 1) / S::RB), (unsigned)nbatch);
     constexpr size_t lds = sum_finish_facets_kernel_lds<LOGM, LOGX, R>();
     return launch_lds<sum_finish_facets_kernel<LOGM, LOGX, R>, lds>(grid, dim3(S::NT), s, a);
+}
+template <int LOGM, int LOGX>
+static int launch_one_g(const SumFinishFacetArgs& a, int nbatch, hipStream_t s) {
+    using S = SFGeo<LOGM, LOGX>;
+    dim3 grid((unsigned)((a.nrows + S::RB - 1) / S::RB), (unsigned)nbatch);
+    constexpr size_t lds = sum_finish_facets_reg_lds<LOGM, LOGX>();
+    return launch_lds<sum_finish_facets_kernel<LOGM, LOGX, float, true>, lds>(grid, dim3(S::NT), s, a);
 }
 template <int LOGM, int LOGX, typename R>
 constexpr size_t split_prepare_lds() {
@@ -61,6 +68,13 @@
 #undef SF_CASE_F
     return -1;
 }
+int launch_sum_finish_groups(int logm, int logx, const SumFinishFacetArgs& a, int nbatch, hipStream_t s) {
+#define SF_CASE_G(M, XX) \
+    if (logm == M && logx == XX) return launch_one_g<M, XX>(a, nbatch, s);
+    K3_GROUP_PAIRS(SF_CASE_G)
+#undef SF_CASE_G
+    return -1;
+}
 int launch_sum_finish_facets_c128(int logm, int logx, const SumFinishFacetArgs& a, int nbatch, hipStream_t s) {
 #define SF_CASE_D(M, XX) \
     if (logm == M && logx == XX) return launch_one_f<M, XX, double>(a, nbatch, s);
diff --git a/ska-sdp-distributed-fourier-transform_amd/csrc/swiftly_abi_pipeline.hip b/ska-sdp-distributed-fourier-transform_amd/csrc/swiftly_abi_pipeline.hip
--- a/ska-sdp-distributed-fourier-transform_amd/csrc/swiftly_abi_pipeline.hip
+++ b/ska-sdp-distributed-fourier-transform_amd/csrc/swiftly_abi_pipeline.hip
@@ -474,6 +474,127 @@
     return 0;
 }
 
+static std::atomic<int> g_k3_group_sum{getenv("SWIFTLY_K3_GROUP_SUM") ? atoi(getenv("SWIFTLY_K3_GROUP_SUM")) != 0 : 1};
+int swiftly_hip_k3_group_sum(int on) {
+    return on < 0 ? g_k3_group_sum.load() : g_k3_group_sum.exchange(on ? 1 : 0);
+}
+}
+
+static std::string plan_group_sum(const swiftly_hip* h, int dtype, int64_t nfacets, const int64_t* facet_off0s,
+                                  const int64_t* facet_off1s, ColGroupArgs* c, int* ngroups) {
+    if (std::string why = why_not_k3_group_sum(*h, dtype, nfacets); !why.empty()) return why;
+    if (h->col_f64) return "group-summing K3: float32 column arithmetic only";
+    if (nfacets <= 0 || nfacets > kColGroupMaxEntries)
+        return reason("group-summing K3: 1..%d facets, got %lld", kColGroupMaxEntries, (long long)nfacets);
+    SumFinishFacetArgs a;
+    fill_facet_groups(a, h, nfacets, facet_off0s, facet_off1s);
+    const int room = col_group_held_rows(h->log_m);
+    for (int g = 0; g < a.ngroups; g++) {
+        const int n0 = a.gstart[g], n = a.gstart[g + 1] - n0;
+        int64_t off0s[kColGroupMaxEntries];
+        GroupEntry e[kColGroupMaxEntries];
+        for (int i = 0; i < n; i++) off0s[i] = facet_off0s[a.fidx[n0 + i]];
+        int held = 0;
+        if (!group_sum_geometry(*h, n, off0s, e, &held))
+            return reason("group-summing K3: the facets of off1 = %lld overlap by more than m / 2 = %lld rows",
+                          (long long)facet_off1s[a.fidx[n0]], (long long)(h->m / 2));
+        if (held > room)
+            return reason("group-summing K3: %d rows of the group off1 = %lld wait at one time, the kernel holds %d", held,
+                          (long long)facet_off1s[a.fidx[n0]], room);
+        for (int i = 0; i < n && c; i++) {
+            c->fidx[n0 + i] = a.fidx[n0 + e[i].facet];
+            c->st_a[n0 + i] = contribution_in_padded_subgrid(*h, off0s[e[i].facet]).a;
+            c->base0[n0 + i] = e[i].base0; c->head[n0 + i] = e[i].head; c->tail[n0 + i] = e[i].tail; c->gap[n0 + i] = e[i].gap;
+        }
+        if (c) c->gstart[g] = n0;
+    }
+    if (c) c->gstart[a.ngroups] = (int)nfacets;
+    if (ngroups) *ngroups = a.ngroups;
+    return {};
+}
+static int check_pieces(const swiftly_hip* h, const char* who, int64_t npieces, const void* const* q,
+                        const int64_t* q_facet_strides, const int64_t* n_rows, const int64_t* first, const int64_t* count) {
+    if (npieces < 0 || npieces > 2) return fail(SWIFTLY_ERR_PARAM, "%s: 0..2 pieces, got %lld", who, (long long)npieces);
+    const int64_t m = h->m;
+    int64_t covered = 0;
+    for (int64_t i = 0; i < npieces; i++) {
+        if (count[i] < 0 || first[i] < 0 || first[i] + count[i] > m || first[i] % 16 || count[i] % 16)
+            return fail(SWIFTLY_ERR_PARAM, "%s: piece %lld = [%lld, +%lld) must be multiples of 16 "
+                        "inside [0, %lld)", who, (long long)i, (long long)first[i], (long long)count[i], (long long)m);
+        if (count[i] && (!q[i] || n_rows[i] <= 0 || n_rows[i] > h->yN || q_facet_strides[i] < n_rows[i] * m))
+            return fail(SWIFTLY_ERR_PARAM, "bad row count %lld / facet stride %lld", (long long)n_rows[i], (long long)q_facet_strides[i]);
+        covered += count[i];
+    }
+    if (npieces == 2 && count[0] && count[1] && first[0] < first[1] + count[1] && first[1] < first[0] + count[0])
+        return fail(SWIFTLY_ERR_PARAM, "%s: the pieces overlap", who);
+    if (covered != m) return fail(SWIFTLY_ERR_PARAM, "%s: the pieces hold %lld of %lld positions", who, (long long)covered, (long long)m);
+    return 0;
+}
+
+extern "C" {
+int swiftly_hip_k3_group_sum_cover(const swiftly_hip_t* h, int dtype, int64_t nfacets, const int64_t* facet_off0s,
+                                   const int64_t* facet_off1s) {
+    if (!h || !facet_off0s || !facet_off1s) return fail(SWIFTLY_ERR_PARAM, "null argument"), 0;
+    if (!g_k3_group_sum.load()) return fail(SWIFTLY_ERR_UNSUPPORTED, "group-summing K3: switched off"), 0;
+    const std::string why = plan_group_sum(h, dtype, nfacets, facet_off0s, facet_off1s, nullptr, nullptr);
+    if (!why.empty()) return fail(SWIFTLY_ERR_UNSUPPORTED, "%s", why.c_str()), 0;
+    return 1;
+}
+
+int swiftly_hip_transform_contributions_groups(swiftly_hip_t* h, int dtype, int64_t npieces, const void* const* q,
+                                               const int64_t* q_facet_strides, const int32_t* const* rowmaps,
+                                               const int64_t* n_rows, const int64_t* first, const int64_t* count,
+                                               int64_t nfacets, const int64_t* facet_off0s, const int64_t* facet_off1s,
+                                               int64_t nsub, const int64_t* sub_off0s, void* p_out, int64_t p_group_stride,
+                                               int64_t p_sub_stride, void* stream) {
+    if (!h || !q || !q_facet_strides || !rowmaps || !n_rows || !first || !count || !p_out || !facet_off0s || !facet_off1s || !sub_off0s)
+        return fail(SWIFTLY_ERR_PARAM, "null argument");
+    DeviceGuard device_guard_(h->device);
+    if (int rc = check_pieces(h, "transform_contributions_groups", npieces, q, q_facet_strides, n_rows, first, count)) return rc;
+    ColGroupArgs c;
+    std::memset(&c, 0, sizeof c);
+    int ngroups = 0;
+    if (std::string why = plan_group_sum(h, dtype, nfacets, facet_off0s, facet_off1s, &c, &ngroups); !why.empty())
+        return fail(SWIFTLY_ERR_UNSUPPORTED, "%s", why.c_str());
+    if (nsub <= 0) return 0;
+    const int64_t m = h->m, xM = h->xM;
+    if (p_sub_stride < xM * m || p_group_stride < xM * m)
+        return fail(SWIFTLY_ERR_PARAM, "transform_contributions_groups: plane strides %lld / %lld below xM * m", (long long)p_group_stride, (long long)p_sub_stride);
+    CHECK_OFFSETS_32(offsets_fit_32((uint64_t)h->yN, (uint64_t)m, (uint64_t)h->yN) && offsets_fit_32((uint64_t)xM, (uint64_t)m * 8, (uint64_t)m * 8));
+    for (int64_t i = 0; i < npieces; i++) CHECK_OFFSETS_32(!count[i] || offsets_fit_32((uint64_t)n_rows[i], (uint64_t)m * 8, (uint64_t)m * 8));
+    int ia = -1, ib = -1;
+    for (int64_t i = 0; i < npieces; i++) {
+        if (!count[i]) continue;
+        if (count[i] == m) ia = (int)i;
+        else if (first[i] == 0) ib = (int)i;
+        else ia = (int)i;
+    }
+    if (ia < 0) return fail(SWIFTLY_ERR_PARAM, "transform_contributions_groups: no piece");
+    c.in_a = (const cx<float>*)q[ia]; c.fs_a = q_facet_strides[ia]; c.map_a = rowmaps[ia];
+    if (ib >= 0) {
+        c.in_b = (const cx<float>*)q[ib]; c.fs_b = q_facet_strides[ib]; c.map_b = rowmaps[ib];
+        c.split = (int)count[ib];
+    }
+    c.in_pitch = (unsigned)m;
+    c.yN = (int)h->yN;
+    c.out_gs = p_group_stride; c.out_bs = p_sub_stride;
+    c.xM = (int)xM; c.ncols = (int)m;
+    c.fn = h->fn_f;
+    c.tw = twiddles<float>(h, h->log_m);
+    if (!c.tw || !c.fn) return fail(SWIFTLY_ERR_HIP, "internal: missing twiddle table");
+    for (int64_t b0 = 0; b0 < nsub; b0 += kColZB) {
+        const int nb = (int)std::min<int64_t>(kColZB, nsub - b0);
+        for (int b = 0; b < nb; b++) {
+            const Window w = window_of(*h, sub_off0s[b0 + b]);
+            c.b_lda[b] = w.rot;
+            c.b_ldc[b] = w.base;
+        }
+        c.out = (cx<float>*)p_out + b0 * p_sub_stride;
+        if (int rc = launch_status(launch_col_group(h->log_m, c, ngroups, nb, (hipStream_t)stream))) return rc;
+    }
+    return 0;
+}
+
 static int sum_finish_facets_impl(swiftly_hip_t* h, int dtype, const void* in, int64_t nfacets, int64_t in_facet_stride,
                                   int64_t in_sub_stride, int64_t in_row_stride, const int64_t* facet_off0s,
                                   const int64_t* facet_off1s, void* out, int64_t out_sub_stride, int64_t out_row_stride,
@@ -717,6 +838,47 @@
     return wave_subgrid_side_impl(h, dtype, g, nfacets, g_facet_stride, g_sub_stride, facet_off0s, facet_off1s, nsub, sub_off0s,
                                   sub_off1s, subgrid_size, mask0, mask0_bs, mask1, mask1_bs, tmp_work, out, scratch, scratch_bytes,
                                   0, stream);
+}
+
+int swiftly_hip_wave_subgrid_side_groups(swiftly_hip_t* h, int dtype, const void* p, int64_t p_group_stride,
+                                         int64_t p_sub_stride, int64_t nfacets, const int64_t* facet_off0s,
+                                         const int64_t* facet_off1s, int64_t nsub, const int64_t* sub_off0s,
+                                         const int64_t* sub_off1s, int64_t subgrid_size, const void* mask0, int64_t mask0_bs,
+                                         const void* mask1, int64_t mask1_bs, void* tmp_work, void* out, void* scratch,
+                                         int64_t scratch_bytes, void* stream) {
+    if (!h || !p || !tmp_work || !out || !sub_off0s || !sub_off1s || !facet_off0s || !facet_off1s)
+        return fail(SWIFTLY_ERR_PARAM, "null argument");
+    DeviceGuard device_guard_(h->device);
+    CHECK_SUBGRID_SIZE();
+    const bool c128 = false;
+    int ngroups = 0;
+    if (std::string why = plan_group_sum(h, dtype, nfacets, facet_off0s, facet_off1s, nullptr, &ngroups); !why.empty())
+        return fail(SWIFTLY_ERR_UNSUPPORTED, "%s", why.c_str());
+    if (nsub <= 0) return 0;
+    const int64_t m = h->m, xM = h->xM, xA = subgrid_size;
+    if (p_sub_stride < xM * m || p_group_stride < xM * m)
+        return fail(SWIFTLY_ERR_PARAM, "wave_subgrid_side_groups: plane strides %lld / %lld below xM * m", (long long)p_group_stride, (long long)p_sub_stride);
+    SumFinishFacetArgs a;
+    std::memset(&a, 0, sizeof a);
+    a.in_fs = p_group_stride; a.in_bs = p_sub_stride; a.in_rs = m;
+    a.out_bs = xM * xA; a.out_rs = xA;
+    a.nrows = (int)xM;
+    a.nfacets = (int)nfacets;
+    a.xA = (int)xA;
+    fill_facet_groups(a, h, nfacets, facet_off0s, facet_off1s);
+    a.mask_bs = mask1 ? mask1_bs : 0;
+    if (int rc = fill_sum_finish_tables(h, c128, &a.fn, &a.tw_m, &a.tw_x, &a.twc_m, &a.twc_x)) return rc;
+    for (int64_t b0 = 0; b0 < nsub; b0 += kSumFinishMaxBatch) {
+        const int nb = (int)std::min<int64_t>(kSumFinishMaxBatch, nsub - b0);
+        a.in = cx_at(p, b0 * p_sub_stride, c128);
+        a.out = cx_at(tmp_work, b0 * xM * xA, c128);
+        a.mask = mask1 ? (const float*)mask1 + b0 * mask1_bs : nullptr;
+        for (int b = 0; b < nb; b++) a.st_a[b] = subgrid_in_padded_subgrid(*h, xA, sub_off1s[b0 + b]).a;
+        if (int rc = launch_status(launch_sum_finish_groups(h->log_m, h->log_xM, a, nb, (hipStream_t)stream))) return rc;
+    }
+    CallWorkspace call_ws(scratch, scratch ? (size_t)scratch_bytes : 0);
+    return swiftly_hip_finish_subgrid_batch(h, dtype, tmp_work, xA, 1, xA, out, 1, xA, 0, subgrid_size, mask0, nsub,
+                                            xM * xA, xA * xA, sub_off0s, mask0 ? mask0_bs : 0, stream);
 }
 
 int swiftly_hip_wave_subgrid_side_placed(swiftly_hip_t* h, int dtype, const void* g, int64_t nfacets, int64_t g_facet_stride,
diff --git a/ska-sdp-distributed-fourier-transform_amd/csrc/swiftly_abi_util.hip b/ska-sdp-distributed-fourier-transform_amd/csrc/swiftly_abi_util.hip
--- a/ska-sdp-distributed-fourier-transform_amd/csrc/swiftly_abi_util.hip
+++ b/ska-sdp-distributed-fourier-transform_amd/csrc/swiftly_abi_util.hip
@@ -64,6 +64,7 @@
             case SWIFTLY_FEATURE_WINDOW_ROWS: why = why_not_window_rows(s); break;
             case SWIFTLY_FEATURE_BACKWARD_BAND_EXPLICIT: why = why_not_backward_band(s, dtype, true); break;
             case SWIFTLY_FEATURE_SPLIT_PREPARE: why = why_not_split_prepare(s, dtype, n_facets); break;
+            case SWIFTLY_FEATURE_K3_GROUP_SUM: why = why_not_k3_group_sum(s, dtype, n_facets); break;
             default: why = reason("unknown feature %d", feature);
         }
     }
diff --git a/ska-sdp-distributed-fourier-transform_amd/csrc/swiftly_caps.h b/ska-sdp-distributed-fourier-transform_amd/csrc/swiftly_caps.h
--- a/ska-sdp-distributed-fourier-transform_amd/csrc/swiftly_caps.h
+++ b/ska-sdp-distributed-fourier-transform_amd/csrc/swiftly_caps.h
@@ -29,6 +29,8 @@
 #define SF_PAIRS_C128(X) X(7, 8) X(7, 10) X(8, 9) X(8, 10) X(9, 10)
 #define SPLIT_PAIRS_C128(X) X(7, 8) X(7, 10) X(8, 9) X(8, 10) X(9, 10)
 
+#define K3_GROUP_PAIRS(X) X(9, 10)
+
 #define SF_HAS(M, XX) \
     if (logm == M && logx == XX) return true;
 inline bool sum_finish_supported(int logm, int logx) {
@@ -37,6 +39,10 @@
 }
 inline bool sum_finish_c128_supported(int logm, int logx) {
     SF_PAIRS_C128(SF_HAS)
+    return false;
+}
+inline bool k3_group_sum_instance(int logm, int logx) {
+    K3_GROUP_PAIRS(SF_HAS)
     return false;
 }
 inline bool split_prepare_c128_supported(int logm, int logx) {
@@ -182,6 +188,13 @@
                       1 << kBandMinLog, 1 << kBandMixedMaxLog, (long long)s.xM, (long long)s.m, (long long)s.yN);
     return {};
 }
+inline std::string why_not_k3_group_sum(const Sizes& s, int dtype, int64_t n_facets) {
+    if (std::string why = why_not_fused_subgrid(s, dtype, n_facets); !why.empty()) return why;
+    if (!k3_group_sum_instance(s.log_m, s.log_xM))
+        return reason("group-summing K3: no instance for m %lld, xM %lld", (long long)s.m, (long long)s.xM);
+    if (s.yN < s.m) return "group-summing K3: yN < m";
+    return {};
+}
 inline std::string why_not_split_band(const Sizes& s) {
     if (band_is_split(&s)) return {};
     return reason("yN %lld keeps the whole padded axis in the plain band layout (split: %d .. %d)", (long long)s.yN,
diff --git a/ska-sdp-distributed-fourier-transform_amd/csrc/swiftly_colpass.h b/ska-sdp-distributed-fourier-transform_amd/csrc/swiftly_colpass.h
--- a/ska-sdp-distributed-fourier-transform_amd/csrc/swiftly_colpass.h
+++ b/ska-sdp-distributed-fourier-transform_amd/csrc/swiftly_colpass.h
@@ -437,8 +437,115 @@
                                                             &S2);
 }
 
+constexpr int kColGroupMaxEntries = 32;
+struct ColGroupArgs {
+    const cx<float>* in_a;
+    const cx<float>* in_b;
+    long long fs_a, fs_b;
+    const int* map_a;
+    const int* map_b;
+    int split;
+    unsigned in_pitch;
+    int yN;
+    cx<float>* out;
+    long long out_gs, out_bs;
+    int xM, ncols;
+    const float* fn;
+    const cx<float>* tw;
+    int b_lda[kColZB], b_ldc[kColZB];
+    int gstart[kColGroupMaxEntries + 1];
+    int fidx[kColGroupMaxEntries];
+    int st_a[kColGroupMaxEntries];
+    int base0[kColGroupMaxEntries], head[kColGroupMaxEntries], tail[kColGroupMaxEntries], gap[kColGroupMaxEntries];
+};
+template <int LOGN_>
+struct CGroupGeo {
+    static constexpr int LOGN = LOGN_, LOGP = 5;
+    static constexpr bool SPLIT = true;
+    static constexpr int N = 1 << LOGN, P = 1 << LOGP, T = N / P;
+    static constexpr bool WAVE_ROWS = false;
+    static constexpr int COLS = 16, NT = COLS * T, RB = COLS;
+    static_assert(LOGN > LOGP && T % 4 == 0, "a wave works on four thread-rows");
+    static constexpr int PITCH = 0, LOGPAD = 4;
+    static constexpr size_t EX_BYTES = (size_t)N * RB * sizeof(float);
+    static constexpr int HELD = LOGN >= 9 ? 352 : N;
+    static constexpr size_t LDS_BYTES = EX_BYTES + (size_t)HELD * COLS * sizeof(cx<float>) + (size_t)N * 8;
+    static constexpr int MINW = 4;
+};
+template <class G>
+__global__ __launch_bounds__(G::NT, G::MINW) void col_group_kernel(const ColGroupArgs A) {
+    constexpr int P = G::P, T = G::T, N = G::N, COLS = G::COLS;
+    extern __shared__ __attribute__((aligned(16))) unsigned char smem[];
+    cx<float>* hold = reinterpret_cast<cx<float>*>(smem + G::EX_BYTES);
+    int* row_tab = reinterpret_cast<int*>(smem + G::EX_BYTES + (size_t)G::HELD * COLS * sizeof(cx<float>));
+    float* fn_tab = reinterpret_cast<float*>(row_tab + N);
+    const int wave = __builtin_amdgcn_readfirstlane(threadIdx.x >> 6), lane = threadIdx.x & 63;
+    const int hq = lane >> 4, clane = lane & 15;
+    const int t = 4 * wave + hq;
+    const int b = blockIdx.z, g = blockIdx.y;
+    const int tile0 = blockIdx.x * COLS, col = tile0 + clane;
+    const bool from_b = tile0 < A.split;
+    const cx<float>* __restrict__ piece = from_b ? A.in_b : A.in_a;
+    const long long fs = from_b ? A.fs_b : A.fs_a;
+    const int* __restrict__ map = from_b ? A.map_b : A.map_a;
+    char* __restrict__ out = reinterpret_cast<char*>(A.out + (long long)g * A.out_gs + (long long)b * A.out_bs);
+    const unsigned col8 = (unsigned)col * 8u, opitch = (unsigned)A.ncols * 8u, ipitch = A.in_pitch * 8u;
+    auto store = [&](unsigned row, cx<float> v) { cp_store<true>(reinterpret_cast<cx<float>*>(out + (row * opitch + col8)), v); };
+    const int xmask = A.xM - 1;
+    for (int i = threadIdx.x; i < N; i += G::NT) {
+        const int q = (((i + (N >> 1)) & (N - 1)) + A.b_lda[b]) & (N - 1);
+        int idx = q + A.b_ldc[b];
+        if (idx >= A.yN) idx -= A.yN;
+        row_tab[i] = map ? map[idx] : idx;
+    }
+    const int n0 = A.gstart[g], n1 = A.gstart[g + 1];
+    const int wrap = A.head[n0];
+    for (int n = n0; n < n1; n++) {
+        const bool first = n == n0, last = n == n1 - 1;
+        const int st_a = A.st_a[n], base0 = A.base0[n], head = A.head[n], tail = A.tail[n], gap = A.gap[n];
+        const char* __restrict__ in = reinterpret_cast<const char*>(piece + (long long)A.fidx[n] * fs);
+        auto row_of = [&](int e) { return (((e + (N >> 1)) & (N - 1)) + st_a) & (N - 1); };
+        for (int e = threadIdx.x; e < N; e += G::NT) fn_tab[e] = A.fn[row_of(e)];
+        __syncthreads();
+        cx<float> x[P];
+        static_for<0, P>([&](auto vI) {
+            constexpr int v = decltype(vI)::value;
+            const int row = row_tab[t + v * T];
+            cx<float> val = {0.f, 0.f};
+            if (row >= 0) val = cp_load<true>(reinterpret_cast<const cx<float>*>(in + ((unsigned)row * ipitch + col8)));
+            x[v] = val;
+        });
+        for (int j = t; j < gap; j += T)
+            store((unsigned)((base0 + N + j) & xmask), cx<float>{0.f, 0.f});
+        cx<float>* stage = reinterpret_cast<cx<float>*>(smem);
+        static_assert((size_t)(N / 2) * COLS * sizeof(cx<float>) <= G::EX_BYTES, "an overlap of m / 2 rows fits the exchange buffer");
+        fft_phases<G, float, 0>(x, t, clane, true, smem, A.tw, [&](int e, cx<float> v) {
+            asm("" : "+v"(e) : "v"(v.x));
+            const float w = fn_tab[e];
+            v.x *= w;
+            v.y *= w;
+            const int k = row_of(e);
+            const bool in_head = k < head, in_tail = k >= N - tail;
+            const bool rd = in_head ? !first : (in_tail && last), wr = in_head ? first : (in_tail && !last);
+            const int slot = in_head ? (first ? k : wrap + k) : k - (N - tail);
+            cx<float>* l = ((in_tail && wr) ? stage : hold) + slot * COLS + clane;
+            cx<float> c = {0.f, 0.f};
+            if (rd) c = *l;
+            if (wr) *l = v;
+            else store((unsigned)((k + base0) & xmask), cx<float>{v.x + c.x, v.y + c.y});
+        });
+        if (!last) {
+            __syncthreads();
+            for (int i = threadIdx.x; i < tail * COLS; i += G::NT) hold[wrap * COLS + i] = stage[i];
+            __syncthreads();
+        }
+    }
+}
+
 constexpr int kColPassMinLog = 2;
 constexpr int kColPassMaxLog = 10;
+int launch_col_group(int logn, const ColGroupArgs& a, int ngroups, int nbatch, hipStream_t s);
+int col_group_held_rows(int logn);
 
 int launch_col_pass(int logn, int mode, const ColPassArgs& a, const ColZ& cz, int outer, int nbatch, hipStream_t s,
                     const ColPassSrc2* src2 = nullptr);
diff --git a/ska-sdp-distributed-fourier-transform_amd/csrc/swiftly_geometry.h b/ska-sdp-distributed-fourier-transform_amd/csrc/swiftly_geometry.h
--- a/ska-sdp-distributed-fourier-transform_amd/csrc/swiftly_geometry.h
+++ b/ska-sdp-distributed-fourier-transform_amd/csrc/swiftly_geometry.h
@@ -67,6 +67,39 @@
     return -1;
 }
 
+struct GroupEntry {
+    int facet;
+    int base0, head, tail, gap;
+};
+inline bool group_sum_geometry(const Sizes& z, int n, const int64_t* facet_off0s, GroupEntry* out, int* held) {
+    const int m = (int)z.m, xM = (int)z.xM;
+    if (held) *held = 0;
+    if (n <= 0 || m <= 0 || m > xM) return false;
+    for (int i = 0; i < n; i++) {
+        GroupEntry e{i, placement_start(z, facet_shift(z, facet_off0s[i])), 0, 0, 0};
+        int j = i;
+        for (; j > 0 && out[j - 1].base0 > e.base0; j--) out[j] = out[j - 1];
+        out[j] = e;
+    }
+    if (n == 1) {
+        out[0].gap = xM - m;
+        return true;
+    }
+    bool ok = true;
+    int most = 0;
+    for (int i = 0; i < n; i++) {
+        const int nx = i + 1 < n ? i + 1 : 0;
+        const int d = out[nx].base0 - out[i].base0 + (nx == 0 ? xM : 0);
+        const int ov = d < m ? m - d : 0;
+        out[i].tail = out[nx].head = ov;
+        out[i].gap = d > m ? d - m : 0;
+        if (2 * ov > m) ok = false;
+        if (nx != 0 && ov > most) most = ov;
+    }
+    if (held) *held = out[0].head + most;
+    return ok;
+}
+
 inline bool offsets_fit_32(uint64_t count, uint64_t stride, uint64_t extra = 0) {
     return count * stride + extra < (uint64_t(1) << 32);
 }
diff --git a/ska-sdp-distributed-fourier-transform_amd/csrc/swiftly_sumfinish.h b/ska-sdp-distributed-fourier-transform_amd/csrc/swiftly_sumfinish.h
--- a/ska-sdp-distributed-fourier-transform_amd/csrc/swiftly_sumfinish.h
+++ b/ska-sdp-distributed-fourier-transform_amd/csrc/swiftly_sumfinish.h
@@ -159,9 +159,10 @@
     int placed;
 };
 
-template <int LOGM, int LOGX, typename R = float>
+template <int LOGM, int LOGX, typename R = float, bool DENSE = false>
 __global__ __launch_bounds__((SFGeo<LOGM, LOGX, R>::NT), (!std::is_same_v<R, float> ? 2 : LOGX <= 10 ? 4 : 1)) void sum_finish_facets_kernel(const SumFinishFacetArgs A) {
     using S = SFGeo<LOGM, LOGX, R>;
+    static_assert(!DENSE || (std::is_same_v<R, float> && !SFWide<LOGM, LOGX>::ON), "group planes: the float register form");
     using GX = typename S::GX;
     using W = SFWide<LOGM, LOGX>;
     using GM = std::conditional_t<W::ON, typename W::GM, typename S::GM>;
@@ -279,9 +280,17 @@
     for (int g = 0; g < A.ngroups; g++) {
         cx<R> xs[PM];
         static_for<0, PM>([&](auto vI) { xs[decltype(vI)::value] = cx<R>{(R)0, (R)0}; });
-        bool anyg = false;
+        bool anyg = DENSE;
+        if constexpr (DENSE) {
+            const cx<R>* __restrict__ in = g_in + (long long)g * A.in_fs + (long long)b * A.in_bs + (long long)(live ? row : 0) * A.in_rs;
+            static_for<0, PM>([&](auto vI) {
+                constexpr int v = decltype(vI)::value;
+                const cx<R> val = in[(t + v * TR) ^ (M >> 1)];
+                xs[v] = live ? val : cx<R>{(R)0, (R)0};
+            });
+        }
         int n = A.gstart[g];
-        const int ne = A.gstart[g + 1];
+        const int ne = DENSE ? n : A.gstart[g + 1];
         while (n < ne) {
             int fs[NB];
             int cnt = 0;
@@ -619,6 +628,7 @@
 int launch_split_prepare_facets_c128(int logm, int logx, const SplitFacetArgs& a, int nbatch, hipStream_t s);
 int launch_sum_finish_facets(int logm, int logx, const SumFinishFacetArgs& a, int nbatch, hipStream_t s);
 int launch_sum_finish_facets_c128(int logm, int logx, const SumFinishFacetArgs& a, int nbatch, hipStream_t s);
+int launch_sum_finish_groups(int logm, int logx, const SumFinishFacetArgs& a, int nbatch, hipStream_t s);
 int launch_sum_finish_rows(int logm, int logx, const SumFinishArgs& a, int nbatch, hipStream_t s);
 int launch_axis1_rows(int logm, const Axis1RowsArgs& a, int nfacets, hipStream_t s);
 
diff --git a/ska-sdp-distributed-fourier-transform_amd/ska_sdp_exec_swiftly_amd/_lib.py b/ska-sdp-distributed-fourier-transform_amd/ska_sdp_exec_swiftly_amd/_lib.py
--- a/ska-sdp-distributed-fourier-transform_amd/ska_sdp_exec_swiftly_amd/_lib.py
+++ b/ska-sdp-distributed-fourier-transform_amd/ska_sdp_exec_swiftly_amd/_lib.py
@@ -8,7 +8,7 @@
 C64, C128 = 0, 1
 ERR_PARAM, ERR_UNSUPPORTED, ERR_HIP = 1, 2, 3
 (FEATURE_FUSED_SUBGRID, FEATURE_BAND_PIPELINE, FEATURE_BAND_PIPELINE_EXPLICIT, FEATURE_BACKWARD_BAND, FEATURE_SPLIT_BAND,
- FEATURE_WINDOW_ROWS, FEATURE_BACKWARD_BAND_EXPLICIT, FEATURE_SPLIT_PREPARE) = range(8)
+ FEATURE_WINDOW_ROWS, FEATURE_BACKWARD_BAND_EXPLICIT, FEATURE_SPLIT_PREPARE, FEATURE_K3_GROUP_SUM) = range(9)
 LIMIT_FUSED_FACETS, LIMIT_WINDOW_ROWS_STAGE_COLUMNS, LIMIT_WINDOW_ROWS_WINDOWS = range(3)
 
 _lib = None
@@ -130,6 +130,18 @@
     lib.swiftly_hip_wave_subgrid_side.argtypes = [
         vp, c_int, vp, i64, i64, i64, pi64, pi64, i64, pi64, pi64, i64, vp, i64, vp, i64, vp, vp, vp, i64, vp,
     ]
+    lib.swiftly_hip_k3_group_sum.restype = c_int
+    lib.swiftly_hip_k3_group_sum.argtypes = [c_int]
+    lib.swiftly_hip_k3_group_sum_cover.restype = c_int
+    lib.swiftly_hip_k3_group_sum_cover.argtypes = [vp, c_int, i64, pi64, pi64]
+    lib.swiftly_hip_transform_contributions_groups.restype = c_int
+    lib.swiftly_hip_transform_contributions_groups.argtypes = [
+        vp, c_int, i64, POINTER(vp), pi64, POINTER(vp), pi64, pi64, pi64, i64, pi64, pi64, i64, pi64, vp, i64, i64, vp,
+    ]
+    lib.swiftly_hip_wave_subgrid_side_groups.restype = c_int
+    lib.swiftly_hip_wave_subgrid_side_groups.argtypes = [
+        vp, c_int, vp, i64, i64, i64, pi64, pi64, i64, pi64, pi64, i64, vp, i64, vp, i64, vp, vp, vp, i64, vp,
+    ]
     lib.swiftly_hip_wave_subgrid_side_placed.restype = c_int
     lib.swiftly_hip_wave_subgrid_side_placed.argtypes = list(lib.swiftly_hip_wave_subgrid_side.argtypes)
     lib.swiftly_hip_prepare_facet_window_rows.restype = c_int
diff --git a/ska-sdp-distributed-fourier-transform_amd/ska_sdp_exec_swiftly_amd/core_hip.py b/ska-sdp-distributed-fourier-transform_amd/ska_sdp_exec_swiftly_amd/core_hip.py
--- a/ska-sdp-distributed-fourier-transform_amd/ska_sdp_exec_swiftly_amd/core_hip.py
+++ b/ska-sdp-distributed-fourier-transform_amd/ska_sdp_exec_swiftly_amd/core_hip.py
@@ -576,6 +576,50 @@
         )
         return g_out
 
+    def supports_k3_group_sum(self, dtype, facet_off0s, facet_off1s):
+        torch = _torch()
+        code = {torch.complex64: _lib.C64, torch.complex128: _lib.C128}.get(dtype)
+        if code is None:
+            return False
+        return bool(self._lib.swiftly_hip_k3_group_sum_cover(self._handle, code, len(facet_off0s), self._i64(facet_off0s),
+                                                             self._i64(facet_off1s)))
+
+    def transform_contributions_groups(self, pieces, facet_off0s, facet_off1s, sub_off0s, p_out=None):
+        n = len(pieces)
+        F, S = pieces[0][0].shape[0], len(sub_off0s)
+        cvp = ctypes.c_void_p
+        if p_out is None:
+            p_out = _torch().empty((len(set(int(o) for o in facet_off1s)), S, self.xM_size, self.xM_yN_size),
+                                   dtype=pieces[0][0].dtype, device=self._device)
+        qs = (cvp * n)(*[pc[0].data_ptr() for pc in pieces])
+        maps = (cvp * n)(*[pc[1].data_ptr() if pc[1] is not None else None for pc in pieces])
+        _lib.check(
+            self._lib.swiftly_hip_transform_contributions_groups(
+                self._handle, self._code(pieces[0][0]), n, qs, self._i64([pc[0].stride(0) for pc in pieces]), maps,
+                self._i64([pc[2] for pc in pieces]), self._i64([pc[3] for pc in pieces]),
+                self._i64([pc[4] for pc in pieces]), F, self._i64(facet_off0s), self._i64(facet_off1s), S,
+                self._i64(sub_off0s), cvp(p_out.data_ptr()), p_out.stride(0), p_out.stride(1), self._stream(),
+            )
+        )
+        return p_out
+
+    def wave_subgrid_side_groups(self, P, facet_off0s, facet_off1s, sub_off0s, sub_off1s, subgrid_size, mask0, mask1, tmp,
+                                 out):
+        S = P.shape[1]
+        cvp = ctypes.c_void_p
+        scr = self.scratch("k5b", min(S, 64) * self.xM_size * int(subgrid_size) * P.element_size())
+        _lib.check(
+            self._lib.swiftly_hip_wave_subgrid_side_groups(
+                self._handle, self._code(P), cvp(P.data_ptr()), P.stride(0), P.stride(1), len(facet_off0s),
+                self._i64(facet_off0s), self._i64(facet_off1s), S, self._i64(sub_off0s), self._i64(sub_off1s),
+                int(subgrid_size), cvp(mask0.data_ptr()) if mask0 is not None else None,
+                mask0.stride(0) if mask0 is not None else 0, cvp(mask1.data_ptr()) if mask1 is not None else None,
+                mask1.stride(0) if mask1 is not None else 0, cvp(tmp.data_ptr()), cvp(out.data_ptr()), cvp(scr.data_ptr()),
+                scr.numel(), self._stream(),
+            )
+        )
+        return out
+
     def transform_contributions(self, src, layout, facet_off0s, subgrid_offs, out=None, rowmap=None, band=None, nsub=None):
         torch = _torch()
         F = src.shape[0]
diff --git a/ska-sdp-distributed-fourier-transform_amd/ska_sdp_exec_swiftly_amd/forward.py b/ska-sdp-distributed-fourier-transform_amd/ska_sdp_exec_swiftly_amd/forward.py
--- a/ska-sdp-distributed-fourier-transform_amd/ska_sdp_exec_swiftly_amd/forward.py
+++ b/ska-sdp-distributed-fourier-transform_amd/ska_sdp_exec_swiftly_amd/forward.py
@@ -489,7 +489,7 @@
             self.core.prepare_facet_columns_range(self.BF_Fs_persist, off0s, self._band, plan.off1(j), first, count, Q, rowmap)
         return len(plan.ranges[j])
 
-    def _facet_side_slabs(self, sgs, g_out, g_layout):
+    def _facet_side_slabs(self, sgs, g_out, g_layout, grouped=False):
         core, off1 = self.core, sgs[0].off1
         if int(off1) not in self._planned_keys:
             raise ValueError(f"subgrid wave off1={off1} was not in the subgrid_configs plan")
@@ -509,6 +509,9 @@
             self._slab_served.setdefault(j, set()).add(int(off1))
             pieces.append((*hit, first, count))
         self._prefetch_slabs_of(nxt)
+        if grouped:
+            return core.transform_contributions_groups(pieces, [cfg.off0 for cfg in self.facet_configs],
+                                                       [cfg.off1 for cfg in self.facet_configs], [sg.off0 for sg in sgs])
         if g_out is None:
             m = core.xM_yN_size
             g_out = torch.empty((len(self.facet_configs), len(sgs), m, m), dtype=self.dtype, device=core.device)
@@ -544,7 +547,17 @@
 
     def _wave_b(self, sgs):
         self._check_planned(sgs)
+        if self._grouped_k3():
+            self.prepare_all_facets()
+            P = self._facet_side_slabs(sgs, None, None, grouped=True)
+            return _finish_from_G(self.core, P, self.facet_configs, sgs, grouped=True)
         return _finish_from_G(self.core, self._facet_side(sgs), self.facet_configs, sgs, placed=self._placed())
+
+    def _grouped_k3(self):
+        if not self._slabs_on() or self._placed():
+            return False
+        return self.core.supports_k3_group_sum(self.dtype, [cfg.off0 for cfg in self.facet_configs],
+                                               [cfg.off1 for cfg in self.facet_configs])
 
 
 def axis1_first_active(core, wave_axis, dtype):
@@ -565,7 +578,7 @@
     return _finish_from_G(core, G, facet_configs, sgs, placed=placed)
 
 
-def _finish_from_G(core, G, facet_configs, sgs, placed=False):
+def _finish_from_G(core, G, facet_configs, sgs, placed=False, grouped=False):
     torch = _torch()
     xM, xA, S = core.xM_size, sgs[0].size, len(sgs)
     dt, dev = G.dtype, core.device
@@ -575,6 +588,9 @@
     mask0 = _mask_table(core, sgs, "mask0", xA, dt)
     tmp = torch.empty((S, xM, xA), dtype=dt, device=dev)
     res = torch.empty((S, xA, xA), dtype=dt, device=dev)
+    if grouped:
+        return core.wave_subgrid_side_groups(G, off0s, off1s, [sg.off0 for sg in sgs], [sg.off1 for sg in sgs], xA, mask0,
+                                             mask1, tmp, res)
     return core.wave_subgrid_side(G, off0s, off1s, [sg.off0 for sg in sgs], [sg.off1 for sg in sgs], xA, mask0, mask1,
                                   tmp, res, placed=placed)
 
```

New measurement: 132,600. -2.3%, worse.
